# mourisl/T1K

Measured on AMD Instinct MI355X. Metric: genotyped reads/sec (end-to-end genotyper stage, 2x150 bp HLA), higher is better.
Workload: dtype u64

## Files before the change

### include/t1k_gpu.h

```cpp
#ifndef T1K_GPU_H
#define T1K_GPU_H

#include <stddef.h>
#include <stdint.h>

#ifdef __cplusplus
extern "C" {
#endif

typedef enum {
  T1K_OK = 0,
  T1K_ERR_ARG = -1,
  T1K_ERR_DEVICE = -2,
  T1K_ERR_CAPACITY = -3,
  T1K_ERR_IO = -4,
  T1K_ERR_STATE = -5,
  T1K_ERR_INTERNAL = -6,
  T1K_ERR_COMMITTED = -7
} t1k_status;

typedef struct t1k_ctx t1k_ctx;
typedef struct t1k_job t1k_job;
typedef struct t1k_rowset t1k_rowset;
typedef struct t1k_comm t1k_comm;

typedef struct {
  int32_t kmer_length;
  int32_t radius;
  int32_t hit_len_required;
  double ref_seq_similarity;
  int32_t relax_intron_align;
  int32_t max_assign_cnt;
  int32_t max_read_len;
  int32_t workgroups;
  int64_t group_cap;
  int64_t cand_cap;
  int64_t ovl_cap;
  int64_t row_cap;
  int32_t n_base_code;
  int32_t store_chunk_mb;
} t1k_params;

void t1k_params_default(t1k_params *p);

int t1k_ctx_create(int device, const t1k_params *params, t1k_ctx **out);
void t1k_ctx_destroy(t1k_ctx *ctx);
const char *t1k_last_error(const t1k_ctx *ctx);
int t1k_device_count(void);
int t1k_device_memory(int device, uint64_t *freeBytes, uint64_t *totalBytes);

int t1k_ref_upload(t1k_ctx *ctx, const char *seqs, const uint64_t *offsets, const uint8_t *exon, uint32_t nAlleles);

int t1k_reads_upload(t1k_ctx *ctx, const char *seqs, const uint64_t *offsets, const uint32_t *weights, uint32_t nReadEnds);
int t1k_reads_upload_begin(t1k_ctx *ctx, uint32_t nReadEnds, uint64_t textBytes, int maxReadLen);
int t1k_reads_upload_piece(t1k_ctx *ctx, int what, const void *src, uint64_t byteOffset, uint64_t bytes, int slot);
int t1k_reads_upload_wait(t1k_ctx *ctx, int slot);
int t1k_reads_upload_end(t1k_ctx *ctx);

int t1k_reads_dedupe(t1k_ctx *ctx, uint32_t *distinctOf, uint32_t *nDistinct);

typedef struct {
  int32_t seq_idx, read_start, read_end, seq_start, seq_end, strand;
  int32_t match_cnt, left_clip, right_clip, relaxed_match_cnt;
  double similarity;
} t1k_overlap;

int t1k_assign_batch(t1k_ctx *ctx);
int t1k_assign_range(t1k_ctx *ctx, uint64_t first, uint32_t count);
int t1k_overlaps_download(t1k_ctx *ctx, uint32_t *counts, t1k_overlap *ovl, uint64_t cap, uint64_t *total);

typedef struct {
  int32_t allele_idx, start, end;
  float weight, qual, adjust_weight;
} t1k_row_entry;

int t1k_pair_batch(t1k_ctx *ctx, const uint32_t *end1, const uint32_t *end2, const uint8_t *hasN, uint32_t nFragments);
int t1k_rows_download(t1k_ctx *ctx, uint32_t *rowCounts, uint8_t *fragAssigned, t1k_row_entry *rows, uint64_t cap, uint64_t *total);

typedef struct {
  int32_t allele, start, end;
  float weight, adjust_weight;
} t1k_group_entry;
int t1k_rowset_create(t1k_ctx *owner, uint64_t nFragments, const uint8_t *whitelist , t1k_rowset **out);
int t1k_rowset_trim(t1k_rowset *rs, uint64_t n_fragments);
void t1k_rowset_destroy(t1k_rowset *rs);
int t1k_rowset_set_raw(t1k_rowset *rs, int raw);
int t1k_rowset_device_bytes(t1k_rowset *rs, uint64_t *bytes, uint64_t *rowEntries);
const char *t1k_rowset_last_error(const t1k_rowset *rs);
int t1k_pair_into(t1k_ctx *ctx, t1k_rowset *rs, const uint32_t *end1, const uint32_t *end2, const uint8_t *hasN, uint32_t nFragments, uint64_t fragBase);
int t1k_rowset_coalesce(t1k_rowset *rs, uint64_t *nGroups, uint64_t *nEntries, uint64_t *assignedFragments);
int t1k_rowset_coalesce_sized(t1k_rowset *rs, uint64_t *nGroups, uint64_t *nEntries, uint64_t *assignedFragments, void (*sized)(uint64_t nGroups, uint64_t nEntries, void *user), void *user);
int t1k_rowset_groups_download(t1k_rowset *rs, uint64_t *groupPtr, t1k_group_entry *entries, uint32_t *firstFragment);
int t1k_rowset_assigned_download(t1k_rowset *rs, uint8_t *fragAssigned);
int t1k_rowset_assigned_range(t1k_rowset *rs, uint64_t first, uint64_t count, uint8_t *fragAssigned);
int t1k_rowset_rows_download(t1k_rowset *rs, uint64_t first, uint32_t count, uint32_t *rowCounts, t1k_row_entry *rows, uint64_t cap, uint64_t *total);

typedef struct t1k_comm_group t1k_comm_group;
int t1k_comm_unique_id(void *id128);
t1k_comm_group *t1k_comm_group_create(int nRanks);
void t1k_comm_group_destroy(t1k_comm_group *g);
int t1k_comm_init(t1k_ctx *ctx, int nRanks, int rank, const void *id128, t1k_comm_group *group, int transport , t1k_comm **out);
int t1k_comm_bind(t1k_comm *c, t1k_ctx *ctx);
int t1k_comm_abort(t1k_comm *c);
void t1k_comm_destroy(t1k_comm *c);
const char *t1k_comm_last_error(const t1k_comm *c);
int t1k_comm_rank(const t1k_comm *c);
int t1k_comm_size(const t1k_comm *c);
int t1k_comm_is_rccl(const t1k_comm *c);
int t1k_comm_allreduce(t1k_comm *c, void *dev, uint64_t count, int kind);
int t1k_comm_allgather_u64(t1k_comm *c, const uint64_t *mine, uint32_t k, uint64_t *all);
int t1k_comm_alltoallv(t1k_comm *c, const void *sendbuf, const uint64_t *sendOff, void *recvbuf, const uint64_t *recvOff);
int t1k_comm_allgatherv(t1k_comm *c, const void *mine, const uint64_t *bytes, const uint64_t *displ, void *out);
int t1k_comm_allgatherv_host(t1k_comm *c, void *host, const uint64_t *bytes, const uint64_t *displ, uint64_t total);
int t1k_rowset_exchange(t1k_rowset *rs, t1k_comm *comm, uint64_t fragBase);
int t1k_rowset_groups_gather(t1k_rowset *rs, t1k_comm *comm, uint64_t *totalGroups, uint64_t *totalEntries, uint64_t *totalAssigned);
int t1k_rowset_groups_download_all(t1k_rowset *rs, uint32_t *sizes, t1k_group_entry *entries, uint32_t *firstFragment);
int t1k_em_shard(t1k_ctx *ctx, uint32_t rowBegin, uint32_t rowEnd, t1k_comm *comm);

int t1k_coverage_get(t1k_ctx *ctx, int32_t *out, uint64_t cap);
int t1k_coverage_reset(t1k_ctx *ctx);
int t1k_missing_coverage(t1k_ctx *ctx, int32_t *missing);
typedef struct t1k_readset t1k_readset;
int t1k_ctx_set_coverage_mode(t1k_ctx *ctx, int deferred);
int t1k_readset_detach(t1k_ctx *reader, t1k_readset **out);
int t1k_readset_take_store(t1k_readset *rs, t1k_ctx *pipe, int slot);
uint64_t t1k_readset_bytes(const t1k_readset *rs);
uint32_t t1k_readset_size(const t1k_readset *rs);
const char *t1k_readset_last_error(const t1k_readset *rs);
void t1k_readset_destroy(t1k_readset *rs);
int t1k_coverage_selected(t1k_ctx *ctx, t1k_readset *rs, const uint8_t *selected, uint64_t *nRecords);
typedef struct t1k_xwin t1k_xwin;
int t1k_xwin_create(t1k_ctx *owner, uint64_t maxReadEnds, uint32_t maxWindows, t1k_xwin **out);
void t1k_xwin_destroy(t1k_xwin *x);
const char *t1k_xwin_last_error(const t1k_xwin *x);
int t1k_xwin_link(t1k_xwin *x, t1k_ctx *reader, uint32_t window, uint32_t *nExternal);
int t1k_xwin_resolve(t1k_xwin *x, t1k_ctx *ctx, uint32_t window);

int t1k_ref_share(t1k_ctx *dst, const t1k_ctx *src);
uint64_t t1k_pool_release(void);
void *t1k_pinned_alloc(uint64_t bytes);
void t1k_pinned_free(void *p);
int t1k_reads_share(t1k_ctx *dst, const t1k_ctx *src);
int t1k_reads_attach(t1k_ctx *dst, const t1k_ctx *src, int storeSlot, int resetStore);
int t1k_coverage_absorb(t1k_ctx *dst, t1k_ctx *src);

int t1k_extract_batch(t1k_ctx *ctx, uint32_t endsPerFragment, uint8_t *good, uint64_t *stats);

int t1k_align_count_batch(t1k_ctx *ctx, const char *text, const uint32_t *tOff, const char *pat, const uint32_t *pOff, const uint32_t *len, uint32_t nJobs,
                          int32_t *nMatch);
int t1k_align_batch(t1k_ctx *ctx, const char *text, const uint32_t *tOff, const uint32_t *tLen, const char *pat, const uint32_t *pOff,
                    const uint32_t *pLen, uint32_t nJobs, int32_t *score, int32_t *nMatch, int32_t *nMismatch, int32_t *nIndel, int8_t *ops,
                    const uint32_t *opsOff, uint32_t *nOps);

typedef void (*t1k_allreduce_fn)(void *dev_f64, uint64_t n, void *user);
int t1k_em_setup(t1k_ctx *ctx, const uint64_t *rowPtr, const uint32_t *ecIdx, const double *count, const int32_t *ecLen, uint32_t nGroups,
                 uint32_t nEc, t1k_allreduce_fn allreduce, void *user);
int t1k_em_update(t1k_ctx *ctx, const double *x0, double *x1, double *ecReadCount, double *diff);

int t1k_barcode_em(t1k_ctx *ctx, uint32_t nBarcodes, const uint64_t *bcAllelePtr, const uint32_t *bcAllele, const uint64_t *bcGroupPtr,
                   const double *groupCount, const uint64_t *groupEntryPtr, const uint32_t *entryLocal, const double *rho, uint32_t nAlleles,
                   double alpha, double tol, int32_t maxIter, double *nOut, int32_t *itersOut, double *kernelMs);

typedef struct {
  uint64_t read_ends, lookups, postings, hits, groups, candidates, extended, near_best, dp_calls, rows, batches;
  double ms_seed, ms_chain, ms_extend, ms_select, ms_fullalign, ms_pair, ms_em, ms_total;
  uint64_t read_ends_total, pair_overlaps, dp_cells;
  double ms_load, ms_device, ms_coalesce, ms_write;
} t1k_stats;
int t1k_stats_get(t1k_ctx *ctx, t1k_stats *out);
double t1k_alloc_ms(t1k_ctx *ctx, uint64_t *bytes);
uint64_t t1k_ctx_mem_report(t1k_ctx *ctx, const char *tag, int print);

int t1k_genotyper_main(int argc, char **argv);
int t1k_extractor_main(int argc, char **argv);
int t1k_bam_extractor_main(int argc, char **argv);
int t1k_analyzer_main(int argc, char **argv);

typedef struct {
  t1k_params dev;
  double filter_frac, filter_cov, cross_gene_rate, squarem_min_alpha;
  int32_t allele_digit_units;
  char allele_delimiter;
  int32_t threads;
  int32_t device;
  int32_t output_read_assignment;
  int32_t batch_fragments;
} t1k_job_params;
void t1k_job_params_default(t1k_job_params *p);

int t1k_job_create(const t1k_job_params *p, const char *refFasta, t1k_job **out);
void t1k_job_destroy(t1k_job *job);
const char *t1k_job_last_error(const t1k_job *job);
int t1k_job_load_reads(t1k_job *job, const char *file1, const char *file2, const char *barcodeFile);
int t1k_job_load_reads_multi(t1k_job *job, const char *const *files1, uint32_t n1, const char *const *files2, uint32_t n2, const char *barcodeFile);
typedef struct t1k_reads t1k_reads;
int t1k_reads_open(const char *const *files1, uint32_t n1, const char *const *files2, uint32_t n2, const char *barcodeFile, int threads, t1k_reads **out);
int t1k_reads_open_stream(const char *const *files1, uint32_t n1, const char *const *files2, uint32_t n2, const char *barcodeFile, int threads, t1k_reads **out);
const char *t1k_reads_last_error(const t1k_reads *reads);
int t1k_reads_fragments(const t1k_reads *reads, uint64_t *nFragments);
void t1k_reads_close(t1k_reads *reads);
int t1k_job_attach_reads(t1k_job *job, t1k_reads *reads);
int t1k_job_set_reads(t1k_job *job, const char *seq1, const uint64_t *off1, const char *seq2, const uint64_t *off2, uint32_t nFragments);
int t1k_job_run(t1k_job *job);
int t1k_job_set_output_prefix(t1k_job *job, const char *prefix);
int t1k_job_write_outputs(t1k_job *job, const char *prefix);
int t1k_job_genotype_text(t1k_job *job, char *buf, uint64_t cap, uint64_t *needed);
int t1k_job_counts(t1k_job *job, uint64_t *fragments, uint64_t *assignedFragments, uint64_t *groups, uint64_t *ecs, int32_t *emIterations);
int t1k_job_stats(t1k_job *job, t1k_stats *out);
t1k_ctx *t1k_job_ctx(t1k_job *job);
int t1k_job_set_shard(t1k_job *job, int rank, int nRanks, t1k_comm *comm);
int t1k_job_share_reads(t1k_job *dst, t1k_job *src);
int t1k_job_run_local(t1k_job *job);
int t1k_job_finish(t1k_job *job);
int t1k_job_groups_serialize(t1k_job *job, void *buf, uint64_t cap, uint64_t *needed);
int t1k_job_groups_merge(t1k_job *job, const void *const *bufs, const uint64_t *lens, uint32_t n);
int t1k_job_coalesce_rows(t1k_job *job, const t1k_row_entry *rows, const uint32_t *rowCounts, const uint32_t *fragments, uint32_t nFragments);
int t1k_coverage_device(t1k_ctx *ctx, void **devPtr, uint64_t *count);

typedef struct {
  int32_t allele_idx;
  int32_t has_mate_pair, o1_from_r2;
  t1k_overlap o1, o2;
  uint64_t ops1, ops2;
  uint32_t n_ops1, n_ops2;
} t1k_frag_assignment;
int t1k_fragment_details(const t1k_overlap *l1, uint32_t n1, const t1k_overlap *l2, uint32_t n2, int paired, const int32_t *alleles, uint32_t nAlleles,
                         t1k_frag_assignment *out);
typedef struct {
  int32_t allele_idx, ref_pos, exon_pos;
  char ref, var;
  int32_t qual, group, output_group;
  double var_support, all_support, var_uniq_support;
} t1k_variant;
typedef struct t1k_variants t1k_variants;
int t1k_variants_call(t1k_job *job, const double *abundance, int32_t var_max_group, uint32_t nFragments, const uint64_t *asgPtr, const t1k_frag_assignment *asg,
                      const int8_t *ops, const char *const *read1, const uint32_t *len1, const char *const *read2, const uint32_t *len2, t1k_variants **out);
uint32_t t1k_variants_count(const t1k_variants *v);
int t1k_variants_get(const t1k_variants *v, t1k_variant *out );
int t1k_variants_vcf(const t1k_variants *v, char *buf, uint64_t cap, uint64_t *needed);
int t1k_variants_adjust(const t1k_variants *v, const t1k_frag_assignment *asg, uint32_t n, const int8_t *ops, const char *read1, uint32_t len1, const char *read2, uint32_t len2,
                        uint8_t *keep);
void t1k_variants_destroy(t1k_variants *v);

#ifdef __cplusplus
}
#endif
#endif
```

### t1k_amd/capi.py

```python
import ctypes as C
import gzip
import os

import numpy as np

_HERE = os.path.dirname(os.path.abspath(__file__))


def lib_path():
    return os.environ.get("T1K_GPU_LIB") or os.path.join(_HERE, "lib", "libt1k_gpu.so")


class T1kError(RuntimeError):
    pass


class Params(C.Structure):
    _fields_ = [("kmer_length", C.c_int32), ("radius", C.c_int32), ("hit_len_required", C.c_int32),
                ("ref_seq_similarity", C.c_double), ("relax_intron_align", C.c_int32), ("max_assign_cnt", C.c_int32),
                ("max_read_len", C.c_int32), ("workgroups", C.c_int32), ("group_cap", C.c_int64),
                ("cand_cap", C.c_int64), ("ovl_cap", C.c_int64), ("row_cap", C.c_int64), ("n_base_code", C.c_int32), ("store_chunk_mb", C.c_int32)]


class JobParams(C.Structure):
    _fields_ = [("dev", Params), ("filter_frac", C.c_double), ("filter_cov", C.c_double),
                ("cross_gene_rate", C.c_double), ("squarem_min_alpha", C.c_double), ("allele_digit_units", C.c_int32),
                ("allele_delimiter", C.c_char), ("threads", C.c_int32), ("device", C.c_int32),
                ("output_read_assignment", C.c_int32), ("batch_fragments", C.c_int32)]


class Stats(C.Structure):
    _fields_ = [(n, C.c_uint64) for n in ("read_ends", "lookups", "postings", "hits", "groups", "candidates", "extended",
                                          "near_best", "dp_calls", "rows", "batches")] + \
               [(n, C.c_double) for n in ("ms_seed", "ms_chain", "ms_extend", "ms_select", "ms_fullalign", "ms_pair", "ms_em", "ms_total")] + \
               [(n, C.c_uint64) for n in ("read_ends_total", "pair_overlaps", "dp_cells")] + \
               [(n, C.c_double) for n in ("ms_load", "ms_device", "ms_coalesce", "ms_write")]

    def as_dict(self):
        return {n: getattr(self, n) for n, _ in self._fields_}


OVERLAP_DTYPE = np.dtype([("seq_idx", "<i4"), ("read_start", "<i4"), ("read_end", "<i4"), ("seq_start", "<i4"),
                          ("seq_end", "<i4"), ("strand", "<i4"), ("match_cnt", "<i4"), ("left_clip", "<i4"),
                          ("right_clip", "<i4"), ("relaxed_match_cnt", "<i4"), ("similarity", "<f8")])
ROW_DTYPE = np.dtype([("allele_idx", "<i4"), ("start", "<i4"), ("end", "<i4"), ("weight", "<f4"), ("qual", "<f4"),
                      ("adjust_weight", "<f4")])
assert OVERLAP_DTYPE.itemsize == 48 and ROW_DTYPE.itemsize == 24
FRAG_ASG_DTYPE = np.dtype([("allele_idx", "<i4"), ("has_mate_pair", "<i4"), ("o1_from_r2", "<i4"), ("_pad", "<i4"), ("o1", OVERLAP_DTYPE), ("o2", OVERLAP_DTYPE),
                           ("ops1", "<u8"), ("ops2", "<u8"), ("n_ops1", "<u4"), ("n_ops2", "<u4")])
VARIANT_DTYPE = np.dtype([("allele_idx", "<i4"), ("ref_pos", "<i4"), ("exon_pos", "<i4"), ("ref", "S1"), ("var", "S1"), ("_pad", "S2"), ("qual", "<i4"), ("group", "<i4"),
                          ("output_group", "<i4"), ("_pad2", "<i4"), ("var_support", "<f8"), ("all_support", "<f8"), ("var_uniq_support", "<f8")])
assert FRAG_ASG_DTYPE.itemsize == 136 and VARIANT_DTYPE.itemsize == 56

ALLREDUCE_FN = C.CFUNCTYPE(None, C.c_void_p, C.c_uint64, C.c_void_p)

_lib = None


def lib():
    global _lib
    if _lib is not None:
        return _lib
    p = lib_path()
    if not os.path.exists(p):
        raise T1kError("%s not found: run `python -c 'import __graft_entry__ as g; g.build()'` first" % p)
    L = C.CDLL(p)
    vp, u64p, u32p, u8p, i32p = C.c_void_p, C.POINTER(C.c_uint64), C.POINTER(C.c_uint32), C.POINTER(C.c_uint8), C.POINTER(C.c_int32)
    L.t1k_params_default.argtypes = [C.POINTER(Params)]
    L.t1k_ctx_create.argtypes = [C.c_int, C.POINTER(Params), C.POINTER(vp)]
    L.t1k_ctx_destroy.argtypes = [vp]
    L.t1k_last_error.argtypes = [vp]
    L.t1k_last_error.restype = C.c_char_p
    L.t1k_device_count.restype = C.c_int
    L.t1k_ref_upload.argtypes = [vp, C.c_char_p, vp, vp, C.c_uint32]
    L.t1k_reads_upload.argtypes = [vp, C.c_char_p, vp, vp, C.c_uint32]
    L.t1k_assign_batch.argtypes = [vp]
    L.t1k_assign_range.argtypes = [vp, C.c_uint64, C.c_uint32]
    L.t1k_overlaps_download.argtypes = [vp, vp, vp, C.c_uint64, u64p]
    L.t1k_pair_batch.argtypes = [vp, vp, vp, vp, C.c_uint32]
    L.t1k_rows_download.argtypes = [vp, vp, vp, vp, C.c_uint64, u64p]
    L.t1k_coverage_get.argtypes = [vp, vp, C.c_uint64]
    L.t1k_coverage_reset.argtypes = [vp]
    L.t1k_missing_coverage.argtypes = [vp, vp]
    L.t1k_coverage_absorb.argtypes = [vp, vp]
    L.t1k_align_batch.argtypes = [vp, C.c_char_p, vp, vp, C.c_char_p, vp, vp, C.c_uint32, vp, vp, vp, vp, vp, vp, vp]
    L.t1k_align_count_batch.argtypes = [vp, C.c_char_p, vp, C.c_char_p, vp, vp, C.c_uint32, vp]
    L.t1k_em_setup.argtypes = [vp, vp, vp, vp, vp, C.c_uint32, C.c_uint32, ALLREDUCE_FN, vp]
    L.t1k_em_update.argtypes = [vp, vp, vp, vp, vp]
    L.t1k_barcode_em.argtypes = [vp, C.c_uint32, vp, vp, vp, vp, vp, vp, vp, C.c_uint32, C.c_double, C.c_double, C.c_int32, vp, vp, C.POINTER(C.c_double)]
    L.t1k_extract_batch.argtypes = [vp, C.c_uint32, vp, vp]
    L.t1k_extractor_main.argtypes = [C.c_int, C.POINTER(C.c_char_p)]
    L.t1k_stats_get.argtypes = [vp, C.POINTER(Stats)]
    L.t1k_genotyper_main.argtypes = [C.c_int, C.POINTER(C.c_char_p)]
    L.t1k_job_params_default.argtypes = [C.POINTER(JobParams)]
    L.t1k_job_create.argtypes = [C.POINTER(JobParams), C.c_char_p, C.POINTER(vp)]
    L.t1k_job_destroy.argtypes = [vp]
    L.t1k_job_last_error.argtypes = [vp]
    L.t1k_job_last_error.restype = C.c_char_p
    L.t1k_job_load_reads.argtypes = [vp, C.c_char_p, C.c_char_p, C.c_char_p]
    L.t1k_job_set_reads.argtypes = [vp, C.c_char_p, vp, C.c_char_p, vp, C.c_uint32]
    L.t1k_job_run.argtypes = [vp]
    L.t1k_job_write_outputs.argtypes = [vp, C.c_char_p]
    L.t1k_pool_release.restype = C.c_uint64
    L.t1k_pool_release.argtypes = []
    L.t1k_job_load_reads_multi.argtypes = [vp, C.POINTER(C.c_char_p), C.c_uint32, C.POINTER(C.c_char_p), C.c_uint32, C.c_char_p]
    L.t1k_reads_open.argtypes = [C.POINTER(C.c_char_p), C.c_uint32, C.POINTER(C.c_char_p), C.c_uint32, C.c_char_p, C.c_int, C.POINTER(vp)]
    L.t1k_reads_open_stream.argtypes = [C.POINTER(C.c_char_p), C.c_uint32, C.POINTER(C.c_char_p), C.c_uint32, C.c_char_p, C.c_int, C.POINTER(vp)]
    L.t1k_reads_last_error.argtypes = [vp]
    L.t1k_reads_last_error.restype = C.c_char_p
    L.t1k_reads_fragments.argtypes = [vp, u64p]
    L.t1k_reads_close.argtypes = [vp]
    L.t1k_reads_close.restype = None
    L.t1k_job_attach_reads.argtypes = [vp, vp]
    L.t1k_job_genotype_text.argtypes = [vp, C.c_char_p, C.c_uint64, u64p]
    L.t1k_job_counts.argtypes = [vp, u64p, u64p, u64p, u64p, i32p]
    L.t1k_job_stats.argtypes = [vp, C.POINTER(Stats)]
    L.t1k_job_ctx.argtypes = [vp]
    L.t1k_job_ctx.restype = vp
    L.t1k_job_run_local.argtypes = [vp]
    L.t1k_job_finish.argtypes = [vp]
    L.t1k_job_groups_serialize.argtypes = [vp, vp, C.c_uint64, u64p]
    L.t1k_reads_dedupe.argtypes = [vp, vp, u32p]
    L.t1k_job_groups_merge.argtypes = [vp, vp, vp, C.c_uint32]
    L.t1k_job_coalesce_rows.argtypes = [vp, vp, vp, vp, C.c_uint32]
    L.t1k_variants_call.argtypes = [vp, vp, C.c_int32, C.c_uint32, vp, vp, vp, vp, vp, vp, vp, C.POINTER(vp)]
    L.t1k_fragment_details.argtypes = [vp, C.c_uint32, vp, C.c_uint32, C.c_int, vp, C.c_uint32, vp]
    L.t1k_variants_count.argtypes = [vp]
    L.t1k_variants_count.restype = C.c_uint32
    L.t1k_variants_get.argtypes = [vp, vp]
    L.t1k_variants_vcf.argtypes = [vp, vp, C.c_uint64, u64p]
    L.t1k_variants_adjust.argtypes = [vp, vp, C.c_uint32, vp, C.c_char_p, C.c_uint32, C.c_char_p, C.c_uint32, vp]
    L.t1k_variants_destroy.argtypes = [vp]
    L.t1k_job_set_shard.argtypes = [vp, C.c_int, C.c_int, vp]
    L.t1k_job_share_reads.argtypes = [vp, vp]
    L.t1k_job_ctx.restype = vp
    L.t1k_job_ctx.argtypes = [vp]
    L.t1k_comm_unique_id.argtypes = [vp]
    L.t1k_comm_init.argtypes = [vp, C.c_int, C.c_int, vp, vp, C.c_int, C.POINTER(vp)]
    L.t1k_comm_bind.argtypes = [vp, vp]
    L.t1k_comm_destroy.argtypes = [vp]
    L.t1k_comm_last_error.restype = C.c_char_p
    L.t1k_comm_last_error.argtypes = [vp]
    L.t1k_comm_is_rccl.argtypes = [vp]
    L.t1k_comm_group_create.restype = vp
    L.t1k_comm_group_create.argtypes = [C.c_int]
    L.t1k_comm_group_destroy.argtypes = [vp]
    L.t1k_coverage_device.argtypes = [vp, C.POINTER(vp), u64p]
    L.t1k_device_memory.argtypes = [C.c_int, u64p, u64p]
    L.t1k_ctx_set_coverage_mode.argtypes = [vp, C.c_int]
    L.t1k_readset_detach.argtypes = [vp, C.POINTER(vp)]
    L.t1k_readset_take_store.argtypes = [vp, vp, C.c_int]
    L.t1k_readset_bytes.argtypes = [vp]
    L.t1k_readset_bytes.restype = C.c_uint64
    L.t1k_readset_size.argtypes = [vp]
    L.t1k_readset_size.restype = C.c_uint32
    L.t1k_readset_destroy.argtypes = [vp]
    L.t1k_coverage_selected.argtypes = [vp, vp, vp, u64p]
    _lib = L
    return L


def _ptr(a):
    return a.ctypes.data_as(C.c_void_p) if a is not None else None


def _concat(seqs):
    offs = np.zeros(len(seqs) + 1, dtype=np.uint64)
    if len(seqs):
        offs[1:] = np.cumsum([len(s) for s in seqs], dtype=np.uint64)
    blob = "".join(seqs).encode("ascii")
    return blob, offs


class Context:

    def __init__(self, device=0, **kw):
        L = lib()
        p = Params()
        L.t1k_params_default(C.byref(p))
        for k, v in kw.items():
            setattr(p, k, v)
        self.params = p
        h = C.c_void_p()
        rc = L.t1k_ctx_create(device, C.byref(p), C.byref(h))
        if rc != 0:
            raise T1kError("t1k_ctx_create failed (%d): no usable GPU / bad parameters" % rc)
        self.h = h
        self.n_read_ends = 0
        self.allele_len = None

    def _check(self, rc, what):
        if rc != 0:
            raise T1kError("%s failed (%d): %s" % (what, rc, lib().t1k_last_error(self.h).decode()))

    def close(self):
        if self.h:
            lib().t1k_ctx_destroy(self.h)
            self.h = None

    def __del__(self):
        try:
            self.close()
        except Exception:
            pass

    def ref_upload(self, seqs, exon_masks=None):
        blob, offs = _concat(seqs)
        ex = None
        if exon_masks is not None:
            ex = np.concatenate([np.asarray(m, dtype=np.uint8) for m in exon_masks]) if len(seqs) else np.zeros(0, np.uint8)
        self.allele_len = np.array([len(s) for s in seqs], dtype=np.int64)
        self._check(lib().t1k_ref_upload(self.h, blob, _ptr(offs), _ptr(ex), len(seqs)), "t1k_ref_upload")

    def reads_upload(self, seqs, weights=None):
        blob, offs = _concat(seqs)
        w = None if weights is None else np.asarray(weights, dtype=np.uint32)
        self.n_read_ends = len(seqs)
        self._check(lib().t1k_reads_upload(self.h, blob, _ptr(offs), _ptr(w), len(seqs)), "t1k_reads_upload")

    def reads_dedupe(self):
        out = np.zeros(self.n_read_ends, dtype=np.uint32)
        nd = C.c_uint32()
        self._check(lib().t1k_reads_dedupe(self.h, _ptr(out), C.byref(nd)), "t1k_reads_dedupe")
        self.n_uploaded, self.n_read_ends = self.n_read_ends, nd.value
        return out

    def assign(self):
        self._check(lib().t1k_assign_batch(self.h), "t1k_assign_batch")

    def extract(self, ends_per_fragment=1):
        good = np.zeros(self.n_read_ends // ends_per_fragment, dtype=np.uint8)
        st = np.zeros(8, dtype=np.uint64)
        self._check(lib().t1k_extract_batch(self.h, ends_per_fragment, _ptr(good), _ptr(st)), "t1k_extract_batch")
        return good, dict(zip(("read_ends", "lookups", "postings", "read_ends_with_hits", "read_ends_chained", "screen_ns", "main_ns", "big_shape"), (int(x) for x in st)))

    def overlaps(self):
        n = self.n_read_ends
        counts = np.zeros(n, dtype=np.uint32)
        tot = C.c_uint64()
        self._check(lib().t1k_overlaps_download(self.h, _ptr(counts), None, 0, C.byref(tot)), "t1k_overlaps_download")
        out = np.zeros(tot.value, dtype=OVERLAP_DTYPE)
        self._check(lib().t1k_overlaps_download(self.h, _ptr(counts), _ptr(out), tot.value, C.byref(tot)), "t1k_overlaps_download")
        return counts, out

    def pair(self, end1, end2, has_n):
        e1 = np.asarray(end1, dtype=np.uint32)
        e2 = None if end2 is None else np.asarray(end2, dtype=np.uint32)
        hn = np.asarray(has_n, dtype=np.uint8)
        self.n_fragments = len(e1)
        self._check(lib().t1k_pair_batch(self.h, _ptr(e1), _ptr(e2), _ptr(hn), len(e1)), "t1k_pair_batch")

    def rows(self):
        n = self.n_fragments
        counts = np.zeros(n, dtype=np.uint32)
        assigned = np.zeros(n, dtype=np.uint8)
        tot = C.c_uint64()
        self._check(lib().t1k_rows_download(self.h, _ptr(counts), _ptr(assigned), None, 0, C.byref(tot)), "t1k_rows_download")
        out = np.zeros(tot.value, dtype=ROW_DTYPE)
        self._check(lib().t1k_rows_download(self.h, _ptr(counts), _ptr(assigned), _ptr(out), tot.value, C.byref(tot)), "t1k_rows_download")
        return counts, assigned, out

    def coverage(self):
        tot = int(self.allele_len.sum())
        out = np.zeros(tot, dtype=np.int32)
        self._check(lib().t1k_coverage_get(self.h, _ptr(out), tot), "t1k_coverage_get")
        return out

    def set_coverage_mode(self, deferred):
        self._check(lib().t1k_ctx_set_coverage_mode(self.h, 1 if deferred else 0), "t1k_ctx_set_coverage_mode")

    def detach_readset(self, slot=0):
        h = C.c_void_p()
        self._check(lib().t1k_readset_detach(self.h, C.byref(h)), "t1k_readset_detach")
        rs = Readset(h)
        self._check(lib().t1k_readset_take_store(rs.h, self.h, slot), "t1k_readset_take_store")
        return rs

    def coverage_selected(self, readset, selected):
        sel = np.ascontiguousarray(selected, dtype=np.uint8)
        n = C.c_uint64()
        self._check(lib().t1k_coverage_selected(self.h, readset.h, _ptr(sel), C.byref(n)), "t1k_coverage_selected")
        return n.value

    def coverage_reset(self):
        self._check(lib().t1k_coverage_reset(self.h), "t1k_coverage_reset")

    def missing_coverage(self):
        out = np.zeros(len(self.allele_len), dtype=np.int32)
        self._check(lib().t1k_missing_coverage(self.h, _ptr(out)), "t1k_missing_coverage")
        return out

    def stats(self):
        s = Stats()
        lib().t1k_stats_get(self.h, C.byref(s))
        return s.as_dict()

    def align_batch(self, texts, pats, want_ops=True):
        n = len(texts)
        tb, toff = _concat(texts)
        pb, poff = _concat(pats)
        tlen = np.array([len(t) for t in texts], dtype=np.uint32)
        plen = np.array([len(p) for p in pats], dtype=np.uint32)
        toff32, poff32 = toff[:-1].astype(np.uint32), poff[:-1].astype(np.uint32)
        score = np.zeros(n, np.int32); nm = np.zeros(n, np.int32); nx = np.zeros(n, np.int32); ni = np.zeros(n, np.int32)
        ops_off = np.zeros(n, np.uint32)
        if n:
            ops_off[1:] = np.cumsum((tlen + plen + 2)[:-1], dtype=np.uint64).astype(np.uint32)
        ops = np.zeros(int((tlen + plen + 2).sum()) + 8, np.int8)
        nops = np.zeros(n, np.uint32)
        self._check(lib().t1k_align_batch(self.h, tb, _ptr(toff32), _ptr(tlen), pb, _ptr(poff32), _ptr(plen), n, _ptr(score), _ptr(nm),
                                          _ptr(nx), _ptr(ni), _ptr(ops) if want_ops else None, _ptr(ops_off), _ptr(nops)), "t1k_align_batch")
        op_list = [ops[ops_off[i]:ops_off[i] + nops[i]].copy() for i in range(n)] if want_ops else None
        return score, nm, nx, ni, op_list

    def align_count_batch(self, texts, pats):
        n = len(texts)
        tb, toff = _concat(texts)
        pb, poff = _concat(pats)
        ln = np.array([len(t) for t in texts], dtype=np.uint32)
        out = np.zeros(n, np.int32)
        self._check(lib().t1k_align_count_batch(self.h, tb, _ptr(toff[:-1].astype(np.uint32)), pb, _ptr(poff[:-1].astype(np.uint32)), _ptr(ln), n,
                                                _ptr(out)), "t1k_align_count_batch")
        return out

    def em_setup(self, row_ptr, ec_idx, count, ec_len, allreduce=None):
        self._em_keep = (np.asarray(row_ptr, np.uint64), np.asarray(ec_idx, np.uint32), np.asarray(count, np.float64), np.asarray(ec_len, np.int32))
        rp, ei, ct, el = self._em_keep
        self._em_cb = ALLREDUCE_FN(allreduce) if allreduce else C.cast(None, ALLREDUCE_FN)
        self._em_nec = len(el)
        self._check(lib().t1k_em_setup(self.h, _ptr(rp), _ptr(ei), _ptr(ct), _ptr(el), len(ct), len(el), self._em_cb, None), "t1k_em_setup")

    def em_update(self, x0):
        x0 = np.ascontiguousarray(x0, dtype=np.float64)
        x1 = np.zeros(self._em_nec, np.float64)
        n = np.zeros(self._em_nec, np.float64)
        diff = C.c_double()
        self._check(lib().t1k_em_update(self.h, _ptr(x0), _ptr(x1), _ptr(n), C.byref(diff)), "t1k_em_update")
        return x1, n, diff.value

    def barcode_em(self, bc_allele_ptr, bc_allele, bc_group_ptr, group_count, group_entry_ptr, entry_local, rho, n_alleles, alpha=0.0, tol=1e-7,
                   max_iter=1000, raw=False):
        ap = np.ascontiguousarray(bc_allele_ptr, np.uint64)
        al = np.ascontiguousarray(bc_allele, np.uint32)
        gp = np.ascontiguousarray(bc_group_ptr, np.uint64)
        gc = np.ascontiguousarray(group_count, np.float64)
        ep = np.ascontiguousarray(group_entry_ptr, np.uint64)
        el = np.ascontiguousarray(entry_local, np.uint32)
        rh = None if rho is None else np.ascontiguousarray(rho, np.float64)
        nb = max(len(ap) - 1, 0)
        n = np.zeros(len(al), np.float64)
        iters = np.zeros(nb, np.int32)
        ms = C.c_double()
        rc = lib().t1k_barcode_em(self.h, nb, _ptr(ap), _ptr(al), _ptr(gp), _ptr(gc), _ptr(ep), _ptr(el), _ptr(rh), n_alleles, alpha, tol, max_iter,
                                  _ptr(n), _ptr(iters), C.byref(ms))
        if raw:
            return rc
        self._check(rc, "t1k_barcode_em")
        return n, iters, ms.value


class Readset:

    def __init__(self, h):
        self.h = h

    def bytes(self):
        return int(lib().t1k_readset_bytes(self.h))

    def size(self):
        return int(lib().t1k_readset_size(self.h))

    def close(self):
        if self.h:
            lib().t1k_readset_destroy(self.h)
            self.h = None

    def __del__(self):
        try:
            self.close()
        except Exception:
            pass


class Reads:

    def __init__(self, f1, f2=None, barcode=None, threads=0, stream=False):
        l1 = [f1] if isinstance(f1, str) else list(f1)
        l2 = [] if not f2 else ([f2] if isinstance(f2, str) else list(f2))
        a1 = (C.c_char_p * len(l1))(*[x.encode() for x in l1])
        a2 = (C.c_char_p * len(l2))(*[x.encode() for x in l2]) if l2 else None
        h = C.c_void_p()
        opener = lib().t1k_reads_open_stream if stream else lib().t1k_reads_open
        rc = opener(a1, len(l1), a2, len(l2), barcode.encode() if barcode else None, threads, C.byref(h))
        if rc != 0:
            msg = lib().t1k_reads_last_error(h).decode() if h else "bad arguments"
            if h:
                lib().t1k_reads_close(h)
            raise T1kError("t1k_reads_open failed (%d): %s" % (rc, msg))
        self.h = h

    def fragments(self):
        n = C.c_uint64()
        if lib().t1k_reads_fragments(self.h, C.byref(n)) != 0:
            raise T1kError("t1k_reads_fragments failed")
        return n.value

    def close(self):
        if self.h:
            lib().t1k_reads_close(self.h)
            self.h = None

    def __del__(self):
        try:
            self.close()
        except Exception:
            pass


class Job:

    def __init__(self, ref_fasta, **kw):
        L = lib()
        p = JobParams()
        L.t1k_job_params_default(C.byref(p))
        for k, v in kw.items():
            if hasattr(p.dev, k):
                setattr(p.dev, k, v)
            elif k == "allele_delimiter":
                p.allele_delimiter = v.encode() if isinstance(v, str) else v
            else:
                setattr(p, k, v)
        self.params = p
        h = C.c_void_p()
        rc = L.t1k_job_create(C.byref(p), ref_fasta.encode(), C.byref(h))
        if rc != 0:
            msg = L.t1k_job_last_error(h).decode() if h else "no GPU / cannot read reference"
            raise T1kError("t1k_job_create failed (%d): %s" % (rc, msg))
        self.h = h

    def _check(self, rc, what):
        if rc != 0:
            raise T1kError("%s failed (%d): %s" % (what, rc, lib().t1k_job_last_error(self.h).decode()))

    def close(self):
        if self.h:
            lib().t1k_job_destroy(self.h)
            self.h = None

    def __del__(self):
# ... 276 lines not shown
```

### t1k_amd/csrc/t1k_capi.hip

```cpp
#include <sys/mman.h>
#include <map>
#include <mutex>
#include <unordered_map>
#include <algorithm>
#include <memory>
#include <thread>
#include <chrono>
#include <cstring>
#include <cstdio>
#include <cstdlib>
#include "t1k_dev.h"
#include "t1k_launch.h"

namespace {
struct DevPool {
  std::mutex m;
  std::map<int, std::multimap<size_t, void *>> freeBlocks;
  std::unordered_map<void *, std::pair<size_t, int>> live;
  size_t pooled = 0;
};
DevPool &devPool() { static DevPool *p = new DevPool(); return *p; }
}

hipError_t t1k_dev_malloc(void **out, size_t bytes) {
// ... 796 lines not shown
  if ((rc = t1k_ensure(ctx, ctx->bWgStage, (size_t)n * maxChunks * 8 + 64))) return rc;
  const int maxK = t1k_chain_max_kmers(ctx->batchMaxLen, ctx->prm.kmer_length);
  if ((rc = t1k_ensure(ctx, ctx->bWgHits, (size_t)n * (t1k_chain_used_u32(maxK) + 2 + 2 * T1K_USED_MASK_WORDS) * 4 + 64))) return rc;
  if ((rc = t1k_ensure(ctx, ctx->bWgCache, (size_t)n * memoN * 8 + 64))) return rc;
  if ((rc = t1k_ensure(ctx, ctx->bWgBig, (size_t)bigBlocks * 64 * t1k_chain_big_scratch_u32() * 4))) return rc;
  const uint32_t groupSegCap = (uint32_t)std::min<uint64_t>(groupCap / T1K_NSTRIPE, 0xFFFFFFFFull / T1K_NSTRIPE);
  const uint32_t listSegCap = (uint32_t)std::max<uint64_t>(ctx->wList / T1K_NSTRIPE, 1024u), rareSegCap = (uint32_t)std::max<uint64_t>(ctx->wRare / T1K_NSTRIPE, 1024u);
  const uint32_t jobSegCap = jobCap / T1K_NSTRIPE, genCandSegCap = genCandCap / T1K_NSTRIPE;
  const size_t listWords = (size_t)listSegCap * T1K_NSTRIPE, rareWords = (size_t)rareSegCap * T1K_NSTRIPE;
  if ((rc = t1k_ensure(ctx, ctx->bLists, ((size_t)jobCap * 2 + listWords * 6 + rareWords * 6 + (size_t)genCandCap * 6 + genHitCap + (size_t)genJobCap * 2) * 4 + 64))) return rc;
  if ((rc = t1k_ensure(ctx, ctx->bCand, (size_t)ctx->wCand * sizeof(T1kCand)))) return rc;
  if ((rc = t1k_ensure(ctx, ctx->bExt, (size_t)ctx->wCand * sizeof(T1kExt)))) return rc;
  const uint64_t chunkEntries = std::max<uint64_t>(ctx->wOvl, (uint64_t)std::max(1, ctx->prm.store_chunk_mb) * ((1ull << 20) / sizeof(T1kOvlP)));
  {
    const int sl = ctx->storeSlot;
    std::vector<T1kDevBuf> &chunks = ctx->storeChunks[sl];
    for (;;) {
      if (ctx->storeChunk[sl] >= chunks.size()) chunks.resize(ctx->storeChunk[sl] + 1);
      T1kDevBuf &ch = chunks[ctx->storeChunk[sl]];
      if (ch.p && ctx->storeUsed[sl] + ctx->wOvl <= ch.bytes / sizeof(T1kOvlP)) break;
      if (ch.p && ctx->storeUsed[sl] > 0) { ++ctx->storeChunk[sl]; ctx->storeUsed[sl] = 0; continue; }
      if (ch.p) { (void)t1k_dev_free(ch.p); ch.p = nullptr; ch.bytes = 0; }
      const auto t0 = std::chrono::steady_clock::now();
      hipError_t e = t1k_dev_malloc(&ch.p, chunkEntries * sizeof(T1kOvlP));
      ctx->msAlloc += std::chrono::duration<double, std::milli>(std::chrono::steady_clock::now() - t0).count(); ctx->bytesAlloc += chunkEntries * sizeof(T1kOvlP);
      if (e != hipSuccess) { ch.p = nullptr; return t1k_fail(ctx, T1K_ERR_DEVICE, std::string("overlap store: hipMalloc of another ") + std::to_string(chunkEntries * sizeof(T1kOvlP) >> 20) + " MB chunk failed (" + hipGetErrorString(e) + "); fewer fragments per window (T1K_WINDOW) need less"); }
      ch.bytes = chunkEntries * sizeof(T1kOvlP);
    }
    ctx->storeBase = (T1kOvlP *)chunks[ctx->storeChunk[sl]].p + ctx->storeUsed[sl];
  }
  if ((rc = t1k_ensure(ctx, ctx->bOvlWork, (size_t)ctx->wOvl * sizeof(T1kOvl)))) return rc;
  ctx->ovlBase = (T1kOvl *)ctx->bOvlWork.p;
  if ((rc = t1k_ensure(ctx, ctx->bCandStart, (size_t)(n + 1) * 4))) return rc;
  if ((rc = t1k_ensure(ctx, ctx->bCandCount, (size_t)(n + 1) * 4))) return rc;
  if ((rc = t1k_ensure(ctx, ctx->bOvlStart, (size_t)(n + 1) * 4))) return rc;
  if ((rc = t1k_ensure(ctx, ctx->bOvlCount, (size_t)(n + 1) * 4))) return rc;
  if ((rc = t1k_ensure(ctx, ctx->bSortScratch, (size_t)std::min(nWg, 512) * sortCap * 48))) return rc;
  T1K_HIP(ctx, hipMemsetAsync(ctx->bCounters.p, 0, (size_t)T1K_COUNTER_WORDS * 8, ctx->stream));
  T1K_HIP(ctx, hipMemsetAsync(ctx->bOvlCount.p, 0, (size_t)n * 4 + 4, ctx->stream));
  T1K_HIP(ctx, hipMemsetAsync(ctx->bCandCount.p, 0, (size_t)n * 4 + 4, ctx->stream));
  T1K_HIP(ctx, hipMemsetAsync(ctx->bWgCache.p, 0, (size_t)n * memoN * 8, ctx->stream));
  ctx->nCand = ctx->nOvl = 0;
  ctx->traceFetch = 0;
  if (getenv("T1K_DEBUG_TRACE")) fprintf(stderr, "[t1k trace] assign_range first %llu count %u\n", (unsigned long long)first, n);
  memset(&ctx->stats, 0, sizeof(ctx->stats));
  if (n == 0) return T1K_OK;
  unsigned long long hc[64];
  double t0 = nowMs();
  ChainArgs a{};
  a.ref = ctx->ref; a.reads = rd;
  a.k = ctx->prm.kmer_length; a.radius = ctx->prm.radius; a.hitLenRequired = ctx->prm.hit_len_required;
  a.sim = ctx->prm.ref_seq_similarity;
  const int relaxFlag = ctx->prm.relax_intron_align;
  a.recs = (uint32_t *)ctx->bWgGroups.p; a.recStride = (uint32_t)recStride; a.groupCap = groupCap;
  a.chunkStart = (uint32_t *)ctx->bWgStage.p; a.chunkCount = a.chunkStart + (size_t)n * maxChunks; a.maxChunks = maxChunks;
  a.usedOut = (uint32_t *)ctx->bWgHits.p; a.usedCount = a.usedOut + (size_t)n * t1k_chain_used_u32(maxK); a.usedMask = a.usedCount + (size_t)n * 2; a.maxK = (uint32_t)maxK;
  a.maxKFast = (uint32_t)t1k_chain_max_kmers(ctx->batchFastMaxLen, ctx->prm.kmer_length);
  a.memo = (unsigned long long *)ctx->bWgCache.p;
  a.jobList = (uint32_t *)ctx->bLists.p; a.jobCap = jobCap;
  a.jobStr = a.jobList + jobCap;
  a.retryList = a.jobStr + jobCap; a.finishList = a.retryList + listWords; a.slowList = a.finishList + listWords;
  a.retryStr = a.slowList + listWords; a.finishStr = a.retryStr + listWords; a.slowStr = a.finishStr + listWords;
  a.generalList = a.slowStr + listWords; a.bigList = a.generalList + rareWords; a.waveList = a.bigList + rareWords;
  a.generalStr = a.waveList + rareWords; a.bigStr = a.generalStr + rareWords; a.waveStr = a.bigStr + rareWords;
  a.genCand = a.waveStr + rareWords; a.genCandCap = genCandCap;
  a.genHits = a.genCand + (size_t)genCandCap * 6; a.genHitSegCap = genHitCap / T1K_NSTRIPE;
  a.genJobStr = a.genHits + genHitCap; a.genJobList = a.genJobStr + genJobCap; a.genJobSegCap = genJobCap / T1K_NSTRIPE;
  a.groupSegCap = groupSegCap; a.jobSegCap = jobSegCap; a.listSegCap = listSegCap; a.rareSegCap = rareSegCap; a.genCandSegCap = genCandSegCap;
  a.bigScratch = (uint32_t *)ctx->bWgBig.p;
  { static const int ns = getenv("T1K_NO_SIMPLE_CHAIN") ? 0 : 1; a.nearSimple = ns; }
  { static const int fz = getenv("T1K_FUSE_SEED") ? atoi(getenv("T1K_FUSE_SEED")) : 0; a.fuse = fz; }
  { static const int ep = getenv("T1K_NO_EARLY_PRUNE") ? 0 : getenv("T1K_WALK_IN_CLOSED") ? atoi(getenv("T1K_WALK_IN_CLOSED")) + 1 : 2; a.earlyPrune = ep; }
  a.cand = (T1kCand *)ctx->bCand.p; a.candCap = ctx->wCand;
  a.candStart = (uint32_t *)ctx->bCandStart.p; a.candCount = (uint32_t *)ctx->bCandCount.p;
  a.counters = (unsigned long long *)ctx->bCounters.p;
  if ((rc = t1k_run_chain(ctx, a, nWg, bigBlocks, longReads, hc))) return rc;
  double t1 = nowMs();
  if (hc[2]) return capacityError(ctx, hc[2]);
  ctx->nCand = hc[0];
  ExtendArgs e{};
  e.ref = ctx->ref; e.reads = rd; e.k = a.k; e.sim = a.sim;
  e.cand = a.cand; e.ext = (T1kExt *)ctx->bExt.p; e.nCand = ctx->nCand; e.counters = a.counters;
  e.memo = a.memo; e.jobStr = a.jobStr; e.jobSegCap = a.jobSegCap; e.retryStr = a.retryStr; e.retrySegCap = a.listSegCap;
  t1k_launch_extend(ctx, e);
  const bool hostDriven = t1k_chain_host_driven();
  if (hostDriven) {
    if ((rc = fetchCounters(ctx, hc))) return rc;
    const T1kArenaCounts ej = t1k_arena_counts(ctx, T1K_AR_EXTJOBS, e.jobSegCap), er = t1k_arena_counts(ctx, T1K_AR_EXTRETRY, e.retrySegCap);
    if (er.overflow || ej.overflow) return capacityError(ctx, 256);
    t1k_arena_compact(ctx, T1K_AR_EXTJOBS, e.jobStr, e.jobSegCap, a.jobList, ej.maxSeg);
    t1k_arena_compact(ctx, T1K_AR_EXTRETRY, e.retryStr, e.retrySegCap, a.retryList, er.maxSeg);
    t1k_launch_dp_dense(ctx, a, a.jobList, (uint32_t)ej.total);
    t1k_launch_extend_retry(ctx, e, a.retryList, (uint32_t)er.total);
  } else if (ctx->nCand) {
    const uint64_t jobCapAll = (uint64_t)e.jobSegCap * T1K_NSTRIPE, retryCapAll = (uint64_t)e.retrySegCap * T1K_NSTRIPE;
    const uint64_t eJ = t1k_arena_estimate(ctx, T1K_AR_EXTJOBS, jobCapAll, n), eR = t1k_arena_estimate(ctx, T1K_AR_EXTRETRY, retryCapAll, n);
    t1k_arena_compact_dev(ctx, T1K_AR_EXTJOBS, e.jobStr, e.jobSegCap, a.jobList, eJ);
    t1k_arena_compact_dev(ctx, T1K_AR_EXTRETRY, e.retryStr, e.retrySegCap, a.retryList, eR);
    t1k_launch_dp_dense_dev(ctx, a, a.jobList, T1K_AR_EXTJOBS, (uint32_t)jobCapAll, eJ);
    t1k_launch_extend_retry_dev(ctx, e, a.retryList, T1K_AR_EXTRETRY, eR);
  }
  T1K_HIP(ctx, hipEventRecord(ctx->ev[2], ctx->stream));
  if (hostDriven) T1K_HIP(ctx, hipStreamSynchronize(ctx->stream));
  double t2 = nowMs();
  SelectArgs s{};
  s.reads = rd; s.cand = a.cand; s.ext = e.ext; s.candStart = a.candStart; s.candCount = a.candCount;
  s.ovl = ctx->ovlBase; s.ovlCap = ctx->wOvl;
  s.ovlStart = (uint32_t *)ctx->bOvlStart.p; s.ovlCount = (uint32_t *)ctx->bOvlCount.p;
  s.sortScratch = (uint64_t *)ctx->bSortScratch.p; s.sortCap = sortCap; s.counters = a.counters;
  s.alleleBits = 1; s.relax = relaxFlag; s.xl = ctx->batchMaxLen > T1K_MAX_READ_LEN ? 1 : 0;
  while ((1u << s.alleleBits) < ctx->ref.nAlleles) ++s.alleleBits;
  t1k_launch_select(ctx, s, nWg);
  T1K_HIP(ctx, hipEventRecord(ctx->ev[3], ctx->stream));
  if ((rc = fetchCounters(ctx, hc))) return rc;
  double t3 = nowMs();
  if (hc[2]) return capacityError(ctx, hc[2]);
  if (!hostDriven) {
    t1k_arena_estimate_set(ctx, T1K_AR_EXTJOBS, t1k_arena_counts(ctx, T1K_AR_EXTJOBS, e.jobSegCap).total, n);
    t1k_arena_estimate_set(ctx, T1K_AR_EXTRETRY, t1k_arena_counts(ctx, T1K_AR_EXTRETRY, e.retrySegCap).total, n);
  }
  ctx->nOvl = hc[1];
  const bool deferCov = ctx->covMode == 1;
  if (relaxFlag || !deferCov) {
    if (!deferCov) ctx->covCommitted = true;
    if ((rc = t1k_fullalign_phase(ctx, rd, s.ovl, ctx->nOvl, relaxFlag, deferCov ? 1 : 0, ctx->batchMaxLen, false, hc))) return rc;
  } else {
    T1K_HIP(ctx, hipEventRecord(ctx->ev[7], ctx->stream));
    hc[8] = hc[15] = hc[20] = 0;
  }
  hipEvent_t evSlow = ctx->ev[9];
  T1K_HIP(ctx, hipEventRecord(evSlow, ctx->stream));
  TruncArgs tr{};
  tr.reads = rd; tr.ovl = s.ovl; tr.ovlStart = s.ovlStart; tr.ovlCount = s.ovlCount; tr.sortScratch = s.sortScratch; tr.sortCap = sortCap; tr.alleleBits = s.alleleBits;
  tr.counters = a.counters; tr.xl = s.xl;
  t1k_launch_truncate(ctx, tr, nWg);
  T1K_HIP(ctx, hipEventRecord(ctx->ev[4], ctx->stream));
  t1k_launch_publish_lists(ctx, rd.listPtr + first, rd.listCount + first, ctx->ovlBase, ctx->storeBase, ctx->nOvl, s.ovlStart, s.ovlCount, n, a.counters, rd.skip);
  if ((rc = fetchCounters(ctx, hc))) return rc;
  double t4 = nowMs();
  if (hc[2]) return capacityError(ctx, hc[2]);
  ctx->storeUsed[ctx->storeSlot] += ctx->nOvl;
  if (getenv("T1K_DEBUG_PHASES")) {
    float a1 = 0, a2 = 0, a3 = 0;
    (void)hipEventElapsedTime(&a1, ctx->ev[3], ctx->ev[7]); (void)hipEventElapsedTime(&a2, ctx->ev[7], evSlow); (void)hipEventElapsedTime(&a3, evSlow, ctx->ev[4]);
    fprintf(stderr, "[t1k] fullalign %.2f ms, eq-DP (%llu jobs) + general-DP (%llu jobs) %.2f ms, truncate %.2f ms; cand %llu ovl %llu dp %llu; groups %llu (gap walk %llu) fast %llu general %llu big %llu; memo jobs %llu parked %llu wide-queue %llu\n",
            a1, hc[8], hc[15], a2, a3, hc[0], hc[1], hc[7], hc[6], (unsigned long long)ctx->lastSlowGroups, hc[11], hc[12], hc[13], hc[16], hc[17], hc[20]);
#ifdef T1K_NEAR_STATS
    fprintf(stderr, "[t1k] multi-diagonal groups: far strays %llu, near count saturated %llu, other fallback %llu, masks ok but not a chain (<= 32 hits) %llu, (> 32 hits) %llu, chain (<= 96) %llu, chain (> 96) %llu\n", hc[40], hc[41], hc[42], hc[43], hc[47], hc[45], hc[46]);
#endif
#ifdef T1K_WALK_STATS
    fprintf(stderr, "[t1k] gap walk classes: exact without a DP %llu, pruned by the per-gap bound %llu, memo / DP %llu\n", hc[40], hc[41], hc[42]);
#endif
  }
  t1k_stats &st = ctx->stats;
  st.read_ends = n; st.lookups = hc[3]; st.postings = hc[4]; st.hits = hc[5]; st.groups = hc[6]; st.candidates = hc[0]; st.extended = hc[1];
  st.dp_calls = hc[7] + hc[14]; st.near_best = hc[10]; st.dp_cells = hc[24];
  float ms[4] = {0, 0, 0, 0}, msSeed = 0;
  for (int i = 0; i < 4; ++i) (void)hipEventElapsedTime(&ms[i], ctx->ev[i], ctx->ev[i + 1]);
  (void)hipEventElapsedTime(&msSeed, ctx->ev[0], ctx->ev[8]);
  (void)t1; (void)t2; (void)t3;
  st.ms_seed = msSeed; st.ms_chain = ms[0] - msSeed; st.ms_extend = ms[1]; st.ms_select = ms[2]; st.ms_fullalign = ms[3]; st.ms_total = t4 - t0;
  st.batches = 1;
  return T1K_OK;
}

int t1k_overlaps_download(t1k_ctx *ctx, uint32_t *counts, t1k_overlap *out, uint64_t cap, uint64_t *total) {
  if (!ctx) return T1K_ERR_ARG;
  T1K_HIP(ctx, hipSetDevice(ctx->device));
  const uint32_t n = ctx->rangeCount;
  std::vector<uint32_t> start(n), cnt(n);
  if (n) {
    T1K_HIP(ctx, hipMemcpy(start.data(), ctx->bOvlStart.p, (size_t)n * 4, hipMemcpyDeviceToHost));
    T1K_HIP(ctx, hipMemcpy(cnt.data(), ctx->bOvlCount.p, (size_t)n * 4, hipMemcpyDeviceToHost));
  }
  uint64_t tot = 0;
  for (uint32_t i = 0; i < n; ++i) tot += cnt[i];
  if (total) *total = tot;
  if (counts) memcpy(counts, cnt.data(), (size_t)n * 4);
  if (!out) return T1K_OK;
  if (cap < tot) return t1k_fail(ctx, T1K_ERR_ARG, "overlap buffer too small");
  std::vector<T1kOvl> h(ctx->nOvl);
  if (ctx->nOvl) T1K_HIP(ctx, hipMemcpy(h.data(), ctx->ovlBase, ctx->nOvl * sizeof(T1kOvl), hipMemcpyDeviceToHost));
  uint64_t w = 0;
  for (uint32_t i = 0; i < n; ++i) {
    for (uint32_t j = 0; j < cnt[i]; ++j) {
      const T1kOvl &o = h[(uint64_t)start[i] + j];
      t1k_overlap &r = out[w++];
      r.seq_idx = (int32_t)o.allele; r.read_start = o.readStart; r.read_end = o.readEnd; r.seq_start = o.seqStart; r.seq_end = o.seqEnd;
      r.strand = (o.flags & 2) ? -1 : 1;
      r.match_cnt = o.matchCnt; r.left_clip = o.leftClip; r.right_clip = o.rightClip; r.relaxed_match_cnt = o.relaxed;
      r.similarity = (double)o.matchCnt / (double)(o.readEnd - o.readStart + 1 + o.seqEnd - o.seqStart + 1 + 2 * o.leftClip + 2 * o.rightClip);
    }
  }
  return T1K_OK;
}

double t1k_alloc_ms(t1k_ctx *ctx, uint64_t *bytes) {
  if (!ctx) return 0;
  if (bytes) *bytes = ctx->bytesAlloc;
  return ctx->msAlloc;
}

int t1k_stats_get(t1k_ctx *ctx, t1k_stats *out) {
  if (!ctx || !out) return T1K_ERR_ARG;
  *out = ctx->stats;
  return T1K_OK;
}

}
```

### t1k_amd/csrc/t1k_chain.hip

```cpp
#include <algorithm>
#include "t1k_dev.h"
#include "t1k_launch.h"
#include "t1k_memo.h"
#include "t1k_group.h"

#define WG 256
#define GROUP_FAST_MAXLEN 320
#define GENERAL_CAP 128
#define BIG_CAP 16384
#define GA_BIG_MAX 2048
#define GA_SCRATCH_INTS (6 * (GA_BIG_MAX + 4))

enum { ERR_HITCAP = 1, ERR_STAGECAP = 2, ERR_CANDCAP = 4, ERR_BIGGROUP = 8, ERR_OVLCAP = 16, ERR_SORTCAP = 32, ERR_SLOWCAP = 64, ERR_ROWCAP = 128, ERR_GROUPCAP = 256, ERR_MEMO = 512 };

struct CandOut {
  uint32_t *dst;
  int n;
  int stride = 3;
  int cap = 0x7FFFFFFF;
  bool overflow = false;
  __device__ void push(int rs, int re, int ss, int se, int m0, int m) {
    if (n >= cap) { overflow = true; return; }
    dst[stride * n + 0] = (uint32_t)rs | ((uint32_t)re << 12);
    dst[stride * n + 1] = (uint32_t)ss | ((uint32_t)m0 << 20);
    dst[stride * n + 2] = (uint32_t)se | ((uint32_t)m << 20);
    if (stride == 6) dst[6 * n + 3] = dst[6 * n + 4] = dst[6 * n + 5] = 0;
    ++n;
  }
  __device__ void setRefs(const uint32_t *refs, int nref) {
    if (overflow || stride != 6 || n == 0) return;
    uint32_t *d = dst + 6 * (n - 1);
    d[0] |= (uint32_t)nref << 24; d[3] = refs[0]; d[4] = refs[1]; d[5] = refs[2];
  }
};

__device__ inline int gapMatches(const ReadCtx &c, int ra, int ga, int lp, int lt, int *gaScratch, int gaMax, unsigned int *dpCounter, unsigned long long *errFlags,
                                 bool *needScratch) {
  if (lp == lt) return t1k_ga_matches_window(c.rb, c.rn, ra, c.gb, c.gn, c.goff + ga, lp, dpCounter);
  if (lt == 0 || lp == 0) return 0;
  if (dpCounter) ++*dpCounter;
  T1kSeqView T{c.gb, c.gn, c.goff + ga}, P{c.rb, c.rn, ra};
  const int diff = lt > lp ? lt - lp : lp - lt;
  if (diff <= 4) return t1k_ga_band<4, false>(T, lt, P, lp, nullptr, 0);
  if (!gaScratch) { *needScratch = true; return 0; }
  int nm = 0;
  if (lt > gaMax) { atomicOr(errFlags, (unsigned long long)ERR_BIGGROUP); return 0; }
  t1k_ga_general(T, lt, P, lp, gaScratch, nullptr, &nm);
  return nm;
}

template <int MW>
__device__ __forceinline__ void shlOr(uint64_t *C, int sft) {
#pragma unroll
  for (int w = MW - 1; w >= 0; --w) {
    uint64_t carry = w > 0 ? (C[w - 1] >> (64 - sft)) : 0ull;
    C[w] |= (C[w] << sft) | carry;
  }
}

#define GROUP_MAX_REFS 4
template <int NW, bool DEFER, bool CLOSED, bool ONDEMAND = false>
__device__ inline int groupFastPath(const uint32_t *Mw, int diag, const ReadCtx &c, bool hasN, int k, int hitLenRequired, double simThreshold, CandOut &out,
                                    unsigned int *dpCounter, int strandBit, const GapSink &sink, uint32_t *refs, int *nRefs, int earlyPrune = 1) {
  constexpr int MW = (NW + 1) / 2;
  uint64_t M[MW];
  int onDiag = 0;
#pragma unroll
  for (int i = 0; i < MW; ++i) {
    M[i] = (uint64_t)Mw[2 * i] | ((2 * i + 1 < NW) ? ((uint64_t)Mw[2 * i + 1] << 32) : 0ull);
    onDiag += __popcll(M[i]);
  }
  if (onDiag < 3) return 1;
  if (onDiag * k < hitLenRequired) return 1;
  int first = -1, last = -1;
#pragma unroll
  for (int w = 0; w < MW; ++w) {
    if (M[w]) {
      if (first < 0) first = w * 64 + __ffsll((long long)M[w]) - 1;
      last = w * 64 + 63 - __clzll((long long)M[w]);
    }
  }
  uint64_t C[MW];
#pragma unroll
  for (int w = 0; w < MW; ++w) C[w] = M[w];
  {
    int have = 1;
    while (2 * have <= k) { shlOr<MW>(C, have); have *= 2; }
    if (have < k) shlOr<MW>(C, k - have);
  }
  int cov = 0;
#pragma unroll
  for (int w = 0; w < MW; ++w) cov += __popcll(C[w]);
  if (cov < hitLenRequired) return 1;
  const int spanEnd = last + k, span = spanEnd - first;
  uint64_t mmw[NW];
  int mmT = 0;
  {
    const int64_t g0 = c.goff + (first - diag);
    const int64_t gw = g0 >> 5;
    const int gsh = (int)(g0 & 31) * 2, rsh = (first & 31) * 2;
    const int rw = first >> 5;
    const int nWin = (span + 31) >> 5;
    constexpr int NP = (NW + 2) / 2;
    if (ONDEMAND) {
      uint64_t G[2 * NP];
#pragma unroll
      for (int j = 0; j < NP; ++j) {
        t1k_u64x2 g = {0ull, 0ull};
        if (2 * j <= nWin) g = *(const t1k_u64x2 *)(c.gb + gw + 2 * j);
        G[2 * j] = g.x; G[2 * j + 1] = g.y;
      }
#pragma unroll
      for (int i = 0; i < NW; ++i) {
        mmw[i] = 0;
        if (i < nWin) {
          const uint64_t r0 = c.rb[rw + i], r1 = c.rb[rw + i + 1], n0 = c.rn[rw + i], n1 = c.rn[rw + i + 1];
          const uint64_t g = (G[i] >> gsh) | ((G[i + 1] << 1) << (63 - gsh)), r = (r0 >> rsh) | ((r1 << 1) << (63 - rsh));
          uint64_t nn = (n0 >> rsh) | ((n1 << 1) << (63 - rsh));
          if (hasN) { const uint64_t q0 = c.gn[gw + i], q1 = c.gn[gw + i + 1]; nn |= (q0 >> gsh) | ((q1 << 1) << (63 - gsh)); }
          const uint64_t xo = g ^ r;
          uint64_t mm = (xo | (xo >> 1)) & T1K_EVEN & ~nn;
          const int rem = span - 32 * i;
          if (rem < 32) mm &= t1k_lowmask(rem);
          mmw[i] = mm;
          mmT += __popcll(mm);
        }
      }
    } else {
    uint64_t G[2 * NP], R[2 * NP], GN[2 * NP], RN[2 * NP];
    const uint64_t *gt = c.gT ? c.gT + (gw - (c.goff >> 5)) * 64 : nullptr;
#pragma unroll
    for (int j = 0; j < NP; ++j) {
      const bool need = 2 * j <= nWin;
      t1k_u64x2 g = {0ull, 0ull}, r = {0ull, 0ull}, rn2 = {0ull, 0ull};
      if (need) {
        if (gt) { g.x = gt[(2 * j) * 64]; g.y = gt[(2 * j + 1) * 64]; } else g = *(const t1k_u64x2 *)(c.gb + gw + 2 * j);
        r = *(const t1k_u64x2 *)(c.rb + rw + 2 * j); rn2 = *(const t1k_u64x2 *)(c.rn + rw + 2 * j);
      }
      G[2 * j] = g.x; G[2 * j + 1] = g.y; R[2 * j] = r.x; R[2 * j + 1] = r.y; RN[2 * j] = rn2.x; RN[2 * j + 1] = rn2.y;
      GN[2 * j] = GN[2 * j + 1] = 0ull;
    }
    if (hasN) {
#pragma unroll
      for (int j = 0; j < NP; ++j) {
        if (2 * j <= nWin) { const t1k_u64x2 g = *(const t1k_u64x2 *)(c.gn + gw + 2 * j); GN[2 * j] = g.x; GN[2 * j + 1] = g.y; }
      }
    }
#pragma unroll
    for (int i = 0; i < NW; ++i) {
      mmw[i] = 0;
      if (i < nWin) {
        const uint64_t g = (G[i] >> gsh) | ((G[i + 1] << 1) << (63 - gsh)), r = (R[i] >> rsh) | ((R[i + 1] << 1) << (63 - rsh));
        const uint64_t nn = ((GN[i] >> gsh) | ((GN[i + 1] << 1) << (63 - gsh))) | ((RN[i] >> rsh) | ((RN[i + 1] << 1) << (63 - rsh)));
        const uint64_t xo = g ^ r;
        uint64_t mm = (xo | (xo >> 1)) & T1K_EVEN & ~nn;
        const int rem = span - 32 * i;
        if (rem < 32) mm &= t1k_lowmask(rem);
        mmw[i] = mm;
        mmT += __popcll(mm);
      }
    }
    }
  }
  int matchCnt;
  int result = 1;
  auto nextClear = [&](int from) -> int {
#pragma unroll
    for (int w = 0; w < MW; ++w) {
      if (from < (w + 1) * 64) {
        uint64_t inv = ~C[w];
        if (from > w * 64) inv &= ~0ull << (from - w * 64);
        if (inv) return w * 64 + __ffsll((long long)inv) - 1;
      }
    }
    return MW * 64;
  };
  auto nextSet = [&](int from) -> int {
#pragma unroll
    for (int w = 0; w < MW; ++w) {
      if (from < (w + 1) * 64) {
        uint64_t v = C[w];
        if (from > w * 64) v &= ~0ull << (from - w * 64);
        if (v) return w * 64 + __ffsll((long long)v) - 1;
      }
    }
    return MW * 64;
  };
  auto mmIn = [&](int gsAbs, int geAbs) -> int {
    const int gs = gsAbs - first, ge = geAbs - first;
    int x = 0;
#pragma unroll
    for (int q = 0; q < NW; ++q) {
      const int p0 = q * 32;
      if (p0 < ge && p0 + 32 > gs) {
        uint64_t msk = ~0ull;
        if (gs > p0) msk &= ~t1k_lowmask(gs - p0);
        if (ge < p0 + 32) msk &= t1k_lowmask(ge - p0);
        x += __popcll(mmw[q] & msk);
      }
    }
    return x;
  };
  if (mmT <= 3) matchCnt = 2 * (span - mmT);
  else if (CLOSED) {
    uint64_t X[MW], E[MW];
    {
      const int ws = first >> 6, bs = first & 63;
#pragma unroll
      for (int w = 0; w < MW; ++w) {
        uint64_t lo = 0, hi = 0;
#pragma unroll
        for (int v = 0; v < MW; ++v) {
          if (v == w + ws) lo = C[v];
          if (v == w + ws + 1) hi = C[v];
        }
        const uint64_t crel = bs ? ((lo >> bs) | (hi << (64 - bs))) : lo;
        const int rem = span - 64 * w;
        X[w] = rem <= 0 ? 0ull : (~crel & (rem >= 64 ? ~0ull : ((1ull << rem) - 1ull)));
        uint64_t e = 0;
#pragma unroll
        for (int h = 0; h < 2; ++h) {
          if (2 * w + h < NW) {
            uint64_t x = mmw[2 * w + h] & 0x5555555555555555ull;
            x = (x | (x >> 1)) & 0x3333333333333333ull; x = (x | (x >> 2)) & 0x0F0F0F0F0F0F0F0Full; x = (x | (x >> 4)) & 0x00FF00FF00FF00FFull;
            x = (x | (x >> 8)) & 0x0000FFFF0000FFFFull; x = (x | (x >> 16)) & 0xFFFFFFFFull;
            e |= x << (32 * h);
          }
        }
        E[w] = e & X[w];
      }
    }
    int nGaps = 0;
    uint64_t carry = 0;
#pragma unroll
    for (int w = 0; w < MW; ++w) {
      const uint64_t s1 = X[w] + E[w], s2 = s1 + carry;
      carry = ((s1 < X[w]) | (s2 < s1)) ? 1ull : 0ull;
      nGaps += __popcll(s2 & ~X[w]);
    }
    const int bound = 2 * (span - nGaps);
    if (earlyPrune && (double)bound / (double)(2 * span) < simThreshold) matchCnt = bound;
    else if (earlyPrune < 2) return 5;
    else {
      int sumSmall = 0, nBig = 0;
      int pos = first;
      while (true) {
        int gs = nextClear(pos);
        if (gs >= spanEnd) break;
        int ge = nextSet(gs);
        if (ge > spanEnd) ge = spanEnd;
        const int x = mmIn(gs, ge);
        if (x <= 3) sumSmall += x; else ++nBig;
        pos = ge;
      }
      const int upper = 2 * (span - sumSmall - nBig);
      if (nBig != 0 && !((double)upper / (double)(2 * span) < simThreshold)) return 5;
      matchCnt = upper;
    }
  }
  else {
    int sumSmall = 0, nBig = 0;
    int pos = first;
    while (true) {
      int gs = nextClear(pos);
      if (gs >= spanEnd) break;
      int ge = nextSet(gs);
      if (ge > spanEnd) ge = spanEnd;
      int x = mmIn(gs, ge);
      if (x <= 3) sumSmall += x; else ++nBig;
      pos = ge;
    }
    const int upper = 2 * (span - sumSmall - nBig);
#ifdef T1K_WALK_STATS
    { const int cls = nBig == 0 ? 0 : ((double)upper / (double)(2 * span) < simThreshold) ? 1 : 2;
      for (int c = 0; c < 3; ++c) { const unsigned long long mk = __ballot(cls == c); if (mk && (int)(threadIdx.x & 63) == __ffsll((long long)mk) - 1) atomicAdd(&sink.counters[40 + c], (unsigned long long)__popcll(mk)); } }
#endif
    if (nBig == 0) matchCnt = upper;
    else if ((double)upper / (double)(2 * span) < simThreshold) matchCnt = upper;
    else {
      int gapMatch = 0, nref = 0;
      bool again = false;
      pos = first;
      while (true) {
        int gs = nextClear(pos);
        if (gs >= spanEnd) break;
        int ge = nextSet(gs);
        if (ge > spanEnd) ge = spanEnd;
        int x = mmIn(gs, ge);
        if (x <= 3) gapMatch += (ge - gs) - x;
        else {
          uint32_t slot = 0;
          int r = gapMatchesCached<DEFER>(c, gs, c.goff + (gs - diag), ge - gs, ge - gs, strandBit, sink, dpCounter, &slot);
          if (r >= 0) gapMatch += r;
          else if (r == -1 && nref < GROUP_MAX_REFS) { refs[nref >> 1] |= slot << (16 * (nref & 1)); ++nref; }
          else again = true;
        }
        pos = ge;
      }
      if (again) return 2;
      matchCnt = 2 * cov + 2 * gapMatch;
      if (nref) { *nRefs = nref; result = 3; }
    }
  }
  out.push(first, last + k - 1, first - diag, last - diag + k - 1, 2 * cov, matchCnt);
  return result;
}

template <class Arr>
__device__ inline void chainRun(const ReadCtx &c, int k, int hitLenRequired, Arr A, Arr B, Arr C, int s, int m, int *gaScratch, int gaMax, CandOut &out,
                                unsigned int *dpCounter, unsigned long long *errFlags, bool *needScratch, const GapSink *sink, int strandBit, bool chainReady = false) {
    int ret, lenR, lenS;
    if (!t1k_run_lis(A, B, C, s, m, k, hitLenRequired, &ret, &lenR, &lenS, chainReady)) return;
    uint32_t refs[3] = {0, 0, 0};
    int nref = 0;
    auto gapM = [&](int ra, int ga, int lp, int lt) -> int {
      if (!sink) return gapMatches(c, ra, ga, lp, lt, gaScratch, gaMax, dpCounter, errFlags, needScratch);
      if (lp <= 0 || lt <= 0) return 0;
      const int diff = lt > lp ? lt - lp : lp - lt;
      if (diff > 4) { *needScratch = true; return 0; }
      uint32_t slot = 0;
      const int r = gapMatchesCached<true>(c, ra, c.goff + ga, lp, lt, strandBit, *sink, dpCounter, &slot);
      if (r >= 0) return r;
      if (r == -1 && nref < GROUP_MAX_REFS) { refs[nref >> 1] |= slot << (16 * (nref & 1)); ++nref; return 0; }
      if (dpCounter) ++*dpCounter;
      return gapAlign(c, ra, c.goff + ga, lp, lt);
    };
    int matchCnt = 2 * k;
    for (int i = 1; i < ret; ++i) {
      int pa = (int)(A[s + i - 1] & 0xFFF), pb = (int)(A[s + i - 1] >> 12), qa = (int)(A[s + i] & 0xFFF), qb = (int)(A[s + i] >> 12);
      bool sameDiag = (pb - pa) == (qb - qa);
      bool readOv = pa + k - 1 >= qa, seqOv = pb + k - 1 >= qb;
      if (sameDiag) {
        if (readOv) matchCnt += 2 * (qa - pa);
        else matchCnt += 2 * k + 2 * gapM(pa + k, pb + k, qa - (pa + k), qb - (pb + k));
      } else {
        if (readOv && !seqOv) matchCnt += 2 * (qa - pa);
        else if (!readOv && seqOv) matchCnt += 2 * (qb - pb);
        else if (readOv && seqOv) matchCnt += 2 * ((qa - pa) < (qb - pb) ? (qa - pa) : (qb - pb));
        else matchCnt += 2 * k + 2 * gapM(pa + k, pb + k, qa - (pa + k), qb - (pb + k));
      }
    }
    int rs = (int)(A[s] & 0xFFF), ss = (int)(A[s] >> 12);
    int re = (int)(A[s + ret - 1] & 0xFFF) + k - 1, se = (int)(A[s + ret - 1] >> 12) + k - 1;
    out.push(rs, re, ss, se, 2 * lenR, matchCnt);
    out.setRefs(refs, nref);
}

template <class Arr>
__device__ inline void groupGeneral(const uint32_t *h, int n, const ReadCtx &c, int k, int radius, int hitLenRequired, Arr A, Arr B,
                                     Arr C, int *gaScratch, int gaMax, CandOut &out, unsigned int *dpCounter, unsigned long long *errFlags, bool *needScratch,
                                     const GapSink *sink = nullptr, int strandBit = 0) {
  for (int i = 0; i < n; ++i) {
    uint32_t x = h[i];
    int j = i - 1;
    while (j >= 0 && hitKeyLess(x, A[j])) { A[j + 1] = A[j]; --j; }
    A[j + 1] = x;
  }
  for (int s = 0; s < n;) {
    auto diagOf = [](uint32_t x) { return (int)(x & 0xFFF) - (int)(x >> 12); };
    int curDiff = diagOf(A[s]), curCnt = 1, domCnt = 0, dominant = 0;
    int e = s + 1;
    for (; e < n; ++e) {
      int d = diagOf(A[e]) - diagOf(A[e - 1]);
      if (d < 0) d = -d;
      if (d > radius) break;
      if (d == 0) ++curCnt;
      else {
        if (curCnt > domCnt) { dominant = curDiff; domCnt = curCnt; }
        curDiff = diagOf(A[e]); curCnt = 1;
      }
    }
    if (curCnt > domCnt) dominant = curDiff;
    if (e - s < 3 || (e - s) * k < hitLenRequired) { s = e; continue; }
    int m = 0;
    for (int q = s; q < e; ++q) {
      int a = (int)(A[q] & 0xFFF);
      int dq = diagOf(A[q]) - dominant; if (dq < 0) dq = -dq;
      bool keep = true;
      for (int r = s; r < e; ++r) {
        if ((int)(A[r] & 0xFFF) != a) continue;
        int dr = diagOf(A[r]) - dominant; if (dr < 0) dr = -dr;
        if (dr < dq) { keep = false; break; }
      }
      if (keep) {
        uint32_t x = A[q];
        int j = m - 1;
        while (j >= 0 && x < B[j]) { B[j + 1] = B[j]; --j; }
        B[j + 1] = x;
        ++m;
      }
    }
    chainRun(c, k, hitLenRequired, A, B, C, s, m, gaScratch, gaMax, out, dpCounter, errFlags, needScratch, sink, strandBit);
    s = e;
  }
}

template <class Arr>
__device__ inline void groupSimple(const uint32_t *h, int n, const ReadCtx &c, int k, int hitLenRequired, Arr A, CandOut &out, unsigned int *dpCounter,
                                   unsigned long long *errFlags, bool *needScratch, const GapSink *sink, int strandBit) {
  for (int i = 0; i < n; ++i) A[i] = h[i];
  if (n < 3 || n * k < hitLenRequired) return;
  chainRun(c, k, hitLenRequired, A, A, A, 0, n, nullptr, 0, out, dpCounter, errFlags, needScratch, sink, strandBit, true);
}

struct VoteKey {
  uint64_t hi, lo;
  __device__ bool operator<(const VoteKey &o) const { return hi != o.hi ? hi < o.hi : lo < o.lo; }
};
__device__ __forceinline__ VoteKey voteKey(int matchCnt0, int rs, int re, uint32_t allele, int strandPlus, int ss, int se) {
  VoteKey k;
  k.hi = ((uint64_t)(4095 - matchCnt0) << 40) | ((uint64_t)(4095 - (re - rs)) << 26) | ((uint64_t)allele << 1) | (uint64_t)strandPlus;
  k.lo = ((uint64_t)rs << 52) | ((uint64_t)re << 40) | ((uint64_t)ss << 20) | (uint64_t)se;
  return k;
}


#define CHUNK_A T1K_SEED_CHUNK
__device__ __forceinline__ uint32_t packDiagMeta(int diag, uint32_t meta) {
  const uint32_t strays = meta & 0xFFFFu, nearCnt = meta >> 16;
  return (uint32_t)(diag + (1 << 21)) | (min(strays - nearCnt, 7u) << 22) | (min(nearCnt, 31u) << 25);
}
__device__ __forceinline__ int recDiag(uint32_t w2) { return (int)(w2 & 0x3FFFFFu) - (1 << 21); }
__device__ __forceinline__ uint32_t recFar(uint32_t w2) { return (w2 >> 22) & 7u; }
__device__ __forceinline__ uint32_t recNear(uint32_t w2) { return (w2 >> 25) & 31u; }
__device__ __forceinline__ bool recIsGeneral(uint32_t w2) { return recNear(w2) > 0 || recFar(w2) > 2; }
#define REC_NEAR_DONE 0x4E454152u
enum { REC_DONE = 0x80000000u };

__device__ __forceinline__ ReadCtx makeCtx(const ChainArgs &P, uint32_t re, int pass, uint32_t allele) {
  const int S = P.reads.S;
  ReadCtx c{P.reads.bases + ((uint64_t)re * 2 + pass) * S, P.reads.nmask + ((uint64_t)re * 2 + pass) * S, (int)P.reads.len[re], P.ref.bases, P.ref.nmask,
            (int64_t)P.ref.alleleOff[allele], (int)P.ref.alleleLen[allele], P.ref.anyN != 0};
  if (P.ref.basesT) c.gT = P.ref.basesT + (uint64_t)P.ref.blockT[allele >> 6] + (allele & 63u);
  return c;
}

#define DIAG_EMPTY 0x7FFFFFFF

template <int NW>
__device__ __forceinline__ uint32_t closedFormGroup(uint32_t *a, const uint64_t *rb, const uint64_t *rn, const uint64_t *gb, const uint64_t *gn, int64_t goff, bool anyN, bool hasN, int k,
                                                    int hitLenRequired, double sim, int pass, int earlyPrune) {
  uint32_t Mw[NW];
#pragma unroll
  for (int w = 0; w < NW; ++w) Mw[w] = a[2 + w];
  const ReadCtx c{rb, rn, 0, gb, gn, goff, 0, anyN};
  uint32_t cbuf[3];
  CandOut out{cbuf, 0};
  const GapSink sink{nullptr, nullptr, nullptr, 0u, 0u, T1K_AR_JOBS};
  uint32_t refs[2] = {0, 0};
  int nRefs = 0;
  const uint32_t kind = (uint32_t)groupFastPath<NW, true, true, true>(Mw, (int)a[0], c, hasN, k, hitLenRequired, sim, out, nullptr, pass, sink, refs, &nRefs, earlyPrune);
  if (kind == 1u && out.n) { a[2] = cbuf[0]; a[3] = cbuf[1]; a[4] = cbuf[2]; return 6u; }
  return kind;
}

#ifndef T1K_SEED_WAVES
#define T1K_SEED_WAVES 7
#endif
#ifndef T1K_SEED_PACK_Q
#define T1K_SEED_PACK_Q 0
#endif
#ifndef T1K_FUSE_WAVES
#define T1K_FUSE_WAVES 5
#endif
template <int NW, bool FUSE>
__device__ __forceinline__ void seedGroupsBody(const ChainArgs &P) {
  constexpr int AW = NW == 5 ? 7 : 13;
  extern __shared__ uint32_t lds[];
  const int k = P.k;
  const int maxK = (int)P.maxKFast;
  uint32_t *acc = lds;
  uint32_t *ukCode = acc;
  uint32_t *ukStart = ukCode + maxK;
  uint32_t *ukLen = ukStart + maxK;
  uint32_t *ukDir = ukLen + maxK;
  uint16_t *usedQ = (uint16_t *)(ukDir + maxK);
  uint32_t *sLo = acc + CHUNK_A * AW;
  uint32_t *pre = sLo + maxK;
  uint32_t *lstStart = pre + maxK + 1;
  uint32_t *lstLen = lstStart + maxK;
  uint32_t *lstDir = lstLen + maxK;
#if T1K_SEED_PACK_Q
  uint16_t *qOf = (uint16_t *)(lstDir + maxK);
#define LST_LEN(x) ((x) & 0x7FFFFFu)
#else
  uint16_t *qOf = (uint16_t *)(lstDir + maxK);
#define LST_LEN(x) (x)
#endif
  const uint32_t A = P.ref.nAlleles;
  const uint32_t nChunks = P.ref.kDirStride - 1;
  uint32_t *bitmaps = 2 * ((A + 31) >> 5) <= (uint32_t)(CHUNK_A * AW) ? acc : (uint32_t *)(qOf + (T1K_SEED_PACK_Q ? 0 : ((maxK + 1) & ~1)));
  __shared__ uint32_t warpSums[4];
  __shared__ uint32_t sHot[8];
  __shared__ uint32_t sUsed[2], sGroupBase, sFallback, sPost;
  __shared__ int sWaveMax[4];
  const int tid = threadIdx.x;
  const uint32_t kmask = (1u << (2 * k)) - 1;
  const uint32_t stride = P.recStride;
  for (uint32_t i = tid; i < CHUNK_A * AW; i += WG) acc[i] = (i % AW) == 0 ? (uint32_t)DIAG_EMPTY : 0u;
  __syncthreads();
#ifdef T1K_SEED_PROFILE
  uint64_t tp_[8] = {0, 0, 0, 0, 0, 0, 0, 0}, tl_ = __builtin_amdgcn_s_memtime();
#endif
  __shared__ uint32_t sUMask[2 * T1K_USED_MASK_WORDS];
  constexpr int RDW = 14;
  __shared__ uint64_t sRd[2][2][FUSE ? RDW : 1];
  __shared__ unsigned long long sStat[3];
  if (tid == 0) { sStat[0] = 0; sStat[1] = 0; sStat[2] = 0; }
  unsigned int fastLocal = 0, groupsLocal = 0, recsLocal = 0;
  for (uint32_t re = blockIdx.x; re < P.reads.nReadEnds; re += gridDim.x) {
    const int len = P.reads.len[re];
    const int S = P.reads.S;
    const uint64_t *rbase = P.reads.bases + (uint64_t)re * 2 * S;
    const uint64_t *rnm = P.reads.nmask + (uint64_t)re * 2 * S;
    for (int c = tid; c < P.maxChunks; c += WG) P.chunkCount[(uint64_t)re * P.maxChunks + c] = 0;
    if (tid == 0) { P.usedCount[2 * re] = 0; P.usedCount[2 * re + 1] = 0; }
    if (len < k || len > T1K_MAX_READ_LEN || (P.reads.skip && P.reads.skip[re])) { __syncthreads(); continue; }
    const int nk = len - k + 1;
    if (tid < 2 * T1K_USED_MASK_WORDS) sUMask[tid] = 0;
    if (FUSE && tid >= 64 && tid < 64 + 2 * 2 * RDW) {
      const int x = tid - 64, strand = x / (2 * RDW), kind = (x / RDW) & 1, w = x % RDW;
      sRd[strand][kind][w] = w < S ? (kind ? rnm : rbase)[strand * S + w] : 0ull;
    }
    for (int q = tid; q < 2 * nk; q += WG) {
      int pass = q / nk, p = q - pass * nk;
      const uint64_t *b = rbase + pass * S, *nm = rnm + pass * S;
      uint32_t code = (uint32_t)t1k_get32(b, p) & kmask;
      bool valid = ((uint32_t)t1k_get32(nm, p) & kmask) == 0;
      uint32_t st = 0, ln = 0, dr = T1K_NO_DIR;
      if (valid) { st = P.ref.kStart[code]; ln = P.ref.kStart[code + 1] - st; dr = P.ref.kDirIdx[code]; }
      ukCode[q] = code | (valid ? 0x80000000u : 0);
      ukStart[q] = st; ukLen[q] = ln; ukDir[q] = dr;
    }
    __syncthreads();

#ifdef T1K_SEED_PROFILE
    { const uint64_t tn_ = __builtin_amdgcn_s_memtime(); tp_[0] += tn_ - tl_; tl_ = tn_; }
#endif
    const int W1 = k / 2 + 1;
    if (tid == 0) { sFallback = 0; sUsed[0] = 0; sUsed[1] = 0; sPost = 0; }
    __syncthreads();
    int qv[3], lastNonBig[3];
    uint32_t szv[3];
    bool bigv[3];
    {
      int localMax = -1;
#pragma unroll
      for (int x = 0; x < 3; ++x) {
        const int q = 3 * tid + x;
        qv[x] = q; szv[x] = 0; bigv[x] = false; lastNonBig[x] = -1;
        if (q < 2 * nk) {
          const int pass = q >= nk ? 1 : 0, p = q - pass * nk;
          const uint32_t code = ukCode[q] & 0x7FFFFFFFu;
          for (int d = 1; d <= W1 && d <= p; ++d)
            if ((ukCode[q - d] & 0x7FFFFFFFu) == code) sFallback = 1;
// ... 726 lines not shown
          if (have < k) andShifted(k - have);
        }
        const int aLo = d > 0 ? d : 0, aHi = d + alleleLen - k;
#pragma unroll
        for (int j = 0; j < NW; ++j) {
          uint32_t m = evenBits32(acc[j] & pst[j]) & um[j];
          const int p0 = 32 * j;
          if (aLo > p0) m &= aLo - p0 >= 32 ? 0u : ~0u << (aLo - p0);
          if (aHi < p0 + 31) m &= aHi < p0 ? 0u : ~0u >> (31 - (aHi - p0));
          if (dl == 0) { if (j == 0) same0 = true; same0 = same0 && m == rv[3 + j]; continue; }
          if (m) {
            if (nearDiags == 0 || d1 != d) { ++nearDiags; if (nearDiags == 1) d1 = d; }
            if (nearDiags == 1) M1[j] = m;
          }
          cntNear += __popc(m);
          while (m) {
            const int p = __ffs((int)m) - 1;
            m &= m - 1;
            const uint32_t a = (uint32_t)(p0 + p);
            if (w < base + n) P.genHits[w] = ((uint32_t)((int)a - d) << 12) | a;
            ++w;
          }
        }
      }
      ok = same0 && cntNear == nearCnt;
      bool simple = false;
      if (ok && P.nearSimple && nearDiags == 1 && n >= 3 && (int)n * k >= P.hitLenRequired) {
        int lo0 = -1, hi0 = -1, lo1 = -1, hi1 = -1;
#pragma unroll
        for (int j = 0; j < NW; ++j) {
          if (rv[3 + j]) { if (lo0 < 0) lo0 = 32 * j + __ffs((int)rv[3 + j]) - 1; hi0 = 32 * j + 31 - __clz((int)rv[3 + j]); }
          if (M1[j]) { if (lo1 < 0) lo1 = 32 * j + __ffs((int)M1[j]) - 1; hi1 = 32 * j + 31 - __clz((int)M1[j]); }
        }
        const bool first0 = hi0 < lo1 && hi0 - d0 < lo1 - d1, first1 = hi1 < lo0 && hi1 - d1 < lo0 - d0;
        if (first0 || first1) {
          simple = true;
          w = base;
          for (int part = 0; part < 2; ++part) {
            const bool zero = (part == 0) == first0;
            const int dd = zero ? d0 : d1;
#pragma unroll
            for (int j = 0; j < NW; ++j) {
              uint32_t m = zero ? rv[3 + j] : M1[j];
              while (m) {
                const int p = __ffs((int)m) - 1;
                m &= m - 1;
                const uint32_t a = (uint32_t)(32 * j + p);
                P.genHits[w++] = ((uint32_t)((int)a - dd) << 12) | a;
              }
            }
          }
        }
      }
      if (ok && simple) { rec[3] = base; rec[4] = n; rec[6] = 1u; toWave = n > 3 * GENERAL_SMALL; }
      else if (ok) {
        rec[6] = 0u;
#pragma unroll
        for (int j = 0; j < NW; ++j) {
          uint32_t m = rv[3 + j];
          while (m) {
            const int p = __ffs((int)m) - 1;
            m &= m - 1;
            const uint32_t a = (uint32_t)(32 * j + p);
            P.genHits[w++] = ((uint32_t)((int)a - d0) << 12) | a;
          }
        }
        rec[3] = base; rec[4] = n;
        toWave = n > GENERAL_SMALL;
      }
    }
    rec[5] = ok ? REC_NEAR_DONE : 0u;
    if (!ok) rec[6] = 0u;
#ifdef T1K_NEAR_STATS
    {
      int cls = 42;
      if (recFar(rv[2]) != 0) cls = 40; else if (nearCnt == 31) cls = 41; else if (ok) cls = rec[6] == 1u ? (n > 96 ? 46 : 45) : (n > 32 ? 47 : 43);
      atomicAdd(&P.counters[cls], 1ull);
    }
#endif
  }
  if (toWave) { const uint32_t wq = t1k_arena_append(P.counters, T1K_AR_WAVE, P.rareSegCap); if (wq != T1K_ARENA_FULL) P.waveStr[wq] = gi; }
  }
}

template <int ROUNDS>
__global__ __launch_bounds__(WG) void k_gather_general(ChainArgs P, uint32_t nItems, int skipDone, const unsigned long long *nDev) {
  if (nDev) { if (P.counters[2]) return; nItems = (uint32_t)*nDev; }
  const int lane = threadIdx.x & 63;
  const uint32_t wave = (blockIdx.x * WG + threadIdx.x) >> 6, nWaves = gridDim.x * (WG / 64);
  const int maxK = (int)P.maxK;
  static_assert(ROUNDS * 64 >= GROUP_FAST_MAXLEN, "lists of one strand");
  for (uint32_t q = wave; q < nItems; q += nWaves) {
    const uint32_t gi = P.generalList[q];
    uint32_t *rec = P.recs + (uint64_t)gi * P.recStride;
    if (skipDone && rec[5] == REC_NEAR_DONE) continue;
    const uint32_t re = rec[0] & 0x7FFFFFFFu, allele = rec[1];
    const int pass = (rec[0] >> 31) ? 0 : 1;
    const uint32_t nPlus = P.usedCount[2 * re], nMinus = P.usedCount[2 * re + 1];
    const uint32_t b = pass == 0 ? 0 : nPlus, e = pass == 0 ? nPlus : nPlus + nMinus;
    const uint32_t *uo = P.usedOut + (uint64_t)re * maxK * 4;
    uint32_t first[ROUNDS], cnt[ROUNDS], mine = 0;
#pragma unroll
    for (int r = 0; r < ROUNDS; ++r) {
      const uint32_t u = b + lane + 64 * r;
      first[r] = 0; cnt[r] = 0;
      if (u < e) {
        const uint32_t st = uo[4 * u + 1], ln = uo[4 * u + 2], dr = uo[4 * u + 3];
        uint32_t l = 0, rr = ln;
        if (dr != T1K_NO_DIR) {
          const uint32_t *dir = P.ref.kDir + (uint64_t)dr * P.ref.kDirStride;
          const uint32_t ci = allele / T1K_SEED_CHUNK;
          l = dir[ci]; rr = dir[ci + 1];
        }
        while (l < rr) { uint32_t m = (l + rr) >> 1; if (P.ref.kPost[st + m].allele < allele) l = m + 1; else rr = m; }
        uint32_t c = 0;
        while (l + c < ln && P.ref.kPost[st + l + c].allele == allele) ++c;
        first[r] = st + l; cnt[r] = c; mine += c;
      }
    }
    uint32_t incl = mine;
#pragma unroll
    for (int o = 1; o < 64; o <<= 1) { uint32_t y = __shfl_up(incl, o, 64); if (lane >= o) incl += y; }
    const uint32_t n = __shfl(incl, 63, 64);
    uint32_t base = 0;
    if (lane == 0) {
      if (n > WAVE_CAP) {
        const uint32_t bq = t1k_arena_append(P.counters, T1K_AR_BIG, P.rareSegCap);
        if (bq != T1K_ARENA_FULL) P.bigStr[bq] = gi;
        rec[4] = 0xFFFFFFFFu;
      } else {
        base = n ? t1k_arena_alloc(P.counters, T1K_AR_GENHITS, n, P.genHitSegCap) : 0u;
        rec[3] = base; rec[4] = n;
        if (n > GENERAL_SMALL) {
          const uint32_t wq = t1k_arena_append(P.counters, T1K_AR_WAVE, P.rareSegCap);
          if (wq != T1K_ARENA_FULL) P.waveStr[wq] = gi;
        }
      }
    }
    base = __shfl(base, 0, 64);
    if (n <= WAVE_CAP && base != T1K_ARENA_FULL) {
      uint32_t w = base + incl - mine;
#pragma unroll
      for (int r = 0; r < ROUNDS; ++r) {
        const uint32_t u = b + lane + 64 * r;
        if (cnt[r]) {
          const uint32_t rOff = uo[4 * u];
          for (uint32_t j = 0; j < cnt[r]; ++j) P.genHits[w++] = (P.ref.kPost[first[r] + j].offset << 12) | rOff;
        }
      }
    }
  }
}

__global__ __launch_bounds__(64) void k_chain_general(ChainArgs P, uint32_t nItems, int useSimple, const unsigned long long *nDev) {
  __shared__ uint32_t sArr[3 * GENERAL_SMALL * 64];
  if (nDev) { if (P.counters[2]) return; nItems = (uint32_t)*nDev; }
  unsigned int dpLocal = 0, genLocal = 0;
  for (uint32_t qb = blockIdx.x * 64; qb < nItems; qb += gridDim.x * 64) {
  const uint32_t q = qb + threadIdx.x;
  uint32_t nHits = 0xFFFFFFFFu;
  bool simple = false;
  if (q < nItems) {
    const uint32_t *r0 = P.recs + (uint64_t)P.generalList[q] * P.recStride;
    nHits = r0[4];
    simple = useSimple && r0[5] == REC_NEAR_DONE && r0[6] == 1u;
  }
  if (nHits <= GENERAL_SMALL || (simple && nHits <= 3 * GENERAL_SMALL)) {
    const uint32_t gi = P.generalList[q];
    uint32_t *rec = P.recs + (uint64_t)gi * P.recStride;
    const uint32_t re = rec[0] & 0x7FFFFFFFu, allele = rec[1];
    const int pass = (rec[0] >> 31) ? 0 : 1;
    ReadCtx c = makeCtx(P, re, pass, allele);
    const int n = (int)nHits;
    if (rec[3] == T1K_ARENA_FULL) atomicOr(&P.counters[2], (unsigned long long)ERR_STAGECAP);
    const uint32_t *hh = P.genHits + (rec[3] == T1K_ARENA_FULL ? 0u : rec[3]);
    bool needScratch = false;
    uint32_t cbuf[2 * GENERAL_SMALL + 6];
    CandOut out{cbuf, 0, 6, GENERAL_SMALL / 3 + 1};
    const GapSink sink{P.memo + (uint64_t)re * GAP_CACHE, P.genJobStr, P.counters, re * GAP_CACHE, P.genJobSegCap, T1K_AR_GENJOBS};
    LaneArr A{sArr + threadIdx.x}, B{sArr + GENERAL_SMALL * 64 + threadIdx.x}, C{sArr + 2 * GENERAL_SMALL * 64 + threadIdx.x};
    if (simple) groupSimple(hh, n, c, P.k, P.hitLenRequired, A, out, &dpLocal, &P.counters[2], &needScratch, &sink, pass);
    else groupGeneral(hh, n, c, P.k, P.radius, P.hitLenRequired, A, B, C, nullptr, 0, out, &dpLocal, &P.counters[2], &needScratch, &sink, pass);
    if (needScratch) { const uint32_t b = t1k_arena_append(P.counters, T1K_AR_BIG, P.rareSegCap); if (b != T1K_ARENA_FULL) P.bigStr[b] = gi; }
    else {
      ++genLocal;
      uint32_t base = 0;
      if (out.n) {
        base = t1k_arena_alloc(P.counters, T1K_AR_GENCAND, (uint32_t)out.n, P.genCandSegCap);
        if (base == T1K_ARENA_FULL) { atomicOr(&P.counters[2], (unsigned long long)ERR_STAGECAP); out.n = 0; base = 0; }
        for (int i = 0; i < 6 * out.n; ++i) P.genCand[(uint64_t)base * 6 + i] = cbuf[i];
      }
      rec[3] = base;
      rec[2] = REC_DONE | 0x40000000u | (uint32_t)out.n;
    }
  }
  }
  t1k_stat_add(P.counters, T1K_STAT_DP, dpLocal);
  t1k_stat_add(P.counters, T1K_STAT_GENERAL, genLocal);
}

__global__ __launch_bounds__(64) void k_chain_wave(ChainArgs P, uint32_t nItems, const unsigned long long *nDev, uint32_t cap, uint32_t above) {
  extern __shared__ uint32_t sW[];
  if (nDev) { if (P.counters[2]) return; nItems = (uint32_t)*nDev; }
  uint32_t *A = sW, *B = sW + cap, *C = sW + 2 * cap;
  const int lane = threadIdx.x;
  unsigned int dpLocal = 0, genLocal = 0;
  auto diagOf = [](uint32_t x) { return (int)(x & 0xFFF) - (int)(x >> 12); };
  for (uint32_t q = blockIdx.x; q < nItems; q += gridDim.x) {
    const uint32_t gi = P.waveList[q];
    uint32_t *rec = P.recs + (uint64_t)gi * P.recStride;
    const uint32_t re = rec[0] & 0x7FFFFFFFu, allele = rec[1];
    const int pass = (rec[0] >> 31) ? 0 : 1;
    const int n = (int)rec[4];
    if ((uint32_t)n <= above || (uint32_t)n > cap) continue;
    const bool lost = rec[3] == T1K_ARENA_FULL;
    if (lost && lane == 0) atomicOr(&P.counters[2], (unsigned long long)ERR_STAGECAP);
    const uint32_t *hh = P.genHits + (lost ? 0u : rec[3]);
    ReadCtx c = makeCtx(P, re, pass, allele);
    const int k = P.k;
    __syncthreads();
    for (int i = lane; i < n; i += 64) C[i] = hh[i];
    __syncthreads();
    for (int i = lane; i < n; i += 64) {
      const uint32_t x = C[i];
      int r = 0;
      for (int j = 0; j < n; ++j) r += hitKeyLess(C[j], x) ? 1 : 0;
      A[r] = x;
    }
    __syncthreads();
    bool needScratch = false;
    uint32_t cbuf[192];
    CandOut out{cbuf, 0, 6, 32};
    const GapSink sink{P.memo + (uint64_t)re * GAP_CACHE, P.genJobStr, P.counters, re * GAP_CACHE, P.genJobSegCap, T1K_AR_GENJOBS};
    for (int s = 0; s < n;) {
      int curDiff = diagOf(A[s]), curCnt = 1, domCnt = 0, dominant = 0;
      int e = s + 1;
      for (; e < n; ++e) {
        int d = diagOf(A[e]) - diagOf(A[e - 1]);
        if (d < 0) d = -d;
        if (d > P.radius) break;
        if (d == 0) ++curCnt;
        else {
          if (curCnt > domCnt) { dominant = curDiff; domCnt = curCnt; }
          curDiff = diagOf(A[e]); curCnt = 1;
        }
      }
      if (curCnt > domCnt) dominant = curDiff;
      if (e - s < 3 || (e - s) * k < P.hitLenRequired) { s = e; continue; }
      int mine = 0;
      for (int qq = s + lane; qq < e; qq += 64) {
        const int a = (int)(A[qq] & 0xFFF);
        int dq = diagOf(A[qq]) - dominant; if (dq < 0) dq = -dq;
        bool keep = true;
        for (int r = s; r < e; ++r) {
          if ((int)(A[r] & 0xFFF) != a) continue;
          int dr = diagOf(A[r]) - dominant; if (dr < 0) dr = -dr;
          if (dr < dq) { keep = false; break; }
        }
        C[qq] = keep ? 1u : 0u;
        mine += keep ? 1 : 0;
      }
      for (int o = 32; o > 0; o >>= 1) mine += __shfl_xor(mine, o, 64);
      const int m = mine;
      __syncthreads();
      for (int qq = s + lane; qq < e; qq += 64) {
        if (!C[qq]) continue;
        const uint32_t x = A[qq];
        int r = 0;
        for (int t = s; t < e; ++t) r += (C[t] && A[t] < x) ? 1 : 0;
        B[r] = x;
      }
      __syncthreads();
      if (lane == 0) chainRun(c, k, P.hitLenRequired, A, B, C, s, m, nullptr, 0, out, &dpLocal, &P.counters[2], &needScratch, &sink, pass);
      __syncthreads();
      s = e;
    }
    if (lane == 0) {
      if (out.overflow) atomicOr(&P.counters[2], (unsigned long long)ERR_BIGGROUP);
      if (needScratch) { const uint32_t b = t1k_arena_append(P.counters, T1K_AR_BIG, P.rareSegCap); if (b != T1K_ARENA_FULL) P.bigStr[b] = gi; }
      else {
        ++genLocal;
        uint32_t base = 0;
        if (out.n) {
          base = t1k_arena_alloc(P.counters, T1K_AR_GENCAND, (uint32_t)out.n, P.genCandSegCap);
          if (base == T1K_ARENA_FULL) { atomicOr(&P.counters[2], (unsigned long long)ERR_STAGECAP); out.n = 0; base = 0; }
          for (int i = 0; i < 6 * out.n; ++i) P.genCand[(uint64_t)base * 6 + i] = cbuf[i];
        }
        rec[3] = base;
        rec[2] = REC_DONE | 0x40000000u | (uint32_t)out.n;
      }
    }
  }
  t1k_stat_add(P.counters, T1K_STAT_DP, dpLocal);
  t1k_stat_add(P.counters, T1K_STAT_GENERAL, genLocal);
}

__global__ __launch_bounds__(WG) void k_general_finish(ChainArgs P, uint32_t nItems, const unsigned long long *nDev) {
  if (nDev) { if (P.counters[2]) return; nItems = (uint32_t)*nDev; }
  for (uint32_t q = blockIdx.x * blockDim.x + threadIdx.x; q < nItems; q += gridDim.x * blockDim.x) {
  const uint32_t *rec = P.recs + (uint64_t)P.generalList[q] * P.recStride;
  if ((rec[2] & (REC_DONE | 0x40000000u)) != (REC_DONE | 0x40000000u)) continue;
  const uint32_t re = rec[0] & 0x7FFFFFFFu, nc = rec[2] & 0x3FFFFFFFu;
  const unsigned long long *memo = P.memo + (uint64_t)re * GAP_CACHE;
  for (uint32_t j = 0; j < nc; ++j) {
    uint32_t *g = P.genCand + ((uint64_t)rec[3] + j) * 6;
    const int nref = (int)((g[0] >> 24) & 0xF);
    if (!nref) continue;
    uint32_t sum = 0;
    for (int i = 0; i < nref; ++i) {
      const uint32_t slot = (g[3 + (i >> 1)] >> (16 * (i & 1))) & 0xFFFFu;
      const unsigned long long e = __hip_atomic_load(&memo[slot], __ATOMIC_RELAXED, __HIP_MEMORY_SCOPE_AGENT);
      const uint32_t v = GAP_VAL(e);
      if (v == GAP_PENDING) atomicOr(&P.counters[2], (unsigned long long)ERR_MEMO);
      sum += v;
    }
    g[2] += (2u * sum) << 20;
    g[0] &= 0x00FFFFFFu;
  }
  }
}

__global__ __launch_bounds__(64) void k_chain_big(ChainArgs P, uint32_t nItems, const unsigned long long *nDev) {
  __shared__ int sGa[GA_SCRATCH_INTS];
  if (threadIdx.x != 0) return;
  if (nDev) { if (P.counters[2]) return; nItems = (uint32_t)*nDev; }
  const uint32_t t = blockIdx.x, nT = gridDim.x;
  uint32_t *mine = P.bigScratch + (uint64_t)t * (4 * BIG_CAP);
  unsigned int dpLocal = 0;
  for (uint32_t q = t; q < nItems; q += nT) {
    const uint32_t gi = P.bigList[q];
    uint32_t *rec = P.recs + (uint64_t)gi * P.recStride;
    const uint32_t re = rec[0] & 0x7FFFFFFFu, allele = rec[1];
    const int pass = (rec[0] >> 31) ? 0 : 1;
    ReadCtx c = makeCtx(P, re, pass, allele);
    uint32_t *hh = mine + 3 * BIG_CAP;
    const int n = gatherHits(P, re, pass, allele, hh, BIG_CAP);
    if (n > BIG_CAP) { atomicOr(&P.counters[2], (unsigned long long)ERR_BIGGROUP); rec[2] = REC_DONE; continue; }
    bool dummy = false;
    uint32_t cbuf[192];
    CandOut o2{cbuf, 0, 6, 32};
    groupGeneral(hh, n, c, P.k, P.radius, P.hitLenRequired, mine, mine + BIG_CAP, mine + 2 * BIG_CAP, sGa, GA_BIG_MAX, o2, &dpLocal,
                 &P.counters[2], &dummy);
    if (o2.overflow) atomicOr(&P.counters[2], (unsigned long long)ERR_BIGGROUP);
    uint32_t base = 0;
    if (o2.n) {
      base = t1k_arena_alloc(P.counters, T1K_AR_GENCAND, (uint32_t)o2.n, P.genCandSegCap);
      if (base == T1K_ARENA_FULL) { atomicOr(&P.counters[2], (unsigned long long)ERR_STAGECAP); o2.n = 0; base = 0; }
      for (int i = 0; i < 6 * o2.n; ++i) P.genCand[(uint64_t)base * 6 + i] = cbuf[i];
    }
    rec[3] = base;
    rec[2] = REC_DONE | 0x40000000u | (uint32_t)o2.n;
    atomicAdd(&P.counters[13], 1ull);
  }
  if (dpLocal) atomicAdd(&P.counters[7], (unsigned long long)dpLocal);
}


template <int MAXLEN>
__device__ __forceinline__ bool lowComplexityFromCounts(const uint16_t (*cnt)[MAXLEN + 1], int rs, int re) {
  const int L = re - rs + 1;
  int low = 0, lowTotal = 0;
#pragma unroll
  for (int b = 0; b < 4; ++b) {
    const int c = (int)cnt[b][re + 1] - (int)cnt[b][rs];
    if (c <= 2) { ++low; lowTotal += c; }
  }
  if (lowTotal * 7 >= L) return false;
  return low >= 2;
}
template <int MAXLEN>
__device__ __forceinline__ bool keepCandidate(const ChainArgs &P, const uint16_t (*baseCnt)[4][MAXLEN + 1], int plus, uint32_t w0, uint32_t w1, uint32_t w2) {
  const int rs = (int)(w0 & 0xFFF), rend = (int)((w0 >> 12) & 0xFFF), ss = (int)(w1 & 0xFFFFF), se = (int)(w2 & 0xFFFFF);
  const int matchCnt = (int)(w2 >> 20);
  const double sim = (double)matchCnt / (double)(se - ss + 1 + rend - rs + 1);
  if (sim < P.sim) return false;
  if (lowComplexityFromCounts<MAXLEN>(baseCnt[plus ? 0 : 1], rs, rend)) return !(0.0 < P.sim);
  return true;
}

__device__ __forceinline__ uint32_t pendingMatchWord(const ChainArgs &P, uint32_t re, uint32_t nRefs, uint32_t w2, uint32_t s0, uint32_t s1) {
  const unsigned long long *memo = P.memo + (uint64_t)re * GAP_CACHE;
  uint32_t sum = 0;
  for (uint32_t i = 0; i < nRefs; ++i) {
    const uint32_t slot = ((i >> 1 ? s1 : s0) >> (16 * (i & 1))) & 0xFFFFu;
    const unsigned long long e = __hip_atomic_load(&memo[slot], __ATOMIC_RELAXED, __HIP_MEMORY_SCOPE_AGENT);
    const uint32_t v = GAP_VAL(e);
    if (v == GAP_PENDING) atomicOr(&P.counters[2], (unsigned long long)ERR_MEMO);
    sum += v;
  }
  return w2 + ((2u * sum) << 20);
}
__device__ __forceinline__ bool recPending(uint32_t state) { return !(state & REC_DONE) && state >= 1u && state <= (uint32_t)GROUP_MAX_REFS; }

#if T1K_COLLECT_WAVES > 0
#define T1K_COLLECT_ATTR T1K_WAVES_ATTR_(T1K_COLLECT_WAVES)
#else
#define T1K_COLLECT_ATTR
#endif
template <int MAXLEN>
__global__ __launch_bounds__(WG) T1K_COLLECT_ATTR void k_collect(ChainArgs P) {
  __shared__ uint32_t warpSums[4];
  __shared__ uint16_t sBaseCnt[2][4][MAXLEN + 1];
  __shared__ uint64_t sVote[2 * WG];
  uint64_t *sVoteHi = sVote, *sVoteLo = sVote + WG;
  __shared__ uint32_t sBase;
  constexpr int MAXCH = 2 * 256 + 2;
  __shared__ uint32_t sCs[MAXCH], sPre[MAXCH + 1], sNCh;
  __shared__ uint8_t sChPlus[MAXCH];
  uint32_t *sPreW = (uint32_t *)sVote;
  static_assert(sizeof(uint64_t) * 2 * WG >= sizeof(uint32_t) * (MAXCH + 1), "the copy-out prefix does not fit the vote arrays");
  constexpr uint32_t KEEP_BITS = 65536;
  __shared__ uint32_t sKeepBits[KEEP_BITS / 32];
  const int tid = threadIdx.x;
  const uint32_t stride = P.recStride;
  if (P.devDriven && P.counters[2]) return;
  __shared__ uint32_t sNextRe;
  uint32_t hoNext = 0, hoLeft = 0;
  for (;;) {
    __syncthreads();
    if (tid == 0) {
      if (hoLeft == 0) { hoNext = (uint32_t)atomicAdd(&P.counters[27], (unsigned long long)T1K_COLLECT_HANDOUT); hoLeft = T1K_COLLECT_HANDOUT; }
      sNextRe = hoNext++; --hoLeft;
    }
    __syncthreads();
    const uint32_t re = sNextRe;
    if (re >= P.reads.nReadEnds) break;
    const uint32_t *cs = P.chunkStart + (uint64_t)re * P.maxChunks, *cc = P.chunkCount + (uint64_t)re * P.maxChunks;
    for (uint32_t i = tid; i < KEEP_BITS / 32; i += WG) sKeepBits[i] = 0;
    {
      const int len = (int)P.reads.len[re], S = P.reads.S;
      for (int idx = tid; idx < 2 * (len + 1); idx += WG) {
        const int strand = idx / (len + 1), p = idx - strand * (len + 1);
        const uint64_t *rb = P.reads.bases + ((uint64_t)re * 2 + strand) * S, *rn = P.reads.nmask + ((uint64_t)re * 2 + strand) * S;
        int c[4] = {0, 0, 0, 0};
        for (int o = 0; o < p; o += 32) {
          const uint64_t x = rb[o >> 5], nn = rn[o >> 5];
          const uint64_t valid = T1K_EVEN & ~nn & t1k_lowmask(p - o);
          const uint64_t lo = x & T1K_EVEN, hi = (x >> 1) & T1K_EVEN;
          c[0] += __popcll(~lo & ~hi & valid); c[1] += __popcll(lo & ~hi & valid); c[2] += __popcll(~lo & hi & valid); c[3] += __popcll(lo & hi & valid);
        }
#pragma unroll
        for (int b = 0; b < 4; ++b) sBaseCnt[strand][b][p] = (uint16_t)c[b];
      }
      __syncthreads();
    }
    if (tid < 64) {
      uint32_t carry = 0, nDense = 0;
// ... 60 lines not shown
          nCand[plus] += kc; kept += kc;
        }
        if (kept && rv[u] < KEEP_BITS) atomicOr(&sKeepBits[rv[u] >> 5], 1u << (rv[u] & 31));
      }
    }
    sVoteHi[tid] = best.hi; sVoteLo[tid] = best.lo;
    __syncthreads();
    for (int o = WG / 2; o > 0; o >>= 1) {
      if (tid < o) {
        VoteKey a{sVoteHi[tid], sVoteLo[tid]}, b{sVoteHi[tid + o], sVoteLo[tid + o]};
        if (b < a) { sVoteHi[tid] = b.hi; sVoteLo[tid] = b.lo; }
      }
      __syncthreads();
    }
    const uint32_t winPlus = (uint32_t)(sVoteHi[0] & 1);
    __syncthreads();
    uint32_t totWin;
    t1k_block_scan_exclusive(nCand[winPlus], warpSums, &totWin);
    if (tid == 0) {
      unsigned long long b = totWin ? atomicAdd(&P.counters[0], (unsigned long long)totWin) : 0ull;
      if (b + totWin > P.candCap) { atomicOr(&P.counters[2], (unsigned long long)ERR_CANDCAP); sBase = 0xFFFFFFFFu; P.candStart[re] = 0; P.candCount[re] = 0; }
      else { sBase = (uint32_t)b; P.candStart[re] = (uint32_t)b; P.candCount[re] = totWin; }
    }
    __syncthreads();
    if (sBase != 0xFFFFFFFFu && totWin) {
      if (tid < 64) {
        uint32_t carry = 0;
        if (tid == 0) sPreW[0] = 0;
        for (int base = 0; base < nCh; base += 64) {
          const int ch = base + tid;
          uint32_t x = (ch < nCh && sChPlus[ch] == (uint8_t)winPlus) ? sPre[ch + 1] - sPre[ch] : 0u;
#pragma unroll
          for (int o = 1; o < 64; o <<= 1) { const uint32_t y = __shfl_up(x, o, 64); if (tid >= o) x += y; }
          if (ch < nCh) sPreW[ch + 1] = carry + x;
          carry += __shfl(x, 63, 64);
        }
      }
      __syncthreads();
      const uint32_t nWin = sPreW[nCh];
      uint32_t written = 0;
      for (uint32_t i0 = 0; i0 < nWin; i0 += WG) {
        const uint32_t q = i0 + tid;
        uint32_t ridx = 0, g = 0;
        if (q < nWin) {
          int lo = 0, hi = nCh;
          while (hi - lo > 1) { const int mid = (lo + hi) >> 1; if (sPreW[mid] <= q) lo = mid; else hi = mid; }
          ridx = sPre[lo] + (q - sPreW[lo]);
          g = sCs[lo] + (q - sPreW[lo]);
        }
        const bool look = q < nWin && (ridx >= KEEP_BITS || ((sKeepBits[ridx >> 5] >> (ridx & 31)) & 1u));
        uint4 hd = make_uint4(0u, 0u, 0u, 0u), cw = make_uint4(0u, 0u, 0u, 0u);
        if (look) { const uint32_t *rec = P.recs + (uint64_t)g * stride; hd = ((const uint4 *)rec)[0]; cw = ((const uint4 *)rec)[1]; }
        const bool pend = look && recPending(hd.z);
        const uint32_t nc = look ? (pend ? 1u : ((hd.z & REC_DONE) ? (hd.z & 0x3FFFFFFFu) : 0u)) : 0;
        const uint32_t w2own = pend ? pendingMatchWord(P, re, hd.z, cw.y, cw.z, cw.w) : cw.y;
        uint32_t keepMask = 0, nk = 0;
        for (uint32_t j = 0; j < nc; ++j) {
          uint32_t w0 = hd.w, w1 = cw.x, w2 = w2own;
          if (hd.z & 0x40000000u) { const uint32_t *gc = P.genCand + ((uint64_t)hd.w + j) * 6; w0 = gc[0]; w1 = gc[1]; w2 = gc[2]; }
          if (keepCandidate<MAXLEN>(P, sBaseCnt, (int)winPlus, w0, w1, w2)) { keepMask |= 1u << j; ++nk; }
        }
        uint32_t tot;
        uint32_t off = t1k_block_scan_exclusive(nk, warpSums, &tot);
        for (uint32_t j = 0; j < nc; ++j) {
          if (!((keepMask >> j) & 1u)) continue;
          uint32_t w0 = hd.w, w1 = cw.x, w2 = w2own;
          if (hd.z & 0x40000000u) { const uint32_t *gc = P.genCand + ((uint64_t)hd.w + j) * 6; w0 = gc[0]; w1 = gc[1]; w2 = gc[2]; }
          T1kCand cd;
          cd.allele = hd.y | (winPlus ? 0x80000000u : 0);
          cd.readSE = (w0 & 0xFFF) | (((w0 >> 12) & 0xFFF) << 16);
          cd.seqStart = (int)(w1 & 0xFFFFF); cd.seqEnd = (int)(w2 & 0xFFFFF);
          cd.match = (w1 >> 20) | ((w2 >> 20) << 16);
          cd.re = re;
          P.cand[(uint64_t)sBase + written + off] = cd;
          ++off;
        }
        written += tot;
      }
    }
    __syncthreads();
  }
}

size_t t1k_chain_big_scratch_u32() { return (size_t)4 * BIG_CAP + GA_SCRATCH_INTS; }
int t1k_chain_max_chunks(uint32_t nAlleles) { return 2 * (int)((nAlleles + CHUNK_A - 1) / CHUNK_A) + 2; }
int t1k_chain_memo_entries() { return GAP_CACHE; }
int t1k_chain_rec_stride(int maxLen) { return maxLen <= 160 ? 8 : 16; }
int t1k_chain_max_kmers(int maxLen, int k) { return (2 * std::max(1, maxLen - k + 1) + 3) / 4 * 4; }
int t1k_chain_used_u32(int maxK) { return maxK * 4; }

static int readCounters(t1k_ctx *ctx, unsigned long long *h) { return t1k_fetch_counters(ctx, h); }

template <class V>
__global__ __launch_bounds__(WG) void k_arena_compact(const V *src, uint32_t segCap, unsigned long long *counters, int arena, V *dst, unsigned long long overflowFlag) {
  const unsigned long long *cursors = counters + T1K_ARENA_BASE + (size_t)arena * T1K_NSTRIPE * T1K_STRIPE_WORDS;
  const uint32_t seg = blockIdx.y;
  uint32_t prefix = 0;
  for (uint32_t s = 0; s < seg; ++s) prefix += (uint32_t)min(cursors[s * T1K_STRIPE_WORDS], (unsigned long long)segCap);
  const uint32_t cnt = (uint32_t)min(cursors[seg * T1K_STRIPE_WORDS], (unsigned long long)segCap);
  if (blockIdx.x == 0 && seg == T1K_NSTRIPE - 1 && threadIdx.x == 0) {
    counters[T1K_TOTAL_BASE + arena] = (unsigned long long)prefix + cnt;
    bool over = false;
    for (uint32_t s = 0; s < T1K_NSTRIPE; ++s) over = over || cursors[s * T1K_STRIPE_WORDS] > (unsigned long long)segCap;
    if (over && overflowFlag) atomicOr(&counters[2], overflowFlag);
  }
  for (uint32_t i = blockIdx.x * WG + threadIdx.x; i < cnt; i += gridDim.x * WG) dst[prefix + i] = src[(uint64_t)seg * segCap + i];
}

T1kArenaCounts t1k_arena_counts(const t1k_ctx *ctx, int arena, uint32_t segCap) {
  T1kArenaCounts r{0, 0, false};
  for (int s = 0; s < T1K_NSTRIPE; ++s) {
    unsigned long long c = ctx->hRaw[T1K_ARENA_BASE + ((size_t)arena * T1K_NSTRIPE + s) * T1K_STRIPE_WORDS];
    if (c > segCap) { r.overflow = true; c = segCap; }
    r.total += c;
    r.maxSeg = std::max<uint32_t>(r.maxSeg, (uint32_t)c);
  }
  return r;
}

void t1k_arena_compact(t1k_ctx *ctx, int arena, const uint32_t *src, uint32_t segCap, uint32_t *dst, uint32_t maxSeg) {
  if (!maxSeg) return;
  hipLaunchKernelGGL(k_arena_compact<uint32_t>, dim3(std::min<uint32_t>((maxSeg + WG - 1) / WG, 256u), T1K_NSTRIPE), dim3(WG), 0, ctx->stream, src, segCap,
                     (unsigned long long *)ctx->bCounters.p, arena, dst, 0ull);
}
void t1k_arena_compact64(t1k_ctx *ctx, int arena, const unsigned long long *src, uint32_t segCap, unsigned long long *dst, uint32_t maxSeg) {
  if (!maxSeg) return;
  hipLaunchKernelGGL(k_arena_compact<unsigned long long>, dim3(std::min<uint32_t>((maxSeg + WG - 1) / WG, 256u), T1K_NSTRIPE), dim3(WG), 0, ctx->stream, src, segCap,
                     (unsigned long long *)ctx->bCounters.p, arena, dst, 0ull);
}
void t1k_arena_compact_dev(t1k_ctx *ctx, int arena, const uint32_t *src, uint32_t segCap, uint32_t *dst, uint64_t estTotal) {
  const uint32_t perSeg = (uint32_t)std::min<uint64_t>(segCap, estTotal / T1K_NSTRIPE * 2 + WG);
  hipLaunchKernelGGL(k_arena_compact<uint32_t>, dim3(std::max(1u, std::min<uint32_t>((perSeg + WG - 1) / WG, 256u)), T1K_NSTRIPE), dim3(WG), 0, ctx->stream, src, segCap,
                     (unsigned long long *)ctx->bCounters.p, arena, dst, (unsigned long long)ERR_GROUPCAP);
}

__global__ __launch_bounds__(WG) void k_job_keys(const unsigned long long *memo, const uint32_t *jobs, unsigned long long *keys, uint32_t n) {
  const uint32_t q = blockIdx.x * blockDim.x + threadIdx.x;
  if (q < n) keys[q] = (memo[jobs[q]] >> 5) & 0x1FF;
}
__global__ __launch_bounds__(WG) void k_group_size_keys(const uint32_t *recs, uint32_t stride, const uint32_t *list, unsigned long long *keys, uint32_t n, int useSimple) {
  const uint32_t q = blockIdx.x * blockDim.x + threadIdx.x;
  if (q < n) {
    const uint32_t *r = recs + (uint64_t)list[q] * stride;
    const bool simple = useSimple && r[5] == REC_NEAR_DONE && r[6] == 1u;
    keys[q] = simple ? min(r[4], 127u) : 128u + min(r[4], 63u);
  }
}
#define CS_BINS 512
#define CS_TILE (WG * 8)
struct JobLenKey {
  const unsigned long long *memo;
  __device__ __forceinline__ uint32_t operator()(uint32_t item) const { return (uint32_t)((memo[item] >> 5) & 0x1FF); }
};
struct GroupSizeKey {
  const uint32_t *recs; uint32_t stride; int useSimple;
  __device__ __forceinline__ uint32_t operator()(uint32_t item) const {
    const uint32_t *r = recs + (uint64_t)item * stride;
    const bool simple = useSimple && r[5] == REC_NEAR_DONE && r[6] == 1u;
    return simple ? min(r[4], 127u) : 128u + min(r[4], 63u);
  }
};
template <class KeyFn>
__global__ __launch_bounds__(WG) void k_csort_count(const uint32_t *list, uint32_t n, uint32_t *scratch, KeyFn key, const unsigned long long *nDev) {
  __shared__ uint32_t h[CS_BINS];
  if (nDev) n = (uint32_t)*nDev;
  for (int b = threadIdx.x; b < CS_BINS; b += WG) h[b] = 0;
  __syncthreads();
  for (uint32_t i = blockIdx.x * WG + threadIdx.x; i < n; i += gridDim.x * WG) atomicAdd(&h[key(list[i])], 1u);
  __syncthreads();
  for (int b = threadIdx.x; b < CS_BINS; b += WG)
    if (h[b]) atomicAdd(&scratch[b], h[b]);
}
template <class KeyFn>
__global__ __launch_bounds__(WG) void k_csort_scatter(const uint32_t *list, uint32_t n, uint32_t *scratch, uint32_t *out, KeyFn key, const unsigned long long *nDev) {
  __shared__ uint32_t base[CS_BINS], h[CS_BINS], off[CS_BINS], warpSums[4];
  __shared__ uint32_t sLast;
  if (nDev) n = (uint32_t)*nDev;
  uint32_t *hist = scratch, *cursor = scratch + CS_BINS, *ticket = scratch + 2 * CS_BINS;
  {
    const uint32_t a = hist[2 * threadIdx.x], b = hist[2 * threadIdx.x + 1];
    uint32_t tot;
    const uint32_t ex = t1k_block_scan_exclusive(a + b, warpSums, &tot);
    base[2 * threadIdx.x] = ex; base[2 * threadIdx.x + 1] = ex + a;
  }
  for (uint32_t t0 = blockIdx.x * CS_TILE; t0 < n; t0 += gridDim.x * CS_TILE) {
    for (int b = threadIdx.x; b < CS_BINS; b += WG) h[b] = 0;
    __syncthreads();
    uint32_t item[8], kk[8], rk[8];
#pragma unroll
    for (int j = 0; j < 8; ++j) {
      const uint32_t i = t0 + j * WG + threadIdx.x;
      kk[j] = 0xFFFFFFFFu;
      if (i < n) { item[j] = list[i]; kk[j] = key(item[j]); rk[j] = atomicAdd(&h[kk[j]], 1u); }
    }
    __syncthreads();
    for (int b = threadIdx.x; b < CS_BINS; b += WG)
      if (h[b]) off[b] = base[b] + atomicAdd(&cursor[b], h[b]);
    __syncthreads();
#pragma unroll
    for (int j = 0; j < 8; ++j)
      if (kk[j] != 0xFFFFFFFFu) { const uint32_t pos = off[kk[j]] + rk[j]; if (pos < n) out[pos] = item[j]; }
    __syncthreads();
  }
  __threadfence();
  if (threadIdx.x == 0) sLast = atomicAdd(ticket, 1u) == gridDim.x - 1 ? 1u : 0u;
  __syncthreads();
  if (sLast) {
    for (int b = threadIdx.x; b < 2 * CS_BINS; b += WG) scratch[b] = 0;
    if (threadIdx.x == 0) *ticket = 0;
  }
}
template <class KeyFn>
static const uint32_t *countingSort(t1k_ctx *ctx, const uint32_t *list, uint32_t n, KeyFn key, const unsigned long long *nDev = nullptr, uint64_t nEst = 0) {
  static_assert(CS_BINS == 2 * WG, "two bins per thread in the prefix");
  const size_t head = (2 * CS_BINS + 16) * 4;
  const bool fresh = ctx->bJobSort.bytes < head + (size_t)n * 4;
  if (t1k_ensure(ctx, ctx->bJobSort, head + (size_t)n * 4) != T1K_OK) return list;
  uint32_t *scratch = (uint32_t *)ctx->bJobSort.p, *sorted = scratch + 2 * CS_BINS + 16;
  if (fresh && hipMemsetAsync(scratch, 0, head, ctx->stream) != hipSuccess) return list;
  const uint64_t forGrid = nDev ? std::min<uint64_t>(n, nEst) : n;
  const uint32_t grid = (uint32_t)std::max<uint64_t>(1, std::min<uint64_t>((forGrid + CS_TILE - 1) / CS_TILE, 1024u));
  hipLaunchKernelGGL(k_csort_count<KeyFn>, dim3(grid), dim3(WG), 0, ctx->stream, list, n, scratch, key, nDev);
  hipLaunchKernelGGL(k_csort_scatter<KeyFn>, dim3(grid), dim3(WG), 0, ctx->stream, list, n, scratch, sorted, key, nDev);
  return sorted;
}
void t1k_launch_dp_dense(t1k_ctx *ctx, const ChainArgs &a, const uint32_t *jobs, uint32_t n) {
  if (!n) return;
  static const bool radix = getenv("T1K_RADIX_SORTS") != nullptr;
  if (n >= 4096 && !radix) jobs = countingSort(ctx, jobs, n, JobLenKey{(const unsigned long long *)a.memo});
  else if (n >= 4096 && t1k_ensure(ctx, ctx->bSlowKeys, (size_t)n * 20 + 64) == T1K_OK) {
    unsigned long long *k0 = (unsigned long long *)ctx->bSlowKeys.p, *k1 = k0 + n;
    uint32_t *sorted = (uint32_t *)(k1 + n);
    hipLaunchKernelGGL(k_job_keys, dim3((n + WG - 1) / WG), dim3(WG), 0, ctx->stream, (const unsigned long long *)a.memo, jobs, k0, n);
    if (t1k_sort_pairs(ctx, k0, k1, jobs, sorted, n, 9) == T1K_OK) jobs = sorted;
  }
  hipLaunchKernelGGL(k_dp_dense, dim3((n + WG - 1) / WG), dim3(WG), 0, ctx->stream, a, jobs, n, (const unsigned long long *)nullptr);
}
void t1k_launch_dp_dense_dev(t1k_ctx *ctx, const ChainArgs &a, const uint32_t *jobs, int arena, uint32_t cap, uint64_t est) {
  const unsigned long long *nDev = (const unsigned long long *)ctx->bCounters.p + T1K_TOTAL_BASE + arena;
  jobs = countingSort(ctx, jobs, cap, JobLenKey{(const unsigned long long *)a.memo}, nDev, est);
  const uint32_t grid = (uint32_t)std::max<uint64_t>(1, (std::min<uint64_t>(cap, est) + WG - 1) / WG);
  hipLaunchKernelGGL(k_dp_dense, dim3(grid), dim3(WG), 0, ctx->stream, a, jobs, cap, nDev);
}

uint64_t t1k_arena_estimate(const t1k_ctx *ctx, int arena, uint64_t cap, uint32_t nRe) {
  if (!ctx->estValid || !ctx->estTotal[arena]) return cap;
  return std::min<uint64_t>(cap, (ctx->estTotal[arena] * std::max(1u, nRe) >> 16) * 5 / 4 + 4096);
}
void t1k_arena_estimate_set(t1k_ctx *ctx, int arena, uint64_t total, uint32_t nRe) { ctx->estTotal[arena] = (total << 16) / std::max(1u, nRe) + 1; }
bool t1k_chain_host_driven() { static const bool h = getenv("T1K_HOST_CHAIN") != nullptr; return h; }
static int runChainDevice(t1k_ctx *ctx, const ChainArgs &aIn, int nWg, int bigBlocks, bool longReads, bool xlong, unsigned long long *hc) {
  ChainArgs a = aIn;
  a.devDriven = 1;
  const unsigned long long *tot = (const unsigned long long *)ctx->bCounters.p + T1K_TOTAL_BASE;
  const uint32_t nRe = std::max<uint32_t>(1u, a.reads.nReadEnds);
  auto est = [&](int arena, uint64_t cap) -> uint64_t { return t1k_arena_estimate(ctx, arena, cap, nRe); };
  auto blocks = [](uint64_t items, uint32_t per) { return (uint32_t)std::max<uint64_t>(1, (items + per - 1) / per); };
  const uint64_t listCap = (uint64_t)a.listSegCap * T1K_NSTRIPE, rareCap = (uint64_t)a.rareSegCap * T1K_NSTRIPE, jobCap = (uint64_t)a.jobSegCap * T1K_NSTRIPE,
                 genJobCap = (uint64_t)a.genJobSegCap * T1K_NSTRIPE, groupCap = (uint64_t)a.groupSegCap * T1K_NSTRIPE;
  {
    const dim3 grid(blocks(a.groupSegCap, WG), T1K_NSTRIPE);
    (void)groupCap;
    if (longReads) hipLaunchKernelGGL((k_chain_fast<10, 0, false>), grid, dim3(WG), 0, ctx->stream, a, (const uint32_t *)nullptr, 0u, tot);
    else hipLaunchKernelGGL((k_chain_fast<5, 0, false>), grid, dim3(WG), 0, ctx->stream, a, (const uint32_t *)nullptr, 0u, tot);
  }
  {
    const uint64_t e = est(T1K_AR_SLOW, listCap);
    t1k_arena_compact_dev(ctx, T1K_AR_SLOW, a.slowStr, a.listSegCap, a.slowList, e);
    if (longReads) hipLaunchKernelGGL((k_chain_fast<10, 1, true>), dim3(blocks(e, WG)), dim3(WG), 0, ctx->stream, a, (const uint32_t *)a.slowList, 0u, tot + T1K_AR_SLOW);
    else hipLaunchKernelGGL((k_chain_fast<5, 1, true>), dim3(blocks(e, WG)), dim3(WG), 0, ctx->stream, a, (const uint32_t *)a.slowList, 0u, tot + T1K_AR_SLOW);
  }
  const uint64_t eJobs = est(T1K_AR_JOBS, jobCap), eRetry = est(T1K_AR_RETRY, listCap), eGen = est(T1K_AR_GENERAL, rareCap);
  t1k_arena_compact_dev(ctx, T1K_AR_JOBS, a.jobStr, a.jobSegCap, a.jobList, eJobs);
  t1k_arena_compact_dev(ctx, T1K_AR_RETRY, a.retryStr, a.listSegCap, a.retryList, eRetry);
  t1k_arena_compact_dev(ctx, T1K_AR_GENERAL, a.generalStr, a.rareSegCap, a.generalList, eGen);
  t1k_launch_dp_dense_dev(ctx, a, a.jobList, T1K_AR_JOBS, (uint32_t)jobCap, eJobs);
  if (longReads) hipLaunchKernelGGL((k_chain_fast<10, 2, true>), dim3(blocks(eRetry, WG)), dim3(WG), 0, ctx->stream, a, (const uint32_t *)a.retryList, 0u, tot + T1K_AR_RETRY);
  else hipLaunchKernelGGL((k_chain_fast<5, 2, true>), dim3(blocks(eRetry, WG)), dim3(WG), 0, ctx->stream, a, (const uint32_t *)a.retryList, 0u, tot + T1K_AR_RETRY);
  {
    static const bool nearHits = getenv("T1K_NO_NEAR_HITS") == nullptr;
    const int skipDone = nearHits && !xlong ? 1 : 0;
    const unsigned long long *nGen = tot + T1K_AR_GENERAL;
    if (skipDone) {
      if (longReads) hipLaunchKernelGGL(k_near_hits<10>, dim3(blocks(eGen, WG)), dim3(WG), 0, ctx->stream, a, 0u, nGen);
      else hipLaunchKernelGGL(k_near_hits<5>, dim3(blocks(eGen, WG)), dim3(WG), 0, ctx->stream, a, 0u, nGen);
    }
    const uint32_t gatherGrid = std::min<uint32_t>(blocks(eGen, 4), 8192u);
    if (xlong) hipLaunchKernelGGL(k_gather_general<(T1K_LONG_READ_LEN + 63) / 64>, dim3(gatherGrid), dim3(WG), 0, ctx->stream, a, 0u, skipDone, nGen);
    else hipLaunchKernelGGL(k_gather_general<GROUP_FAST_MAXLEN / 64>, dim3(gatherGrid), dim3(WG), 0, ctx->stream, a, 0u, skipDone, nGen);
    ChainArgs g = a;
    g.generalList = (uint32_t *)countingSort(ctx, a.generalList, (uint32_t)rareCap, GroupSizeKey{(const uint32_t *)a.recs, a.recStride, skipDone}, nGen, eGen);
    hipLaunchKernelGGL(k_chain_general, dim3(blocks(eGen, 64)), dim3(64), 0, ctx->stream, g, 0u, skipDone, nGen);
    const uint64_t eWave = est(T1K_AR_WAVE, rareCap);
    t1k_arena_compact_dev(ctx, T1K_AR_WAVE, a.waveStr, a.rareSegCap, a.waveList, eWave);
    T1K_HIP(ctx, hipFuncSetAttribute((const void *)k_chain_wave, hipFuncAttributeMaxDynamicSharedMemorySize, 3 * WAVE_CAP * 4));
    {
      const uint32_t wgrid = (uint32_t)std::max<uint64_t>(1, std::min<uint64_t>(eWave, 2048u));
      static const uint32_t smallCap = getenv("T1K_WAVE_SMALL") ? (uint32_t)atoi(getenv("T1K_WAVE_SMALL")) : 512u;
      if (smallCap) hipLaunchKernelGGL(k_chain_wave, dim3(wgrid), dim3(64), 3 * smallCap * 4, ctx->stream, a, 0u, tot + T1K_AR_WAVE, smallCap, 0u);
      hipLaunchKernelGGL(k_chain_wave, dim3(wgrid), dim3(64), 3 * WAVE_CAP * 4, ctx->stream, a, 0u, tot + T1K_AR_WAVE, (uint32_t)WAVE_CAP, smallCap);
    }
    const uint64_t eGenJobs = est(T1K_AR_GENJOBS, genJobCap);
    t1k_arena_compact_dev(ctx, T1K_AR_GENJOBS, a.genJobStr, a.genJobSegCap, a.genJobList, eGenJobs);
    t1k_launch_dp_dense_dev(ctx, a, a.genJobList, T1K_AR_GENJOBS, (uint32_t)genJobCap, eGenJobs);
    hipLaunchKernelGGL(k_general_finish, dim3(blocks(eGen, WG)), dim3(WG), 0, ctx->stream, a, 0u, nGen);
    t1k_arena_compact_dev(ctx, T1K_AR_BIG, a.bigStr, a.rareSegCap, a.bigList, est(T1K_AR_BIG, rareCap));
    hipLaunchKernelGGL(k_chain_big, dim3(bigBlocks * 64), dim3(64), 0, ctx->stream, a, 0u, tot + T1K_AR_BIG);
  }
  if (xlong) hipLaunchKernelGGL(k_collect<T1K_LONG_READ_LEN>, dim3(nWg), dim3(WG), 0, ctx->stream, a);
  else hipLaunchKernelGGL(k_collect<T1K_MAX_READ_LEN>, dim3(nWg), dim3(WG), 0, ctx->stream, a);
  T1K_HIP(ctx, hipEventRecord(ctx->ev[1], ctx->stream));
  const int rc = readCounters(ctx, hc);
  if (rc) return rc;
  const T1kArenaCounts groups = t1k_arena_counts(ctx, T1K_AR_GROUPS, a.groupSegCap), slow = t1k_arena_counts(ctx, T1K_AR_SLOW, a.listSegCap), jobs = t1k_arena_counts(ctx, T1K_AR_JOBS, a.jobSegCap),
                       retry = t1k_arena_counts(ctx, T1K_AR_RETRY, a.listSegCap), fin = t1k_arena_counts(ctx, T1K_AR_FINISH, a.listSegCap), gen = t1k_arena_counts(ctx, T1K_AR_GENERAL, a.rareSegCap),
                       wv = t1k_arena_counts(ctx, T1K_AR_WAVE, a.rareSegCap), gj = t1k_arena_counts(ctx, T1K_AR_GENJOBS, a.genJobSegCap), big = t1k_arena_counts(ctx, T1K_AR_BIG, a.rareSegCap);
  if (groups.overflow || slow.overflow || jobs.overflow || retry.overflow || gen.overflow || wv.overflow || gj.overflow || big.overflow) hc[2] |= ERR_GROUPCAP;
  if (hc[2] & ERR_GROUPCAP) hc[2] &= ~(unsigned long long)ERR_MEMO;
  ctx->lastSlowGroups = slow.total;
  hc[16] = jobs.total; hc[17] = retry.total; hc[18] = gen.total; hc[19] = big.total; hc[22] = fin.total;
  if (!hc[2]) {
    const T1kArenaCounts *cs[] = {&groups, &slow, &jobs, &retry, &gen, &wv, &gj, &big};
    const int ar[] = {T1K_AR_GROUPS, T1K_AR_SLOW, T1K_AR_JOBS, T1K_AR_RETRY, T1K_AR_GENERAL, T1K_AR_WAVE, T1K_AR_GENJOBS, T1K_AR_BIG};
    for (int i = 0; i < 8; ++i) t1k_arena_estimate_set(ctx, ar[i], cs[i]->total, nRe);
    ctx->estValid = true;
  }
  return 0;
}

int t1k_run_chain(t1k_ctx *ctx, const ChainArgs &a, int nWg, int bigBlocks, bool longReads, unsigned long long *hc) {
  const int AW = longReads ? 13 : 7;
  const size_t maxK = a.maxKFast;
  const bool xlong = a.maxK > a.maxKFast;
  size_t lds = (size_t)CHUNK_A * AW * 4 + maxK * (5 * 4 + (T1K_SEED_PACK_Q ? 0 : 2)) + 4 + (T1K_SEED_PACK_Q ? 8 : 64);
  const size_t bitmapWords = 2 * (((size_t)a.ref.nAlleles + 31) / 32);
  if (bitmapWords > (size_t)CHUNK_A * AW) lds += bitmapWords * 4 + 8;
  if (a.ref.kDirStride - 1 > 256) return t1k_fail(ctx, T1K_ERR_ARG, "the reference holds more than 131 072 distinct sequences (256 seeding chunks)");
  if (lds > 160 * 1024) return t1k_fail(ctx, T1K_ERR_ARG, "the reference holds too many sequences for the seeding kernel's LDS bitmaps");
  const char *esw = getenv("T1K_SEED_WG");
  const int seedWg = (int)std::min<uint32_t>(a.reads.nReadEnds, esw ? (uint32_t)atoi(esw) : 32768u);
  T1K_HIP(ctx, hipEventRecord(ctx->ev[0], ctx->stream));
  if (a.fuse) {
    if (longReads) {
      T1K_HIP(ctx, hipFuncSetAttribute((const void *)k_seed_chain<10>, hipFuncAttributeMaxDynamicSharedMemorySize, (int)lds));
      hipLaunchKernelGGL(k_seed_chain<10>, dim3(seedWg), dim3(WG), lds, ctx->stream, a);
    } else {
      T1K_HIP(ctx, hipFuncSetAttribute((const void *)k_seed_chain<5>, hipFuncAttributeMaxDynamicSharedMemorySize, (int)lds));
      hipLaunchKernelGGL(k_seed_chain<5>, dim3(seedWg), dim3(WG), lds, ctx->stream, a);
    }
  } else if (longReads) {
    T1K_HIP(ctx, hipFuncSetAttribute((const void *)k_seed_groups<10>, hipFuncAttributeMaxDynamicSharedMemorySize, (int)lds));
    hipLaunchKernelGGL(k_seed_groups<10>, dim3(seedWg), dim3(WG), lds, ctx->stream, a);
  } else {
    T1K_HIP(ctx, hipFuncSetAttribute((const void *)k_seed_groups<5>, hipFuncAttributeMaxDynamicSharedMemorySize, (int)lds));
    hipLaunchKernelGGL(k_seed_groups<5>, dim3(seedWg), dim3(WG), lds, ctx->stream, a);
  }
  if (xlong) {
    const size_t ldsLong = (size_t)a.maxK * (4 * 4 + 2) + 8 + (size_t)LONG_CH * 4;
    T1K_HIP(ctx, hipFuncSetAttribute((const void *)k_seed_long, hipFuncAttributeMaxDynamicSharedMemorySize, (int)ldsLong));
    hipLaunchKernelGGL(k_seed_long, dim3(std::min<uint32_t>(a.reads.nReadEnds, 32768u)), dim3(WG), ldsLong, ctx->stream, a);
  }
  T1K_HIP(ctx, hipEventRecord(ctx->ev[8], ctx->stream));
  if (!t1k_chain_host_driven() && !a.fuse) return runChainDevice(ctx, a, nWg, bigBlocks, longReads, xlong, hc);
  const unsigned long long *NODEV = nullptr;
  int rc = readCounters(ctx, hc);
  if (rc) return rc;
  if (hc[2]) return 0;
  const T1kArenaCounts groups = t1k_arena_counts(ctx, T1K_AR_GROUPS, a.groupSegCap);
  const unsigned long long groupsSeeded = hc[6];
  if (!a.fuse) {
    if (groups.maxSeg) {
      const dim3 grid((groups.maxSeg + WG - 1) / WG, T1K_NSTRIPE);
      if (longReads) hipLaunchKernelGGL((k_chain_fast<10, 0, false>), grid, dim3(WG), 0, ctx->stream, a, (const uint32_t *)nullptr, 0u, NODEV);
      else hipLaunchKernelGGL((k_chain_fast<5, 0, false>), grid, dim3(WG), 0, ctx->stream, a, (const uint32_t *)nullptr, 0u, NODEV);
    }
    if ((rc = readCounters(ctx, hc))) return rc;
  }
  const T1kArenaCounts slow = t1k_arena_counts(ctx, T1K_AR_SLOW, a.listSegCap);
  if (slow.overflow) { hc[2] |= ERR_GROUPCAP; return 0; }
  ctx->lastSlowGroups = slow.total;
  if (slow.total) {
    t1k_arena_compact(ctx, T1K_AR_SLOW, a.slowStr, a.listSegCap, a.slowList, slow.maxSeg);
    const uint32_t nSlowGroups = (uint32_t)slow.total;
    if (longReads) hipLaunchKernelGGL((k_chain_fast<10, 1, false>), dim3((nSlowGroups + WG - 1) / WG), dim3(WG), 0, ctx->stream, a, (const uint32_t *)a.slowList, nSlowGroups, NODEV);
    else hipLaunchKernelGGL((k_chain_fast<5, 1, false>), dim3((nSlowGroups + WG - 1) / WG), dim3(WG), 0, ctx->stream, a, (const uint32_t *)a.slowList, nSlowGroups, NODEV);
  }
  if ((rc = readCounters(ctx, hc))) return rc;
  hc[6] = groupsSeeded;
  const T1kArenaCounts jobs = t1k_arena_counts(ctx, T1K_AR_JOBS, a.jobSegCap), retry = t1k_arena_counts(ctx, T1K_AR_RETRY, a.listSegCap),
                       fin = t1k_arena_counts(ctx, T1K_AR_FINISH, a.listSegCap), gen = t1k_arena_counts(ctx, T1K_AR_GENERAL, a.rareSegCap);
  if (retry.overflow || fin.overflow || gen.overflow || jobs.overflow) { hc[2] |= ERR_GROUPCAP; return 0; }
  hc[16] = jobs.total; hc[17] = retry.total; hc[18] = gen.total; hc[22] = fin.total;
  t1k_arena_compact(ctx, T1K_AR_JOBS, a.jobStr, a.jobSegCap, a.jobList, jobs.maxSeg);
  t1k_arena_compact(ctx, T1K_AR_FINISH, a.finishStr, a.listSegCap, a.finishList, fin.maxSeg);
  t1k_arena_compact(ctx, T1K_AR_RETRY, a.retryStr, a.listSegCap, a.retryList, retry.maxSeg);
  t1k_arena_compact(ctx, T1K_AR_GENERAL, a.generalStr, a.rareSegCap, a.generalList, gen.maxSeg);
  const uint32_t nJobs = (uint32_t)jobs.total, nRetry = (uint32_t)retry.total, nGen = (uint32_t)gen.total, nFinish = (uint32_t)fin.total;
  t1k_launch_dp_dense(ctx, a, a.jobList, nJobs);
  static const bool finishKernel = getenv("T1K_FINISH_KERNEL") != nullptr;
  if (nFinish && finishKernel) hipLaunchKernelGGL(k_chain_finish, dim3((nFinish + WG - 1) / WG), dim3(WG), 0, ctx->stream, a, nFinish);
  if (nRetry) {
    if (longReads) hipLaunchKernelGGL((k_chain_fast<10, 2, false>), dim3((nRetry + WG - 1) / WG), dim3(WG), 0, ctx->stream, a, (const uint32_t *)a.retryList, nRetry, NODEV);
    else hipLaunchKernelGGL((k_chain_fast<5, 2, false>), dim3((nRetry + WG - 1) / WG), dim3(WG), 0, ctx->stream, a, (const uint32_t *)a.retryList, nRetry, NODEV);
  }
  uint32_t nBig = 0;
  if (nGen) {
    static const bool nearHits = getenv("T1K_NO_NEAR_HITS") == nullptr;
    const int skipDone = nearHits && !xlong ? 1 : 0;
    if (skipDone) {
      if (longReads) hipLaunchKernelGGL(k_near_hits<10>, dim3((nGen + WG - 1) / WG), dim3(WG), 0, ctx->stream, a, nGen, NODEV);
      else hipLaunchKernelGGL(k_near_hits<5>, dim3((nGen + WG - 1) / WG), dim3(WG), 0, ctx->stream, a, nGen, NODEV);
    }
    if (xlong) hipLaunchKernelGGL(k_gather_general<(T1K_LONG_READ_LEN + 63) / 64>, dim3(std::min<uint32_t>((nGen + 3) / 4, 8192u)), dim3(WG), 0, ctx->stream, a, nGen, skipDone, NODEV);
    else hipLaunchKernelGGL(k_gather_general<GROUP_FAST_MAXLEN / 64>, dim3(std::min<uint32_t>((nGen + 3) / 4, 8192u)), dim3(WG), 0, ctx->stream, a, nGen, skipDone, NODEV);
    ChainArgs g = a;
    static const bool radix = getenv("T1K_RADIX_SORTS") != nullptr;
    if (nGen >= 4096 && !radix)
      g.generalList = (uint32_t *)countingSort(ctx, a.generalList, nGen, GroupSizeKey{(const uint32_t *)a.recs, a.recStride, skipDone});
    else if (nGen >= 4096 && t1k_ensure(ctx, ctx->bSlowKeys, (size_t)nGen * 20 + 64) == T1K_OK) {
      unsigned long long *k0 = (unsigned long long *)ctx->bSlowKeys.p, *k1 = k0 + nGen;
      uint32_t *sorted = (uint32_t *)(k1 + nGen);
      hipLaunchKernelGGL(k_group_size_keys, dim3((nGen + WG - 1) / WG), dim3(WG), 0, ctx->stream, (const uint32_t *)a.recs, a.recStride, (const uint32_t *)a.generalList, k0, nGen, skipDone);
      if (t1k_sort_pairs(ctx, k0, k1, a.generalList, sorted, nGen, 8) == T1K_OK) g.generalList = sorted;
    }
    hipLaunchKernelGGL(k_chain_general, dim3((nGen + 63) / 64), dim3(64), 0, ctx->stream, g, nGen, skipDone, NODEV);
    if ((rc = readCounters(ctx, hc))) return rc;
    const T1kArenaCounts wv = t1k_arena_counts(ctx, T1K_AR_WAVE, a.rareSegCap);
    if (wv.overflow) { hc[2] |= ERR_GROUPCAP; return 0; }
    if (wv.total) {
      t1k_arena_compact(ctx, T1K_AR_WAVE, a.waveStr, a.rareSegCap, a.waveList, wv.maxSeg);
      T1K_HIP(ctx, hipFuncSetAttribute((const void *)k_chain_wave, hipFuncAttributeMaxDynamicSharedMemorySize, 3 * WAVE_CAP * 4));
      hipLaunchKernelGGL(k_chain_wave, dim3(std::min<uint32_t>((uint32_t)wv.total, 2048u)), dim3(64), 3 * WAVE_CAP * 4, ctx->stream, a, (uint32_t)wv.total, NODEV, (uint32_t)WAVE_CAP, 0u);
    }
    if ((rc = readCounters(ctx, hc))) return rc;
    const T1kArenaCounts gj = t1k_arena_counts(ctx, T1K_AR_GENJOBS, a.genJobSegCap);
    if (gj.overflow) { hc[2] |= ERR_GROUPCAP; return 0; }
    t1k_arena_compact(ctx, T1K_AR_GENJOBS, a.genJobStr, a.genJobSegCap, a.genJobList, gj.maxSeg);
    t1k_launch_dp_dense(ctx, a, a.genJobList, (uint32_t)gj.total);
    hipLaunchKernelGGL(k_general_finish, dim3((nGen + WG - 1) / WG), dim3(WG), 0, ctx->stream, a, nGen, NODEV);
    const T1kArenaCounts big = t1k_arena_counts(ctx, T1K_AR_BIG, a.rareSegCap);
    if (big.overflow) { hc[2] |= ERR_GROUPCAP; return 0; }
    t1k_arena_compact(ctx, T1K_AR_BIG, a.bigStr, a.rareSegCap, a.bigList, big.maxSeg);
    nBig = (uint32_t)big.total;
  }
  if (nBig) hipLaunchKernelGGL(k_chain_big, dim3(bigBlocks * 64), dim3(64), 0, ctx->stream, a, nBig, NODEV);
  if (xlong) hipLaunchKernelGGL(k_collect<T1K_LONG_READ_LEN>, dim3(nWg), dim3(WG), 0, ctx->stream, a);
  else hipLaunchKernelGGL(k_collect<T1K_MAX_READ_LEN>, dim3(nWg), dim3(WG), 0, ctx->stream, a);
  T1K_HIP(ctx, hipEventRecord(ctx->ev[1], ctx->stream));
  rc = readCounters(ctx, hc);
  hc[6] = groupsSeeded; hc[16] = jobs.total; hc[17] = retry.total; hc[18] = gen.total; hc[19] = nBig; hc[22] = fin.total;
  return rc;
}
```

### t1k_amd/csrc/t1k_dev.h

```cpp
#pragma once
#include <hip/hip_runtime.h>
#include <stdint.h>
#include <string>
#include <type_traits>
#include <vector>
#include "../../include/t1k_gpu.h"

#define T1K_MAX_READ_LEN 320
#define T1K_LONG_READ_LEN 1000
#define T1K_EVEN 0x5555555555555555ull
#define T1K_NEG_BIG (-(1 << 28))

struct T1kPosting { uint32_t allele, offset; };

struct T1kCand {
  uint32_t allele;
  uint32_t readSE;
  int32_t seqStart, seqEnd;
  uint32_t match;
  uint32_t re;
};

struct T1kExt {
  int32_t seqStart, seqEnd;
// ... 373 lines not shown
  return t1k_ga_matches_equal(T, P, L, nullptr);
#endif
}

__device__ inline int t1k_ga_general(const T1kSeqView &T, int lent, const T1kSeqView &P, int lenp, int *scratch, uint8_t *trace, int *nMatch) {
  if (lent == 0 || lenp == 0) { if (nMatch) *nMatch = 0; return 0; }
  if (lent == 1 && lenp == 1) {
    bool eq = t1k_eq(T.code(0), P.code(0));
    if (nMatch) *nMatch = eq ? 1 : 0;
    if (trace) { trace[0] = 0; trace[1 * 2 + 1] = (uint8_t)(1 | (eq ? 16 : 0)); }
    return eq ? 2 : -2;
  }
  int leftBand = 5, rightBand = 5;
  if (lent > lenp) rightBand += lent - lenp; else if (lent < lenp) leftBand += lenp - lent;
  const int W = lent + 1;
  const int negInf = (lent + 1) * (lenp + 1) * -4;
  int *m = scratch, *e = scratch + (W + 1), *f = scratch + 2 * (W + 1);
  int *cm = scratch + 3 * (W + 1), *ce = scratch + 4 * (W + 1), *cf = scratch + 5 * (W + 1);
  m[0] = e[0] = f[0] = 0; cm[0] = ce[0] = cf[0] = 0;
  for (int j = 1; j <= lent; ++j) { f[j] = -4 - j; e[j] = -4 - 4 * (lenp + 1); m[j] = -4 - 4 * j; cm[j] = ce[j] = cf[j] = 0; }
  if (trace) {
    for (int j = 0; j <= lent; ++j) {
      uint8_t t = 0;
      if (j > 0) {
        if (f[j] >= e[j]) t |= 2;
        int mprev = (j - 1 == 0) ? 0 : -4 - 4 * (j - 1);
        if (mprev - 5 == f[j]) t |= 8;
      }
      trace[j] = t;
    }
  }
  for (int i = 1; i <= lenp; ++i) {
    int start = (i - leftBand < 1) ? 1 : (i - leftBand);
    int end = (i + rightBand > lent) ? lent : (i + rightBand);
    int pc = P.code(i - 1);
    int mDiag, cmDiag;
    int mL, fL, cmL, cfL;
    if (start == 1) {
      mDiag = (i - 1 == 0) ? 0 : -4 - 4 * (i - 1);
      cmDiag = 0;
      mL = -4 - 4 * i; fL = -4 - 4 * i; cmL = 0; cfL = 0;
    } else {
      mDiag = m[start - 1]; cmDiag = cm[start - 1];
      mL = negInf; fL = negInf; cmL = 0; cfL = 0;
    }
    int saveM0 = m[0], saveE0 = e[0];
    (void)saveM0; (void)saveE0;
    if (start == 1) {  }
    for (int j = start; j <= end; ++j) {
      int eu = e[j] - 1, mu = m[j] - 5;
      int ne = eu > mu ? eu : mu;
      int nce = (mu == ne) ? cm[j] : ce[j];
      int fl = fL - 1, ml = mL - 5;
      int nf = fl > ml ? fl : ml;
      int ncf = (ml == nf) ? cmL : cfL;
      bool eq = t1k_eq(T.code(j - 1), pc);
      int dg = mDiag + (eq ? 2 : -2);
      int nm = dg;
      if (ne > nm) nm = ne;
      if (nf > nm) nm = nf;
      int ncm;
      if (dg == nm) ncm = cmDiag + (eq ? 1 : 0);
      else if (nf >= ne) ncm = ncf;
      else ncm = nce;
      if (trace) {
        uint8_t t = 0;
        if (dg == nm) t |= 1;
        if (nf >= ne) t |= 2;
        if (mu == ne) t |= 4;
        if (ml == nf) t |= 8;
        if (eq) t |= 16;
        trace[i * W + j] = t;
      }
      mDiag = m[j]; cmDiag = cm[j];
      m[j] = nm; e[j] = ne; f[j] = nf; cm[j] = ncm; ce[j] = nce; cf[j] = ncf;
      mL = nm; fL = nf; cmL = ncm; cfL = ncf;
    }
    if (end < lent) { m[end + 1] = e[end + 1] = f[end + 1] = negInf; cm[end + 1] = ce[end + 1] = cf[end + 1] = 0; }
    if (start > 1) { m[start - 1] = e[start - 1] = f[start - 1] = negInf; cm[start - 1] = ce[start - 1] = cf[start - 1] = 0; }
    m[0] = -4 - 4 * i; e[0] = -4 - i; f[0] = -4 - 4 * i; cm[0] = ce[0] = cf[0] = 0;
    if (trace) {
      uint8_t t = 0;
      if (f[0] >= e[0]) t |= 2;
      int mprev = (i - 1 == 0) ? 0 : -4 - 4 * (i - 1);
      if (mprev - 5 == e[0]) t |= 4;
      trace[i * W] = t;
    }
  }
  if (nMatch) *nMatch = cm[lent];
  return m[lent];
}

__device__ inline int t1k_ga_traceback(const uint8_t *trace, int lent, int lenp, int8_t *ops) {
  if (lent == 0 || lenp == 0) return 0;
  const int W = lent + 1;
  int ti = lenp, tj = lent, mat = 0, n = 0;
  if (lent == 1 && lenp == 1) { ops[0] = (trace[1 * 2 + 1] & 16) ? 0 : 1; return 1; }
  while (ti > 0 || tj > 0) {
    uint8_t t = trace[ti * W + tj];
    if (mat == 0) {
      if (ti > 0 && tj > 0 && (t & 1)) { ops[n++] = (t & 16) ? 0 : 1; --ti; --tj; }
      else if (t & 2) mat = 2;
      else mat = 1;
    } else if (mat == 1) {
      ops[n++] = 2;
      if (ti > 0) { if (t & 4) mat = 0; --ti; }
      else mat = 2;
    } else {
      ops[n++] = 3;
      if (tj > 0) { if (t & 8) mat = 0; --tj; }
      else mat = 1;
    }
  }
  for (int a = 0, b = n - 1; a < b; ++a, --b) { int8_t x = ops[a]; ops[a] = ops[b]; ops[b] = x; }
  return n;
}

#define T1K_STAT_STRIPES 256
enum { T1K_STAT_DP = 0, T1K_STAT_FAST = 1, T1K_STAT_GENERAL = 2, T1K_STAT_EXTEND_DP = 3, T1K_STAT_NEARBEST = 4, T1K_STAT_LOOKUPS = 5, T1K_STAT_POSTINGS = 6, T1K_STAT_HITS = 7 };
#ifndef T1K_OCC8
#define T1K_OCC8 __attribute__((amdgpu_waves_per_eu(8)))
#endif
#define T1K_WAVES_ATTR_(n) __attribute__((amdgpu_waves_per_eu(n)))
#ifndef T1K_COLLECT_HANDOUT
#define T1K_COLLECT_HANDOUT 1
#endif
#ifndef T1K_SELECT_SMALL_HANDOUT
#define T1K_SELECT_SMALL_HANDOUT 2
#endif
#ifndef T1K_SELECT_LARGE_HANDOUT
#define T1K_SELECT_LARGE_HANDOUT 1
#endif
#ifndef T1K_TRUNC_SMALL_HANDOUT
#define T1K_TRUNC_SMALL_HANDOUT 4
#endif
#ifndef T1K_TRUNC_LARGE_HANDOUT
#define T1K_TRUNC_LARGE_HANDOUT 1
#endif
#ifndef T1K_COLLECT_WAVES
#define T1K_COLLECT_WAVES 0
#endif
#ifndef T1K_EXTEND_WAVES
#define T1K_EXTEND_WAVES 0
#endif
#ifndef T1K_CF0_WAVES
#define T1K_CF0_WAVES 0
#endif
#ifndef T1K_TRUNC_SMALL_WAVES
#define T1K_TRUNC_SMALL_WAVES 0
#endif
#ifndef T1K_TRUNC_LARGE_WAVES
#define T1K_TRUNC_LARGE_WAVES 0
#endif
#define T1K_NSTRIPE 32
enum { T1K_AR_GROUPS = 0, T1K_AR_JOBS, T1K_AR_RETRY, T1K_AR_FINISH, T1K_AR_GENERAL, T1K_AR_BIG, T1K_AR_GENCAND, T1K_AR_EQ, T1K_AR_BAND, T1K_AR_WIDE, T1K_AR_GENHITS, T1K_AR_GENJOBS, T1K_AR_WAVE, T1K_AR_EXTJOBS, T1K_AR_EXTRETRY, T1K_AR_SLOW, T1K_NARENA };
#define T1K_ARENA_BASE (64 + T1K_STAT_STRIPES * 8)
#ifndef T1K_STRIPE_WORDS
#define T1K_STRIPE_WORDS 8
#endif
#define T1K_TOTAL_BASE (T1K_ARENA_BASE + T1K_NARENA * T1K_NSTRIPE * T1K_STRIPE_WORDS)
#define T1K_COUNTER_WORDS (T1K_TOTAL_BASE + ((T1K_NARENA + 7) & ~7))
#define T1K_ARENA_FULL 0xFFFFFFFFu
__device__ __forceinline__ unsigned long long *t1k_arena_cursor(unsigned long long *counters, int arena, uint32_t stripe) {
  return counters + T1K_ARENA_BASE + ((uint32_t)arena * T1K_NSTRIPE + stripe) * T1K_STRIPE_WORDS;
}
__device__ __forceinline__ uint32_t t1k_arena_alloc(unsigned long long *counters, int arena, uint32_t n, uint32_t segCap) {
  const uint32_t stripe = blockIdx.x & (T1K_NSTRIPE - 1);
  const unsigned long long off = atomicAdd(t1k_arena_cursor(counters, arena, stripe), (unsigned long long)n);
  return off + n <= segCap ? stripe * segCap + (uint32_t)off : T1K_ARENA_FULL;
}
__device__ __forceinline__ uint32_t t1k_arena_append(unsigned long long *counters, int arena, uint32_t segCap) {
  const uint64_t m = __ballot(1);
  const int lane = threadIdx.x & 63;
  const uint32_t stripe = blockIdx.x & (T1K_NSTRIPE - 1);
  uint32_t base = 0;
  if (lane == __ffsll((long long)m) - 1) {
    const unsigned long long off = atomicAdd(t1k_arena_cursor(counters, arena, stripe), (unsigned long long)__popcll(m));
    base = off > 0xFFFFFFFFull ? 0xFFFFFFFFu : (uint32_t)off;
  }
  base = (uint32_t)__builtin_amdgcn_readfirstlane((int)base);
  const uint64_t off = (uint64_t)base + (uint32_t)__popcll(m & ((1ull << lane) - 1));
  return off < segCap ? stripe * segCap + (uint32_t)off : T1K_ARENA_FULL;
}
__device__ __forceinline__ void t1k_stat_add(unsigned long long *counters, int kind, unsigned int v) {
#pragma unroll
  for (int o = 32; o > 0; o >>= 1) v += __shfl_down(v, o, 64);
  if ((threadIdx.x & 63) == 0 && v) {
    const unsigned int stripe = (blockIdx.x * (blockDim.x >> 6) + (threadIdx.x >> 6)) & (T1K_STAT_STRIPES - 1);
    atomicAdd(&counters[64 + stripe * 8 + kind], (unsigned long long)v);
  }
}

__device__ __forceinline__ void t1k_lds_barrier() { asm volatile("s_waitcnt lgkmcnt(0)\n\ts_barrier" ::: "memory"); }

template <int NWAVES, bool LDS_ONLY = false>
__device__ __forceinline__ uint32_t t1k_block_scan_exclusive_n(uint32_t v, uint32_t *warpSums, uint32_t *total) {
  int lane = threadIdx.x & 63, wave = threadIdx.x >> 6;
  uint32_t x = v;
#pragma unroll
  for (int o = 1; o < 64; o <<= 1) {
    uint32_t y = __shfl_up(x, o, 64);
    if (lane >= o) x += y;
  }
  if (lane == 63) warpSums[wave] = x;
  if (LDS_ONLY) t1k_lds_barrier(); else __syncthreads();
  uint32_t base = 0, tot = 0;
#pragma unroll
  for (int w = 0; w < NWAVES; ++w) { const uint32_t s = warpSums[w]; if (w < wave) base += s; tot += s; }
  if (LDS_ONLY) t1k_lds_barrier(); else __syncthreads();
  *total = tot;
  return base + x - v;
}
__device__ __forceinline__ uint32_t t1k_block_scan_exclusive(uint32_t v, uint32_t *warpSums, uint32_t *total) {
  return t1k_block_scan_exclusive_n<4>(v, warpSums, total);
}

struct T1kDevBuf {
  void *p = nullptr;
  size_t bytes = 0;
};

struct t1k_ctx {
  int device = 0;
  std::vector<unsigned long long> hRaw;
  hipStream_t stream = nullptr;
  hipEvent_t ev[12] = {};
  t1k_params prm;
  std::string err;
  T1kRefDev ref{};
  std::vector<uint64_t> hAlleleOff;
  std::vector<uint32_t> hAlleleLen;
  std::vector<T1kDevBuf> refBufs;
  T1kReadsDev reads{};
  T1kDevBuf bReadAscii, bReadOffs, bReadBases, bReadN, bReadLen, bReadWeight, bListPtr, bListCount;
  T1kDevBuf bDedupScratch, bDedupBases, bDedupN, bDedupLen, bDedupWeight;
  bool readsShared = false;
  int batchMaxLen = 0;
  int batchFastMaxLen = 0;
  int covFullLen = 0;
  bool covFullDirty = false;
  uint32_t rangeCount = 0;
  T1kDevBuf bWgHits, bWgGroups, bWgStage, bWgBig, bWgCache, bLists;
  std::vector<T1kDevBuf> storeChunks[2];
  int storeSlot = 0;
  size_t storeChunk[2] = {0, 0};
  uint64_t storeUsed[2] = {0, 0};
  T1kOvl *ovlBase = nullptr;
  T1kDevBuf bOvlWork;
  T1kOvlP *storeBase = nullptr;
  uint64_t wGroup = 0, wList = 0, wRare = 0, wCand = 0, wOvl = 0, wJob = 0, wGenJob = 0, wGenHit = 0;
  uint64_t needGroup = 0, needList = 0, needRare = 0, needCand = 0, needOvl = 0, needJob = 0, needGenJob = 0, needGenHit = 0;
  unsigned long long lastCapFlags = 0;
  bool scaledOnce = false;
  bool covCommitted = false;
  uint32_t queueBoost = 1;
  int covMode = 0;
  double msAlloc = 0;
  uint64_t bytesAlloc = 0;
  T1kDevBuf bCand, bExt, bCandStart, bCandCount, bOvlStart, bOvlCount, bCounters, bSlowQueue, bSlowScratch, bSortScratch, bEqTrace, bSortTmp, bSlowKeys, bJobSort;
  uint64_t nCand = 0, nOvl = 0;
  T1kDevBuf bEnd1, bEnd2, bHasN, bRows, bRowStart, bRowCount, bFragAssigned, bPairScratch, bPairOverflow, bPairBig, bExtractHuge;
  uint32_t nFragments = 0;
  uint64_t nRows = 0;
  T1kDevBuf bEmRowPtr, bEmEc, bEmCount, bEmLen, bEmX0, bEmN, bEmPsum, bEmColPtr, bEmRowOf;
  std::vector<uint64_t> emPieceBytes, emPieceDispl;
  uint32_t emGroups = 0, emEc = 0, emRowBegin = 0, emRowEnd = 0;
  struct t1k_comm *emComm = nullptr;
  bool emReduceMode = false;
  uint64_t emNnz = 0;
  std::vector<int32_t> hEmLen;
  int traceFetch = 0;
  uint32_t upN = 0; int upS = 0, upMaxLen = 0; uint64_t upBytes = 0; bool upOpen = false;
  hipEvent_t upEv[4] = {nullptr, nullptr, nullptr, nullptr}; bool upEvSet[4] = {false, false, false, false};
  uint64_t lastSlowGroups = 0;
  uint64_t estTotal[T1K_NARENA] = {};
  bool estValid = false;
  uint64_t pairEpoch = 0;
  uint64_t pairBigCap = 0;
  unsigned long long *countersPinned = nullptr;
  double *emPinned = nullptr;
  size_t emPinnedN = 0;
  double emMs[4] = {0, 0, 0, 0};
  t1k_allreduce_fn emAllreduce = nullptr;
  void *emUser = nullptr;
  T1kDevBuf bAlign[12];
  T1kDevBuf bExtract;
  t1k_stats stats{};
};

hipError_t t1k_dev_malloc(void **out, size_t bytes);
hipError_t t1k_dev_free(void *p);
uint64_t t1k_pool_cached_bytes(int device);
int t1k_fail(t1k_ctx *ctx, int code, const std::string &msg);
int t1k_ensure(t1k_ctx *ctx, T1kDevBuf &b, size_t bytes);
#define T1K_HIP(ctx, call)                                                                              \
  do {                                                                                                  \
    hipError_t e_ = (call);                                                                             \
    if (e_ != hipSuccess) return t1k_fail(ctx, T1K_ERR_DEVICE, std::string(#call) + ": " + hipGetErrorString(e_)); \
  } while (0)
```

Baseline: 3.653 million.

## Split general chaining into per-thread simple kernel and team-cooperative kernel

Replaces the single per-thread k_chain_general kernel with two kernels. k_chain_simple handles small single-chain groups with one output slot and defers inline DP to the wave queue. k_chain_team has 16-lane teams process each general group cooperatively, using rank-based sorting and run bounds in shared memory. The counting sort now exports bin boundaries so the team kernel only scans the relevant range of the sorted list. This aims to cut per-thread serial work and divergence on larger groups, at the cost of an extra launch, new path-count atomics, and more complex code.

```diff
diff --git a/include/t1k_gpu.h b/include/t1k_gpu.h
--- a/include/t1k_gpu.h
+++ b/include/t1k_gpu.h
@@ -168,6 +168,7 @@
   double ms_load, ms_device, ms_coalesce, ms_write;
 } t1k_stats;
 int t1k_stats_get(t1k_ctx *ctx, t1k_stats *out);
+int t1k_chain_path_counts(t1k_ctx *ctx, uint64_t out[6]);
 double t1k_alloc_ms(t1k_ctx *ctx, uint64_t *bytes);
 uint64_t t1k_ctx_mem_report(t1k_ctx *ctx, const char *tag, int print);
 
diff --git a/t1k_amd/capi.py b/t1k_amd/capi.py
--- a/t1k_amd/capi.py
+++ b/t1k_amd/capi.py
@@ -91,6 +91,8 @@
     L.t1k_extract_batch.argtypes = [vp, C.c_uint32, vp, vp]
     L.t1k_extractor_main.argtypes = [C.c_int, C.POINTER(C.c_char_p)]
     L.t1k_stats_get.argtypes = [vp, C.POINTER(Stats)]
+    if hasattr(L, "t1k_chain_path_counts"):
+        L.t1k_chain_path_counts.argtypes = [vp, u64p]
     L.t1k_genotyper_main.argtypes = [C.c_int, C.POINTER(C.c_char_p)]
     L.t1k_job_params_default.argtypes = [C.POINTER(JobParams)]
     L.t1k_job_create.argtypes = [C.POINTER(JobParams), C.c_char_p, C.POINTER(vp)]
@@ -295,6 +297,11 @@
         lib().t1k_stats_get(self.h, C.byref(s))
         return s.as_dict()
 
+    def chain_path_counts(self):
+        out = (C.c_uint64 * 6)()
+        self._check(lib().t1k_chain_path_counts(self.h, out), "t1k_chain_path_counts")
+        return dict(zip(("chains_short", "chains_long", "team_low", "team_high", "wave", "big"), (int(v) for v in out)))
+
     def align_batch(self, texts, pats, want_ops=True):
         n = len(texts)
         tb, toff = _concat(texts)
diff --git a/t1k_amd/csrc/t1k_capi.hip b/t1k_amd/csrc/t1k_capi.hip
--- a/t1k_amd/csrc/t1k_capi.hip
+++ b/t1k_amd/csrc/t1k_capi.hip
@@ -972,6 +972,8 @@
     fprintf(stderr, "[t1k] gap walk classes: exact without a DP %llu, pruned by the per-gap bound %llu, memo / DP %llu\n", hc[40], hc[41], hc[42]);
 #endif
   }
+  for (int i = 0; i < 5; ++i) ctx->pathCounts[i] += hc[T1K_PATH_BASE + i];
+  ctx->pathCounts[5] += hc[13];
   t1k_stats &st = ctx->stats;
   st.read_ends = n; st.lookups = hc[3]; st.postings = hc[4]; st.hits = hc[5]; st.groups = hc[6]; st.candidates = hc[0]; st.extended = hc[1];
   st.dp_calls = hc[7] + hc[14]; st.near_best = hc[10]; st.dp_cells = hc[24];
@@ -1021,6 +1023,12 @@
   return ctx->msAlloc;
 }
 
+int t1k_chain_path_counts(t1k_ctx *ctx, uint64_t *out) {
+  if (!ctx || !out) return T1K_ERR_ARG;
+  for (int i = 0; i < 6; ++i) out[i] = ctx->pathCounts[i];
+  return T1K_OK;
+}
+
 int t1k_stats_get(t1k_ctx *ctx, t1k_stats *out) {
   if (!ctx || !out) return T1K_ERR_ARG;
   *out = ctx->stats;
diff --git a/t1k_amd/csrc/t1k_chain.hip b/t1k_amd/csrc/t1k_chain.hip
--- a/t1k_amd/csrc/t1k_chain.hip
+++ b/t1k_amd/csrc/t1k_chain.hip
@@ -6,7 +6,6 @@
 
 #define WG 256
 #define GROUP_FAST_MAXLEN 320
-#define GENERAL_CAP 128
 #define BIG_CAP 16384
 #define GA_BIG_MAX 2048
 #define GA_SCRATCH_INTS (6 * (GA_BIG_MAX + 4))
@@ -31,6 +30,22 @@
     if (overflow || stride != 6 || n == 0) return;
     uint32_t *d = dst + 6 * (n - 1);
     d[0] |= (uint32_t)nref << 24; d[3] = refs[0]; d[4] = refs[1]; d[5] = refs[2];
+  }
+};
+
+struct CandOne {
+  uint32_t w[6];
+  int n = 0;
+  bool overflow = false;
+  __device__ void push(int rs, int re, int ss, int se, int m0, int m) {
+    if (n >= 1) { overflow = true; return; }
+    w[0] = (uint32_t)rs | ((uint32_t)re << 12); w[1] = (uint32_t)ss | ((uint32_t)m0 << 20); w[2] = (uint32_t)se | ((uint32_t)m << 20);
+    w[3] = w[4] = w[5] = 0;
+    n = 1;
+  }
+  __device__ void setRefs(const uint32_t *refs, int nref) {
+    if (overflow || n == 0) return;
+    w[0] |= (uint32_t)nref << 24; w[3] = refs[0]; w[4] = refs[1]; w[5] = refs[2];
   }
 };
 
@@ -306,22 +321,29 @@
   return result;
 }
 
-template <class Arr>
-__device__ inline void chainRun(const ReadCtx &c, int k, int hitLenRequired, Arr A, Arr B, Arr C, int s, int m, int *gaScratch, int gaMax, CandOut &out,
-                                unsigned int *dpCounter, unsigned long long *errFlags, bool *needScratch, const GapSink *sink, int strandBit, bool chainReady = false) {
+template <bool INLINE_DP = true, class Arr, class Out>
+__device__ inline void chainRun(const ReadCtx &c, int k, int hitLenRequired, Arr A, Arr B, Arr C, int s, int m, int *gaScratch, int gaMax, Out &out,
+                                unsigned int *dpCounter, unsigned long long *errFlags, bool *needScratch, const GapSink *sink, int strandBit, bool chainReady = false,
+                                bool *needInline = nullptr) {
     int ret, lenR, lenS;
     if (!t1k_run_lis(A, B, C, s, m, k, hitLenRequired, &ret, &lenR, &lenS, chainReady)) return;
     uint32_t refs[3] = {0, 0, 0};
     int nref = 0;
     auto gapM = [&](int ra, int ga, int lp, int lt) -> int {
-      if (!sink) return gapMatches(c, ra, ga, lp, lt, gaScratch, gaMax, dpCounter, errFlags, needScratch);
+      if (INLINE_DP && !sink) return gapMatches(c, ra, ga, lp, lt, gaScratch, gaMax, dpCounter, errFlags, needScratch);
       if (lp <= 0 || lt <= 0) return 0;
       const int diff = lt > lp ? lt - lp : lp - lt;
       if (diff > 4) { *needScratch = true; return 0; }
       uint32_t slot = 0;
       const int r = gapMatchesCached<true>(c, ra, c.goff + ga, lp, lt, strandBit, *sink, dpCounter, &slot);
       if (r >= 0) return r;
-      if (r == -1 && nref < GROUP_MAX_REFS) { refs[nref >> 1] |= slot << (16 * (nref & 1)); ++nref; return 0; }
+      if (r == -1 && nref < GROUP_MAX_REFS) {
+        const uint32_t v = slot << (16 * (nref & 1));
+        if ((nref >> 1) == 0) refs[0] |= v; else refs[1] |= v;
+        ++nref;
+        return 0;
+      }
+      if (!INLINE_DP) { *needInline = true; return 0; }
       if (dpCounter) ++*dpCounter;
       return gapAlign(c, ra, c.goff + ga, lp, lt);
     };
@@ -346,9 +368,9 @@
     out.setRefs(refs, nref);
 }
 
-template <class Arr>
+template <class Arr, class Out>
 __device__ inline void groupGeneral(const uint32_t *h, int n, const ReadCtx &c, int k, int radius, int hitLenRequired, Arr A, Arr B,
-                                     Arr C, int *gaScratch, int gaMax, CandOut &out, unsigned int *dpCounter, unsigned long long *errFlags, bool *needScratch,
+                                     Arr C, int *gaScratch, int gaMax, Out &out, unsigned int *dpCounter, unsigned long long *errFlags, bool *needScratch,
                                      const GapSink *sink = nullptr, int strandBit = 0) {
   for (int i = 0; i < n; ++i) {
     uint32_t x = h[i];
@@ -395,12 +417,61 @@
   }
 }
 
-template <class Arr>
-__device__ inline void groupSimple(const uint32_t *h, int n, const ReadCtx &c, int k, int hitLenRequired, Arr A, CandOut &out, unsigned int *dpCounter,
-                                   unsigned long long *errFlags, bool *needScratch, const GapSink *sink, int strandBit) {
+template <bool INLINE_DP = true, class Arr, class Out>
+__device__ inline void groupSimple(const uint32_t *h, int n, const ReadCtx &c, int k, int hitLenRequired, Arr A, Out &out, unsigned int *dpCounter,
+                                   unsigned long long *errFlags, bool *needScratch, const GapSink *sink, int strandBit, bool *needInline = nullptr) {
   for (int i = 0; i < n; ++i) A[i] = h[i];
   if (n < 3 || n * k < hitLenRequired) return;
-  chainRun(c, k, hitLenRequired, A, A, A, 0, n, nullptr, 0, out, dpCounter, errFlags, needScratch, sink, strandBit, true);
+  chainRun<INLINE_DP>(c, k, hitLenRequired, A, A, A, 0, n, nullptr, 0, out, dpCounter, errFlags, needScratch, sink, strandBit, true, needInline);
+}
+
+__device__ __forceinline__ int t1kHitDiag(uint32_t x) { return (int)(x & 0xFFF) - (int)(x >> 12); }
+template <class Arr>
+__device__ __forceinline__ int teamRankByKey(Arr C, int n, int i) {
+  const uint32_t x = C[i];
+  int r = 0;
+  for (int j = 0; j < n; ++j) { const uint32_t y = C[j]; r += (hitKeyLess(y, x) || (y == x && j < i)) ? 1 : 0; }
+  return r;
+}
+template <class Arr>
+__device__ __forceinline__ void teamRunBounds(Arr A, int s, int n, int radius, int *eOut, int *dominantOut) {
+  int curDiff = t1kHitDiag(A[s]), curCnt = 1, domCnt = 0, dominant = 0, prev = curDiff;
+  int e = s + 1;
+  for (; e < n; ++e) {
+    const int de = t1kHitDiag(A[e]);
+    int d = de - prev;
+    if (d < 0) d = -d;
+    if (d > radius) break;
+    if (d == 0) ++curCnt;
+    else {
+      if (curCnt > domCnt) { dominant = curDiff; domCnt = curCnt; }
+      curDiff = de; curCnt = 1;
+    }
+    prev = de;
+  }
+  if (curCnt > domCnt) dominant = curDiff;
+  *eOut = e; *dominantOut = dominant;
+}
+template <class Arr>
+__device__ __forceinline__ bool teamKeep(Arr A, int s, int e, int dominant, int q) {
+  const uint32_t x = A[q];
+  const int a = (int)(x & 0xFFF);
+  int dq = t1kHitDiag(x) - dominant; if (dq < 0) dq = -dq;
+  bool keep = true;
+  for (int r = s; r < e; ++r) {
+    const uint32_t y = A[r];
+    if ((int)(y & 0xFFF) != a) continue;
+    int dr = t1kHitDiag(y) - dominant; if (dr < 0) dr = -dr;
+    if (dr < dq) keep = false;
+  }
+  return keep;
+}
+template <class Arr>
+__device__ __forceinline__ int teamRankKept(Arr A, Arr C, int s, int e, int q) {
+  const uint32_t x = A[q];
+  int r = 0;
+  for (int t = s; t < e; ++t) { const uint32_t y = A[t]; r += (C[t] && (y < x || (y == x && t < q))) ? 1 : 0; }
+  return r;
 }
 
 struct VoteKey {
@@ -1433,51 +1504,166 @@
   }
 }
 
-__global__ __launch_bounds__(64) void k_chain_general(ChainArgs P, uint32_t nItems, int useSimple, const unsigned long long *nDev) {
-  __shared__ uint32_t sArr[3 * GENERAL_SMALL * 64];
+__device__ __forceinline__ void t1k_path_add(unsigned long long *counters, int which, unsigned int v) {
+#pragma unroll
+  for (int o = 32; o > 0; o >>= 1) v += __shfl_down(v, o, 64);
+  if ((threadIdx.x & 63) == 0 && v) atomicAdd(&counters[T1K_PATH_BASE + which], (unsigned long long)v);
+}
+template <class Src>
+__device__ __forceinline__ void closeGeneralGroup(const ChainArgs &P, uint32_t *rec, int nc, Src src) {
+  uint32_t base = 0;
+  if (nc) {
+    base = t1k_arena_alloc(P.counters, T1K_AR_GENCAND, (uint32_t)nc, P.genCandSegCap);
+    if (base == T1K_ARENA_FULL) { atomicOr(&P.counters[2], (unsigned long long)ERR_STAGECAP); nc = 0; base = 0; }
+    for (int i = 0; i < 6 * nc; ++i) P.genCand[(uint64_t)base * 6 + i] = src[i];
+  }
+  rec[3] = base;
+  rec[2] = REC_DONE | 0x40000000u | (uint32_t)nc;
+}
+
+__global__ __launch_bounds__(64) void k_chain_simple(ChainArgs P, uint32_t nItems, const unsigned long long *nDev, const unsigned long long *bnd) {
+  __shared__ uint32_t sArr[GENERAL_SMALL * 64];
   if (nDev) { if (P.counters[2]) return; nItems = (uint32_t)*nDev; }
+  if (bnd) nItems = min(nItems, (uint32_t)bnd[0]);
   unsigned int dpLocal = 0, genLocal = 0;
   for (uint32_t qb = blockIdx.x * 64; qb < nItems; qb += gridDim.x * 64) {
-  const uint32_t q = qb + threadIdx.x;
-  uint32_t nHits = 0xFFFFFFFFu;
-  bool simple = false;
-  if (q < nItems) {
-    const uint32_t *r0 = P.recs + (uint64_t)P.generalList[q] * P.recStride;
-    nHits = r0[4];
-    simple = useSimple && r0[5] == REC_NEAR_DONE && r0[6] == 1u;
-  }
-  if (nHits <= GENERAL_SMALL || (simple && nHits <= 3 * GENERAL_SMALL)) {
+    const uint32_t q = qb + threadIdx.x;
+    if (q >= nItems) continue;
     const uint32_t gi = P.generalList[q];
     uint32_t *rec = P.recs + (uint64_t)gi * P.recStride;
-    const uint32_t re = rec[0] & 0x7FFFFFFFu, allele = rec[1];
-    const int pass = (rec[0] >> 31) ? 0 : 1;
-    ReadCtx c = makeCtx(P, re, pass, allele);
-    const int n = (int)nHits;
-    if (rec[3] == T1K_ARENA_FULL) atomicOr(&P.counters[2], (unsigned long long)ERR_STAGECAP);
-    const uint32_t *hh = P.genHits + (rec[3] == T1K_ARENA_FULL ? 0u : rec[3]);
-    bool needScratch = false;
-    uint32_t cbuf[2 * GENERAL_SMALL + 6];
-    CandOut out{cbuf, 0, 6, GENERAL_SMALL / 3 + 1};
+    const uint4 r0 = *(const uint4 *)rec, r1 = *(const uint4 *)(rec + 4);
+    const uint32_t nHits = r1.x;
+    if (!(r1.y == REC_NEAR_DONE && r1.z == 1u && nHits <= GENERAL_SMALL)) continue;
+    const uint32_t re = r0.x & 0x7FFFFFFFu, allele = r0.y;
+    const int pass = (r0.x >> 31) ? 0 : 1;
+    const ReadCtx c = makeCtx(P, re, pass, allele);
+    if (r0.w == T1K_ARENA_FULL) atomicOr(&P.counters[2], (unsigned long long)ERR_STAGECAP);
+    const uint32_t *hh = P.genHits + (r0.w == T1K_ARENA_FULL ? 0u : r0.w);
+    bool needScratch = false, needInline = false;
+    CandOne out;
     const GapSink sink{P.memo + (uint64_t)re * GAP_CACHE, P.genJobStr, P.counters, re * GAP_CACHE, P.genJobSegCap, T1K_AR_GENJOBS};
-    LaneArr A{sArr + threadIdx.x}, B{sArr + GENERAL_SMALL * 64 + threadIdx.x}, C{sArr + 2 * GENERAL_SMALL * 64 + threadIdx.x};
-    if (simple) groupSimple(hh, n, c, P.k, P.hitLenRequired, A, out, &dpLocal, &P.counters[2], &needScratch, &sink, pass);
-    else groupGeneral(hh, n, c, P.k, P.radius, P.hitLenRequired, A, B, C, nullptr, 0, out, &dpLocal, &P.counters[2], &needScratch, &sink, pass);
+    const LaneArr A{sArr + threadIdx.x};
+    groupSimple<false>(hh, (int)nHits, c, P.k, P.hitLenRequired, A, out, &dpLocal, &P.counters[2], &needScratch, &sink, pass, &needInline);
     if (needScratch) { const uint32_t b = t1k_arena_append(P.counters, T1K_AR_BIG, P.rareSegCap); if (b != T1K_ARENA_FULL) P.bigStr[b] = gi; }
+    else if (needInline) { const uint32_t wq = t1k_arena_append(P.counters, T1K_AR_WAVE, P.rareSegCap); if (wq != T1K_ARENA_FULL) P.waveStr[wq] = gi; }
     else {
       ++genLocal;
       uint32_t base = 0;
-      if (out.n) {
-        base = t1k_arena_alloc(P.counters, T1K_AR_GENCAND, (uint32_t)out.n, P.genCandSegCap);
-        if (base == T1K_ARENA_FULL) { atomicOr(&P.counters[2], (unsigned long long)ERR_STAGECAP); out.n = 0; base = 0; }
-        for (int i = 0; i < 6 * out.n; ++i) P.genCand[(uint64_t)base * 6 + i] = cbuf[i];
+      int nc = out.n;
+      if (nc) {
+        base = t1k_arena_alloc(P.counters, T1K_AR_GENCAND, 1u, P.genCandSegCap);
+        if (base == T1K_ARENA_FULL) { atomicOr(&P.counters[2], (unsigned long long)ERR_STAGECAP); nc = 0; base = 0; }
+        else {
+          uint32_t *g = P.genCand + (uint64_t)base * 6;
+#pragma unroll
+          for (int i = 0; i < 6; ++i) g[i] = out.w[i];
+        }
       }
       rec[3] = base;
-      rec[2] = REC_DONE | 0x40000000u | (uint32_t)out.n;
-    }
-  }
+      rec[2] = REC_DONE | 0x40000000u | (uint32_t)nc;
+    }
   }
   t1k_stat_add(P.counters, T1K_STAT_DP, dpLocal);
   t1k_stat_add(P.counters, T1K_STAT_GENERAL, genLocal);
+  t1k_path_add(P.counters, 0, genLocal);
+}
+
+__device__ __forceinline__ void teamSync() {
+  __builtin_amdgcn_fence(__ATOMIC_RELEASE, "wavefront");
+  __builtin_amdgcn_wave_barrier();
+  __builtin_amdgcn_fence(__ATOMIC_ACQUIRE, "wavefront");
+}
+#define TEAM_CAND_CAP (GENERAL_SMALL / 3 + 1)
+template <int TEAM>
+__global__ __launch_bounds__(64) void k_chain_team(ChainArgs P, uint32_t nItems, int useSimple, const unsigned long long *nDev, const unsigned long long *bnd) {
+  constexpr int NT = 64 / TEAM, HP = GENERAL_SMALL / TEAM;
+  static_assert(TEAM * NT == 64 && HP * TEAM == GENERAL_SMALL, "team width");
+  __shared__ uint32_t sArr[NT * 3 * GENERAL_SMALL], sCand[NT * 6 * TEAM_CAND_CAP];
+  if (nDev) { if (P.counters[2]) return; nItems = (uint32_t)*nDev; }
+  uint32_t first = 0;
+  if (bnd) { first = min(nItems, (uint32_t)bnd[0]); nItems = min(nItems, (uint32_t)bnd[1]); }
+  const int team = threadIdx.x / TEAM, tl = threadIdx.x % TEAM;
+  uint32_t *A = sArr + team * 3 * GENERAL_SMALL, *B = A + GENERAL_SMALL, *C = B + GENERAL_SMALL, *cbuf = sCand + team * 6 * TEAM_CAND_CAP;
+  unsigned int dpLocal = 0, genLocal = 0, nLong = 0, nLow = 0, nHigh = 0;
+  const int k = P.k;
+  for (uint32_t qb = first + blockIdx.x * NT; qb < nItems; qb += gridDim.x * NT) {
+    const uint32_t q = qb + team;
+    int kind = 0;
+    uint32_t gi = 0, nHits = 0;
+    uint4 r0 = make_uint4(0u, 0u, 0u, 0u);
+    uint32_t *rec = P.recs;
+    if (q < nItems) {
+      gi = P.generalList[q];
+      rec = P.recs + (uint64_t)gi * P.recStride;
+      r0 = *(const uint4 *)rec;
+      const uint4 r1 = *(const uint4 *)(rec + 4);
+      nHits = r1.x;
+      const bool simple = useSimple && r1.y == REC_NEAR_DONE && r1.z == 1u;
+      if (!simple && nHits <= GENERAL_SMALL) kind = 1;
+      else if (simple && nHits > GENERAL_SMALL && nHits <= 3 * GENERAL_SMALL) kind = 2;
+    }
+    const uint32_t re = r0.x & 0x7FFFFFFFu, allele = r0.y;
+    const int pass = (r0.x >> 31) ? 0 : 1;
+    const bool lost = r0.w == T1K_ARENA_FULL;
+    const uint32_t *hh = P.genHits + (lost ? 0u : r0.w);
+    const bool lead = kind != 0 && tl == 0;
+    if (lead && lost) atomicOr(&P.counters[2], (unsigned long long)ERR_STAGECAP);
+    ReadCtx c{};
+    if (lead) c = makeCtx(P, re, pass, allele);
+    bool needScratch = false, needInline = false;
+    CandOut out{cbuf, 0, 6, TEAM_CAND_CAP};
+    const GapSink sink{P.memo + (uint64_t)re * GAP_CACHE, P.genJobStr, P.counters, re * GAP_CACHE, P.genJobSegCap, T1K_AR_GENJOBS};
+    teamSync();
+    if (lead && kind == 2) groupSimple<false>(hh, (int)nHits, c, k, P.hitLenRequired, A, out, &dpLocal, &P.counters[2], &needScratch, &sink, pass, &needInline);
+    const int n = kind == 1 ? (int)nHits : 0;
+#pragma unroll
+    for (int j = 0; j < HP; ++j) { const int i = tl + j * TEAM; if (i < n) C[i] = hh[i]; }
+    teamSync();
+#pragma unroll
+    for (int j = 0; j < HP; ++j) { const int i = tl + j * TEAM; if (i < n) A[teamRankByKey(C, n, i)] = C[i]; }
+    teamSync();
+    int s = 0;
+    while (__ballot(s < n) != 0ull) {
+      int e = s, dominant = 0;
+      bool run = false;
+      if (s < n) {
+        teamRunBounds(A, s, n, P.radius, &e, &dominant);
+        run = !(e - s < 3 || (e - s) * k < P.hitLenRequired);
+      }
+      bool kp[HP];
+      int m = 0;
+#pragma unroll
+      for (int j = 0; j < HP; ++j) {
+        const int qq = s + tl + j * TEAM;
+        kp[j] = run && qq < e && teamKeep(A, s, e, dominant, qq);
+        if (run && qq < e) C[qq] = kp[j] ? 1u : 0u;
+        m += kp[j] ? 1 : 0;
+      }
+#pragma unroll
+      for (int o = TEAM / 2; o > 0; o >>= 1) m += __shfl_xor(m, o, 64);
+      teamSync();
+#pragma unroll
+      for (int j = 0; j < HP; ++j) { const int qq = s + tl + j * TEAM; if (kp[j]) B[teamRankKept(A, C, s, e, qq)] = A[qq]; }
+      teamSync();
+      if (run && tl == 0) chainRun<false>(c, k, P.hitLenRequired, A, B, C, s, m, nullptr, 0, out, &dpLocal, &P.counters[2], &needScratch, &sink, pass, false, &needInline);
+      teamSync();
+      s = e;
+    }
+    if (lead) {
+      if (needScratch) { const uint32_t b = t1k_arena_append(P.counters, T1K_AR_BIG, P.rareSegCap); if (b != T1K_ARENA_FULL) P.bigStr[b] = gi; }
+      else if (needInline) { const uint32_t wq = t1k_arena_append(P.counters, T1K_AR_WAVE, P.rareSegCap); if (wq != T1K_ARENA_FULL) P.waveStr[wq] = gi; }
+      else {
+        ++genLocal;
+        if (kind == 2) ++nLong; else if (nHits <= GENERAL_SMALL / 2) ++nLow; else ++nHigh;
+        closeGeneralGroup(P, rec, out.n, cbuf);
+      }
+    }
+  }
+  t1k_stat_add(P.counters, T1K_STAT_DP, dpLocal);
+  t1k_stat_add(P.counters, T1K_STAT_GENERAL, genLocal);
+  t1k_path_add(P.counters, 1, nLong);
+  t1k_path_add(P.counters, 2, nLow);
+  t1k_path_add(P.counters, 3, nHigh);
 }
 
 __global__ __launch_bounds__(64) void k_chain_wave(ChainArgs P, uint32_t nItems, const unsigned long long *nDev, uint32_t cap, uint32_t above) {
@@ -1574,6 +1760,7 @@
   }
   t1k_stat_add(P.counters, T1K_STAT_DP, dpLocal);
   t1k_stat_add(P.counters, T1K_STAT_GENERAL, genLocal);
+  t1k_path_add(P.counters, 4, genLocal);
 }
 
 __global__ __launch_bounds__(WG) void k_general_finish(ChainArgs P, uint32_t nItems, const unsigned long long *nDev) {
@@ -1940,6 +2127,8 @@
   const unsigned long long *memo;
   __device__ __forceinline__ uint32_t operator()(uint32_t item) const { return (uint32_t)((memo[item] >> 5) & 0x1FF); }
 };
+#define GEN_BIN_LONG_CHAINS (GENERAL_SMALL + 1)
+#define GEN_BIN_WAVE (128 + GENERAL_SMALL + 1)
 struct GroupSizeKey {
   const uint32_t *recs; uint32_t stride; int useSimple;
   __device__ __forceinline__ uint32_t operator()(uint32_t item) const {
@@ -1960,7 +2149,8 @@
     if (h[b]) atomicAdd(&scratch[b], h[b]);
 }
 template <class KeyFn>
-__global__ __launch_bounds__(WG) void k_csort_scatter(const uint32_t *list, uint32_t n, uint32_t *scratch, uint32_t *out, KeyFn key, const unsigned long long *nDev) {
+__global__ __launch_bounds__(WG) void k_csort_scatter(const uint32_t *list, uint32_t n, uint32_t *scratch, uint32_t *out, KeyFn key, const unsigned long long *nDev,
+                                                       unsigned long long *bounds, uint32_t binA, uint32_t binB) {
   __shared__ uint32_t base[CS_BINS], h[CS_BINS], off[CS_BINS], warpSums[4];
   __shared__ uint32_t sLast;
   if (nDev) n = (uint32_t)*nDev;
@@ -1971,6 +2161,10 @@
     const uint32_t ex = t1k_block_scan_exclusive(a + b, warpSums, &tot);
     base[2 * threadIdx.x] = ex; base[2 * threadIdx.x + 1] = ex + a;
   }
+  if (bounds) {
+    __syncthreads();
+    if (blockIdx.x == 0 && threadIdx.x == 0) { bounds[0] = base[binA]; bounds[1] = base[binB]; }
+  }
   for (uint32_t t0 = blockIdx.x * CS_TILE; t0 < n; t0 += gridDim.x * CS_TILE) {
     for (int b = threadIdx.x; b < CS_BINS; b += WG) h[b] = 0;
     __syncthreads();
@@ -1999,7 +2193,8 @@
   }
 }
 template <class KeyFn>
-static const uint32_t *countingSort(t1k_ctx *ctx, const uint32_t *list, uint32_t n, KeyFn key, const unsigned long long *nDev = nullptr, uint64_t nEst = 0) {
+static const uint32_t *countingSort(t1k_ctx *ctx, const uint32_t *list, uint32_t n, KeyFn key, const unsigned long long *nDev = nullptr, uint64_t nEst = 0,
+                                    unsigned long long *bounds = nullptr, uint32_t binA = 0, uint32_t binB = 0) {
   static_assert(CS_BINS == 2 * WG, "two bins per thread in the prefix");
   const size_t head = (2 * CS_BINS + 16) * 4;
   const bool fresh = ctx->bJobSort.bytes < head + (size_t)n * 4;
@@ -2009,7 +2204,7 @@
   const uint64_t forGrid = nDev ? std::min<uint64_t>(n, nEst) : n;
   const uint32_t grid = (uint32_t)std::max<uint64_t>(1, std::min<uint64_t>((forGrid + CS_TILE - 1) / CS_TILE, 1024u));
   hipLaunchKernelGGL(k_csort_count<KeyFn>, dim3(grid), dim3(WG), 0, ctx->stream, list, n, scratch, key, nDev);
-  hipLaunchKernelGGL(k_csort_scatter<KeyFn>, dim3(grid), dim3(WG), 0, ctx->stream, list, n, scratch, sorted, key, nDev);
+  hipLaunchKernelGGL(k_csort_scatter<KeyFn>, dim3(grid), dim3(WG), 0, ctx->stream, list, n, scratch, sorted, key, nDev, bounds, binA, binB);
   return sorted;
 }
 void t1k_launch_dp_dense(t1k_ctx *ctx, const ChainArgs &a, const uint32_t *jobs, uint32_t n) {
@@ -2029,6 +2224,17 @@
   jobs = countingSort(ctx, jobs, cap, JobLenKey{(const unsigned long long *)a.memo}, nDev, est);
   const uint32_t grid = (uint32_t)std::max<uint64_t>(1, (std::min<uint64_t>(cap, est) + WG - 1) / WG);
   hipLaunchKernelGGL(k_dp_dense, dim3(grid), dim3(WG), 0, ctx->stream, a, jobs, cap, nDev);
+}
+
+#ifndef T1K_TEAM
+#define T1K_TEAM 16
+#endif
+static void launchChainSmall(t1k_ctx *ctx, const ChainArgs &g, uint32_t nItems, uint64_t est, int useSimple, const unsigned long long *nDev, const unsigned long long *bnd) {
+  constexpr uint32_t perWg = 64 / T1K_TEAM;
+  const uint64_t nb = std::max<uint64_t>(1, est);
+  if (useSimple) hipLaunchKernelGGL(k_chain_simple, dim3((uint32_t)((nb + 63) / 64)), dim3(64), 0, ctx->stream, g, nItems, nDev, bnd);
+  const uint32_t tgrid = (uint32_t)std::max<uint64_t>(1, std::min<uint64_t>((nb + perWg - 1) / perWg, std::max<uint64_t>(4096, nb / (4 * perWg))));
+  hipLaunchKernelGGL(k_chain_team<T1K_TEAM>, dim3(tgrid), dim3(64), 0, ctx->stream, g, nItems, useSimple, nDev, bnd);
 }
 
 uint64_t t1k_arena_estimate(const t1k_ctx *ctx, int arena, uint64_t cap, uint32_t nRe) {
@@ -2077,8 +2283,10 @@
     if (xlong) hipLaunchKernelGGL(k_gather_general<(T1K_LONG_READ_LEN + 63) / 64>, dim3(gatherGrid), dim3(WG), 0, ctx->stream, a, 0u, skipDone, nGen);
     else hipLaunchKernelGGL(k_gather_general<GROUP_FAST_MAXLEN / 64>, dim3(gatherGrid), dim3(WG), 0, ctx->stream, a, 0u, skipDone, nGen);
     ChainArgs g = a;
-    g.generalList = (uint32_t *)countingSort(ctx, a.generalList, (uint32_t)rareCap, GroupSizeKey{(const uint32_t *)a.recs, a.recStride, skipDone}, nGen, eGen);
-    hipLaunchKernelGGL(k_chain_general, dim3(blocks(eGen, 64)), dim3(64), 0, ctx->stream, g, 0u, skipDone, nGen);
+    unsigned long long *bnd = a.counters + T1K_GEN_BOUNDS;
+    g.generalList = (uint32_t *)countingSort(ctx, a.generalList, (uint32_t)rareCap, GroupSizeKey{(const uint32_t *)a.recs, a.recStride, skipDone}, nGen, eGen, bnd,
+                                             GEN_BIN_LONG_CHAINS, GEN_BIN_WAVE);
+    launchChainSmall(ctx, g, 0u, eGen, skipDone, nGen, g.generalList != a.generalList ? bnd : nullptr);
     const uint64_t eWave = est(T1K_AR_WAVE, rareCap);
     t1k_arena_compact_dev(ctx, T1K_AR_WAVE, a.waveStr, a.rareSegCap, a.waveList, eWave);
     T1K_HIP(ctx, hipFuncSetAttribute((const void *)k_chain_wave, hipFuncAttributeMaxDynamicSharedMemorySize, 3 * WAVE_CAP * 4));
@@ -2203,15 +2411,19 @@
     else hipLaunchKernelGGL(k_gather_general<GROUP_FAST_MAXLEN / 64>, dim3(std::min<uint32_t>((nGen + 3) / 4, 8192u)), dim3(WG), 0, ctx->stream, a, nGen, skipDone, NODEV);
     ChainArgs g = a;
     static const bool radix = getenv("T1K_RADIX_SORTS") != nullptr;
-    if (nGen >= 4096 && !radix)
-      g.generalList = (uint32_t *)countingSort(ctx, a.generalList, nGen, GroupSizeKey{(const uint32_t *)a.recs, a.recStride, skipDone});
+    const unsigned long long *bnd = nullptr;
+    if (nGen >= 4096 && !radix) {
+      g.generalList = (uint32_t *)countingSort(ctx, a.generalList, nGen, GroupSizeKey{(const uint32_t *)a.recs, a.recStride, skipDone}, nullptr, 0, a.counters + T1K_GEN_BOUNDS,
+                                               GEN_BIN_LONG_CHAINS, GEN_BIN_WAVE);
+      if (g.generalList != a.generalList) bnd = a.counters + T1K_GEN_BOUNDS;
+    }
     else if (nGen >= 4096 && t1k_ensure(ctx, ctx->bSlowKeys, (size_t)nGen * 20 + 64) == T1K_OK) {
       unsigned long long *k0 = (unsigned long long *)ctx->bSlowKeys.p, *k1 = k0 + nGen;
       uint32_t *sorted = (uint32_t *)(k1 + nGen);
       hipLaunchKernelGGL(k_group_size_keys, dim3((nGen + WG - 1) / WG), dim3(WG), 0, ctx->stream, (const uint32_t *)a.recs, a.recStride, (const uint32_t *)a.generalList, k0, nGen, skipDone);
       if (t1k_sort_pairs(ctx, k0, k1, a.generalList, sorted, nGen, 8) == T1K_OK) g.generalList = sorted;
     }
-    hipLaunchKernelGGL(k_chain_general, dim3((nGen + 63) / 64), dim3(64), 0, ctx->stream, g, nGen, skipDone, NODEV);
+    launchChainSmall(ctx, g, nGen, nGen, skipDone, NODEV, bnd);
     if ((rc = readCounters(ctx, hc))) return rc;
     const T1kArenaCounts wv = t1k_arena_counts(ctx, T1K_AR_WAVE, a.rareSegCap);
     if (wv.overflow) { hc[2] |= ERR_GROUPCAP; return 0; }
diff --git a/t1k_amd/csrc/t1k_dev.h b/t1k_amd/csrc/t1k_dev.h
--- a/t1k_amd/csrc/t1k_dev.h
+++ b/t1k_amd/csrc/t1k_dev.h
@@ -549,6 +549,8 @@
 #ifndef T1K_TRUNC_LARGE_WAVES
 #define T1K_TRUNC_LARGE_WAVES 0
 #endif
+#define T1K_PATH_BASE 32
+#define T1K_GEN_BOUNDS 38
 #define T1K_NSTRIPE 32
 enum { T1K_AR_GROUPS = 0, T1K_AR_JOBS, T1K_AR_RETRY, T1K_AR_FINISH, T1K_AR_GENERAL, T1K_AR_BIG, T1K_AR_GENCAND, T1K_AR_EQ, T1K_AR_BAND, T1K_AR_WIDE, T1K_AR_GENHITS, T1K_AR_GENJOBS, T1K_AR_WAVE, T1K_AR_EXTJOBS, T1K_AR_EXTRETRY, T1K_AR_SLOW, T1K_NARENA };
 #define T1K_ARENA_BASE (64 + T1K_STAT_STRIPES * 8)
@@ -669,6 +671,7 @@
   int traceFetch = 0;
   uint32_t upN = 0; int upS = 0, upMaxLen = 0; uint64_t upBytes = 0; bool upOpen = false;
   hipEvent_t upEv[4] = {nullptr, nullptr, nullptr, nullptr}; bool upEvSet[4] = {false, false, false, false};
+  uint64_t pathCounts[6] = {0, 0, 0, 0, 0, 0};
   uint64_t lastSlowGroups = 0;
   uint64_t estTotal[T1K_NARENA] = {};
   bool estValid = false;
```

Result: no change. 3.606 million (median of 3 runs) (-1.3%).
